# gleb-kov/wordpiece

Hardware: AMD Instinct MI355X
Metric: input MB/s tokenized (bert-base-cased vocab; offline stand-in: synthetic BERT-like vocab) (higher is better)
Workload: dtype int32

## Files before the change

wordpiece_amd/csrc/context.h:

```cpp
#pragma once
#include <array>
#include <cstring>
#include <memory>
#include <mutex>
#include <string>
#include <vector>

#include "../../include/wordpiece_amd.h"
#include "code.h"
#include "decode.h"
#include "detok.h"
#include "radix_sort.h"
#include "scanline.h"
#include "suffix_array.h"
#include "vocab.h"

namespace wp {

static thread_local std::string g_last_error;

struct EnvOptions {
  bool arena_guard;
  bool vocab_in_s;
  bool sparse_emit;
  bool no_pool;
  static bool flag(const char *name) {
    const char *e = getenv(name);
    return e && atoi(e) != 0;
  }
  static const EnvOptions &get() {
    static const EnvOptions o{flag("WP_ARENA_GUARD"), flag("WP_VOCAB_IN_S"), flag("WP_SPARSE_EMIT"), flag("WP_NO_CONTEXT_POOL")};
    return o;
  }
};

struct DeviceBuffer {
  void *p = nullptr;
  size_t cap = 0;
  void ensure(size_t bytes, bool slack = true) {
    if (bytes <= cap) return;
    if (p) WP_HIP(hipFree(p));
    p = nullptr;
    cap = 0;
    size_t want = slack ? bytes + bytes / 16 + (1 << 20) : bytes;
    WP_HIP(hipMalloc(&p, want));
    cap = want;
  }
  void release() {
    if (p) (void)hipFree(p);
    p = nullptr;
    cap = 0;
  }
};

static size_t text_room(size_t len) { return len + 64; }
static void zero_text_tail(void *d_text, size_t len, hipStream_t st) {
  WP_HIP(hipMemsetAsync(static_cast<char *>(d_text) + (len & ~static_cast<size_t>(15)), 0, 32, st));
}

constexpr size_t kGuardBytes = 256;
constexpr uint32_t kGuardWord = 0xA5C3F00Du;

__global__ __launch_bounds__(kBlock) void guard_fill_kernel(char *base, const unsigned long long *offs, int count) {
  const int z = blockIdx.x;
  if (z >= count) return;
  uint32_t *g = reinterpret_cast<uint32_t *>(base + offs[z]);
  if (threadIdx.x < kGuardBytes / 4) g[threadIdx.x] = kGuardWord;
}
__global__ __launch_bounds__(kBlock) void guard_check_kernel(const char *base, const unsigned long long *offs, int count,
                                                             uint32_t *bad) {
  const int z = blockIdx.x;
  if (z >= count) return;
  const uint32_t *g = reinterpret_cast<const uint32_t *>(base + offs[z]);
  const bool broken = threadIdx.x < kGuardBytes / 4 && g[threadIdx.x] != kGuardWord;
  if (__syncthreads_or(broken) && threadIdx.x == 0) {
    atomicAdd(&bad[0], 1u);
    atomicMin(&bad[1], static_cast<uint32_t>(z) + 1u);
  }
}

struct Arena {
  DeviceBuffer *buf;
  size_t off = 0, planned = 0;
  bool planning = true, guard = false;
  std::vector<unsigned long long> zones;
  explicit Arena(DeviceBuffer *b, bool g = false) : buf(b), guard(g) {}
  template <typename T>
  T *take(size_t count) {
    size_t bytes = (count * sizeof(T) + 255) & ~static_cast<size_t>(255);
    size_t o = off;
    off += bytes;
    if (guard) {
      if (!planning) zones.push_back(off);
      off += kGuardBytes;
    }
    if (planning) return nullptr;
    if (off > planned) throw std::logic_error("arena: the allocation sequence differs from the planned one");
    return reinterpret_cast<T *>(static_cast<char *>(buf->p) + o);
  }
  void commit() {
    buf->ensure(off + (guard ? 8 * 512 : 0));
    planned = off;
    off = 0;
    planning = false;
  }
  unsigned long long *zone_table() const {
    return reinterpret_cast<unsigned long long *>(static_cast<char *>(buf->p) + ((off + 255) & ~static_cast<size_t>(255)));
  }
  void arm(hipStream_t st) {
    if (!guard || zones.empty()) return;
    if (zones.size() > 500) throw std::logic_error("arena guard: too many allocations");
    WP_HIP(hipMemcpyAsync(zone_table(), zones.data(), zones.size() * sizeof(unsigned long long), hipMemcpyHostToDevice, st));
    WP_HIP(hipStreamSynchronize(st));
    hipLaunchKernelGGL(guard_fill_kernel, dim3(zones.size()), dim3(kBlock), 0, st, static_cast<char *>(buf->p), zone_table(),
                       static_cast<int>(zones.size()));
  }
  void check(hipStream_t st, uint32_t *bad) const {
    if (!guard || zones.empty()) return;
    hipLaunchKernelGGL(guard_check_kernel, dim3(zones.size()), dim3(kBlock), 0, st, static_cast<const char *>(buf->p),
                       zone_table(), static_cast<int>(zones.size()), bad);
  }
};

static int bit_length(uint64_t v) {
  int b = 0;
  while (v) {
    b++;
    v >>= 1;
  }
  return b;
}

constexpr int kScalars = 56;
constexpr int kScalarCps = 0;
constexpr int kScalarAlphabet = 1;
constexpr int kScalarInvalid = 2;
constexpr int kScalarList = 4;
constexpr int kScalarListEntries = kScalarList + 0;
constexpr int kScalarListGroups = kScalarList + 1;
constexpr int kScalarListLargeGroups = kScalarList + 2;
constexpr int kScalarListLargeEntries = kScalarList + 3;
constexpr int kScalarListWanted = 8;
constexpr int kScalarIds = 9;
constexpr int kScalarAnchors = 10;
constexpr int kScalarAnchorGap = 11;
constexpr int kScalarLongWords = 12;
constexpr int kScalarWideWords = 13;
constexpr int kScalarCps64 = 14;
constexpr int kScalarGuard = 16;
constexpr int kScalarGuardBad = kScalarGuard + 0;
constexpr int kScalarGuardFirst = kScalarGuard + 1;
constexpr int kScalarSplitTotals = 18;
constexpr int kScalarAlphaWord0 = 20;
constexpr int kScalarRows = 21, kScalarRowsBad = 22, kScalarRowsCut = 23;
constexpr int kScalarCand = 24;
constexpr int kScalarKept = 25;
constexpr int kScalarSrcRows = 26;
constexpr int kScalarInCut = 27, kScalarInRows = 28, kScalarInWindowed = 30;
constexpr int kScalarFree31 = 31;
constexpr int kScalarMask = 32;
constexpr int kScalarDetokLast = 44, kScalarDetokBad = 46;
constexpr int kScalarFree47 = 47;
constexpr int kScalarDetok = 48;
constexpr int kScalarNormBytes = kScalarCps;
constexpr int kScalarNormCps = kScalarAlphabet;
constexpr int kScalarNormSrcCps = kScalarListEntries;
constexpr int kScalarNormBytes64 = kScalarCps64;

struct ScalarRange {
  int first, words;
};
constexpr ScalarRange kScalarLayout[] = {
    {kScalarCps, 1},         {kScalarAlphabet, 1},   {kScalarInvalid, 2},         {kScalarListEntries, 1},
    {kScalarListGroups, 1},  {kScalarListLargeGroups, 1}, {kScalarListLargeEntries, 1}, {kScalarListWanted, 1},
    {kScalarIds, 1},         {kScalarAnchors, 1},    {kScalarAnchorGap, 1},       {kScalarLongWords, 1},
    {kScalarWideWords, 1},   {kScalarCps64, 2},      {kScalarGuardBad, 1},        {kScalarGuardFirst, 1},
    {kScalarSplitTotals, 2},      {kScalarAlphaWord0, 1}, {kScalarRows, 1},            {kScalarRowsBad, 1},
    {kScalarRowsCut, 1},     {kScalarCand, 1},       {kScalarKept, 1},            {kScalarSrcRows, 1},
    {kScalarInCut, 1},       {kScalarInRows, 2},     {kScalarInWindowed, 1},      {kScalarFree31, 1},
    {kScalarMask, 12},       {kScalarDetokLast, 2},  {kScalarDetokBad, 1},        {kScalarFree47, 1},
    {kScalarDetok, 8}};
constexpr int scalar_end(int slot) {
  for (const ScalarRange &r : kScalarLayout) {
    if (slot < r.first + r.words) return r.first + r.words;
  }
  return kScalars;
}
constexpr bool scalar_layout_ok() {
  int at = 0;
  for (const ScalarRange &r : kScalarLayout) {
    if (r.first != at || r.words < 1 || (r.words % 2 == 0 && r.first % 2 != 0)) return false;
    at += r.words;
  }
  return at == kScalars;
}
static_assert(scalar_layout_ok(), "the scalar table must cover d_scalars word by word, 64-bit slots on even words");
static_assert(kScalarList % 2 == 0 && kScalarListLargeGroups % 2 == 0, "both halves of the list block are also read as 64-bit words");

struct RowsCall {
  const long long *d_doc_off = nullptr;
  size_t n_docs = 0;
  int unit = -1;
  size_t capacity = SIZE_MAX;
  size_t n_rows = 0;
  const long long *d_starts = nullptr;
  const long long *d_row_splits = nullptr;
  uint32_t *d_line_cnt = nullptr;
};

enum SideEvent { kEvFork, kEvJoin, kEvScalars, kEvKeysFree, kEvPartition, kEvTrieNodes, kEvLargeSorted, kEvKeysBuilt, kEvCandCount,
                 kEvSpine, kEvKept, kEvSorted, kEvListBuilt, kEvRoundDone, kSideEvents };
enum TimingMark { kMarkStart, kMarkCounted, kMarkSymbols, kMarkSorted, kMarkLcp, kMarkScanned, kMarkWalked, kMarkNormStart,
                  kMarkRound0, kTimingMarks, kMarkNormEnd = kMarkStart };

struct Context {
  int device = 0;
  hipStream_t stream = nullptr;
  hipStream_t stream2 = nullptr;
  hipStream_t stream3 = nullptr;
  hipEvent_t evs[kSideEvents] = {};
  uint32_t *d_stream = nullptr, *d_elig_start = nullptr, *d_elig_info = nullptr, *d_soft = nullptr;
  uint32_t *d_vocab_word_idx = nullptr, *d_vocab_word_bits = nullptr;
  uint8_t *d_cls_bmp = nullptr;
  uint32_t *d_lt_chain_len = nullptr, *d_lt_chain_off = nullptr, *d_lt_child_begin = nullptr, *d_lt_child_cp = nullptr,
           *d_lt_child_node = nullptr, *d_elig_node = nullptr, *d_elig_subtree = nullptr;
  int32_t *d_elig_id = nullptr, *d_tok_len = nullptr;
  uint8_t *d_tok_class = nullptr;
  DetokRec *d_detok_rec = nullptr;
  uint8_t *d_detok_pool = nullptr;
  size_t detok_pool_bytes = 0;
  unsigned long long *d_trie_key = nullptr;
  uint32_t *d_trie_child = nullptr;
  int32_t *d_trie_id = nullptr;
  DeviceBuffer text_buf, a_buf, b_buf, fmt_buf;
  DeviceBuffer text_buf2, ids_stage[2];
  DeviceBuffer rows_in, rows_out, pad_buf;
  DeviceBuffer inputs_buf;
  DeviceBuffer detok_in, detok_aux, detok_out;
  uint16_t *d_norm_index = nullptr;
  uint32_t *d_norm_pages = nullptr, *d_norm_pool = nullptr;
  DeviceBuffer norm_buf, norm_aux, norm_map;
  hipStream_t up_stream = nullptr, down_stream = nullptr;
  hipEvent_t pipe_ev[4] = {};
  uint32_t *d_used = nullptr, *d_lut = nullptr, *d_scan_tmp = nullptr;
  uint32_t *d_scalars = nullptr;
  uint8_t *d_code = nullptr;
  size_t list_hint = 0;
  SymbolCode code_cache;
  bool code_cached = false;
  uint32_t code_alphabet = 0;
  int code_bits = 0, code_lo = 0, code_uses = 0;
  double code_blank_share = 0.0;
  uint8_t *h_code = nullptr;
  uint32_t *d_symhist = nullptr;
  uint32_t *h_scalars = nullptr;
  RadixStats rstats;
  hipEvent_t ev[kTimingMarks] = {};
  const int32_t *d_ids = nullptr;
  const uint32_t *d_offs = nullptr;
  struct {
    const void *sym = nullptr;
    int sym_bytes = 0;
    const uint32_t *sa = nullptr, *cps = nullptr;
    const RankEntry *rank = nullptr;
    const int32_t *lcp = nullptr;
    const uint8_t *cls = nullptr;
    StepTable steps{};
    int32_t *best_scratch = nullptr;
    const int32_t *step_views = nullptr;
    size_t n = 0, n_text = 0;
  } dbg;
  std::array<DeviceBuffer *, 17> buffers() {
    return {&text_buf, &a_buf,    &b_buf,   &fmt_buf,    &text_buf2, &ids_stage[0], &ids_stage[1], &rows_in,   &rows_out,
            &pad_buf,  &inputs_buf, &norm_buf, &norm_aux, &norm_map, &detok_in,     &detok_aux,    &detok_out};
  }
  Context() = default;
  Context(const Context &) = delete;
  Context &operator=(const Context &) = delete;
  ~Context();
};

struct DeviceGuard {
  int prev = -1;
  DeviceGuard() {
    if (hipGetDevice(&prev) != hipSuccess) prev = -1;
  }
  ~DeviceGuard() {
    if (prev >= 0) (void)hipSetDevice(prev);
  }
  DeviceGuard(const DeviceGuard &) = delete;
  DeviceGuard &operator=(const DeviceGuard &) = delete;
};

#ifdef WP_DEBUG_BOUNDS
static void take_oob(int first, int count, unsigned int *oob) {
  WP_HIP(hipMemcpyFromSymbol(oob, HIP_SYMBOL(g_wp_oob), count * sizeof(unsigned int), first * sizeof(unsigned int)));
  bool any = false;
  for (int i = 0; i < count; i++) any = any || oob[i] != 0;
  if (!any) return;
  const unsigned int zero[kBoundSites] = {};
  WP_HIP(hipMemcpyToSymbol(HIP_SYMBOL(g_wp_oob), zero, count * sizeof(unsigned int), first * sizeof(unsigned int)));
}
#endif

}

using namespace wp;

struct EncodeStats : wp_stats {
  int32_t normalize;
  int64_t norm_bytes;
  double ms_normalize;
  wp_walk_stats walk;
  wp_refine_stats refine;
  wp_refine_sched sched;
  wp_step_stats step;
  wp_inputs_stats inputs;
  int32_t inputs_call;
  wp_mask_stats mask;
  int32_t mask_call;
  wp_detok_stats detok;
  int32_t detok_call;
};

#ifndef WP_LATE_REFINE_DEFAULT
#define WP_LATE_REFINE_DEFAULT 0
#endif

struct wp_vocab {
  HostVocab hv;
  std::unique_ptr<Context> ctx;
  std::vector<std::unique_ptr<Context>> multi;
  int device = -1;
  bool full_depth = false, keep_debug = false, stage_timing = false, lcp_kasai = false, cover_anchors = false;
  bool keep_step_views = false;
  bool arena_guard = false;
  bool sparse_emit = false;
  bool vocab_in_s = false;
  bool indexed_round0 = false;
  bool sort_blanks = false;
  bool late_refine = WP_LATE_REFINE_DEFAULT != 0;
  int normalize = 0;
  int n_devices = 1;
  EncodeStats stats{};
  ~wp_vocab();
};

namespace wp {

template <typename... T>
static void free_dev(T *&...p) {
  (((p ? (void)hipFree(p) : (void)0), p = nullptr), ...);
}

static void free_vocab_tables(Context *c) {
  free_dev(c->d_stream, c->d_elig_start, c->d_elig_info, c->d_soft, c->d_elig_id, c->d_tok_len, c->d_tok_class, c->d_detok_rec, c->d_detok_pool, c->d_trie_key,
           c->d_trie_child, c->d_trie_id, c->d_vocab_word_idx, c->d_vocab_word_bits, c->d_cls_bmp, c->d_lt_chain_len,
           c->d_lt_chain_off, c->d_lt_child_begin, c->d_lt_child_cp, c->d_lt_child_node, c->d_elig_node, c->d_elig_subtree);
}

template <size_t N>
static void destroy_events(hipEvent_t (&events)[N]) {
  for (auto &e : events) {
    if (e) (void)hipEventDestroy(e);
    e = nullptr;
  }
}

static void destroy_context(Context *c) {
  if (!c) return;
  bool owns = c->stream || c->stream2 || c->stream3 || c->d_used || c->d_lut || c->d_scan_tmp || c->d_scalars || c->d_code ||
              c->d_symhist || c->h_scalars || c->h_code || c->d_stream;
  for (DeviceBuffer *b : c->buffers()) owns = owns || b->p;
  if (!owns) return;
  DeviceGuard keep;
  (void)hipSetDevice(c->device);
  free_vocab_tables(c);
  free_dev(c->d_used, c->d_lut, c->d_scan_tmp, c->d_scalars, c->d_code, c->d_symhist, c->d_norm_index, c->d_norm_pages, c->d_norm_pool);
  if (c->h_scalars) (void)hipHostFree(c->h_scalars);
  if (c->h_code) (void)hipHostFree(c->h_code);
  c->h_scalars = nullptr;
  c->h_code = nullptr;
  for (DeviceBuffer *b : c->buffers()) b->release();
  destroy_events(c->pipe_ev);
  destroy_events(c->ev);
  destroy_events(c->evs);
  for (hipStream_t *s : {&c->up_stream, &c->down_stream, &c->stream3, &c->stream2, &c->stream}) {
    if (*s) (void)hipStreamDestroy(*s);
    *s = nullptr;
  }
}
Context::~Context() { destroy_context(this); }

template <typename T>
static T *upload(const std::vector<T> &v, hipStream_t st) {
  T *d = nullptr;
  WP_HIP(hipMalloc(&d, std::max<size_t>(v.size(), 1) * sizeof(T)));
  if (!v.empty()) WP_HIP(hipMemcpyAsync(d, v.data(), v.size() * sizeof(T), hipMemcpyHostToDevice, st));
  return d;
}

static constexpr size_t kPoolArenaBytes = size_t(256) << 20;
static constexpr size_t kPoolContexts = 4;
static std::mutex g_pool_mu;
static std::vector<std::unique_ptr<Context>> &context_pool() {
  static auto *pool = new std::vector<std::unique_ptr<Context>>();
  return *pool;
}

static void release_arenas(Context *c) {
  for (DeviceBuffer *b : c->buffers()) b->release();
  c->d_ids = nullptr;
  c->d_offs = nullptr;
  c->dbg = {};
}

static void park_context(std::unique_ptr<Context> c) {
  if (!c) return;
  const bool no_pool = EnvOptions::get().no_pool;
  DeviceGuard keep;
  (void)hipSetDevice(c->device);
  if (!no_pool && hipStreamSynchronize(c->stream) == hipSuccess && hipStreamSynchronize(c->stream2) == hipSuccess &&
      hipStreamSynchronize(c->stream3) == hipSuccess) {
    free_vocab_tables(c.get());
    size_t held = 0;
    for (DeviceBuffer *b : c->buffers()) held += b->cap;
    if (held > kPoolArenaBytes) release_arenas(c.get());
    c->d_ids = nullptr;
    c->d_offs = nullptr;
    c->dbg = {};
    std::lock_guard<std::mutex> g(g_pool_mu);
    if (context_pool().size() < kPoolContexts) {
      context_pool().push_back(std::move(c));
      return;
    }
  }
  destroy_context(c.get());
}

static void upload_vocab_tables(Context *c, const HostVocab &hv) {
  c->d_stream = upload(hv.stream, c->stream);
  c->d_elig_start = upload(hv.elig_start, c->stream);
  c->d_elig_info = upload(hv.elig_info, c->stream);
  c->d_elig_id = upload(hv.elig_id, c->stream);
  c->d_tok_len = upload(hv.tok_len, c->stream);
  c->d_soft = upload(hv.soft, c->stream);
  c->d_vocab_word_idx = upload(hv.used_word_idx, c->stream);
  c->d_vocab_word_bits = upload(hv.used_word_bits, c->stream);
  c->d_cls_bmp = upload(hv.cls_bmp, c->stream);
  c->d_lt_chain_len = upload(hv.lt_chain_len, c->stream);
  c->d_lt_chain_off = upload(hv.lt_chain_off, c->stream);
  c->d_lt_child_begin = upload(hv.lt_child_begin, c->stream);
  c->d_lt_child_cp = upload(hv.lt_child_cp, c->stream);
  c->d_lt_child_node = upload(hv.lt_child_node, c->stream);
  c->d_elig_node = upload(hv.elig_node, c->stream);
  c->d_elig_subtree = upload(hv.elig_subtree, c->stream);
  {
    std::vector<unsigned long long> tk(hv.trie_key.begin(), hv.trie_key.end());
    c->d_trie_key = upload(tk, c->stream);
    WP_HIP(hipStreamSynchronize(c->stream));
  }
  c->d_trie_child = upload(hv.trie_child, c->stream);
  c->d_trie_id = upload(hv.trie_id, c->stream);
  WP_HIP(hipStreamSynchronize(c->stream));
}

static int device_count_or_throw() {
  int count = 0;
  if (hipGetDeviceCount(&count) != hipSuccess || count == 0) {
    throw HipError("no HIP device available: the Linear WordPiece path has no CPU fallback");
  }
  return count;
}

static std::unique_ptr<Context> make_context(const wp_vocab *v, int device) {
  const int count = device_count_or_throw();
  if (device >= 0) {
    if (device >= count) throw std::invalid_argument("no such HIP device: " + std::to_string(device));
  } else {
    WP_HIP(hipGetDevice(&device));
  }
  WP_HIP(hipSetDevice(device));
  std::unique_ptr<Context> c;
  {
    std::lock_guard<std::mutex> g(g_pool_mu);
    auto &pool = context_pool();
    for (size_t i = 0; i < pool.size(); i++) {
      if (pool[i]->device == device) {
        c = std::move(pool[i]);
        pool.erase(pool.begin() + static_cast<long>(i));
        break;
      }
    }
  }
  if (c) {
    upload_vocab_tables(c.get(), v->hv);
    return c;
  }
  c.reset(new Context());
  c->device = device;
  WP_HIP(hipStreamCreateWithFlags(&c->stream, hipStreamNonBlocking));
  WP_HIP(hipStreamCreateWithFlags(&c->stream2, hipStreamNonBlocking));
  WP_HIP(hipStreamCreateWithFlags(&c->stream3, hipStreamNonBlocking));
  for (auto &e : c->evs) WP_HIP(hipEventCreateWithFlags(&e, hipEventDisableTiming));
  WP_HIP(hipMalloc(&c->d_used, sizeof(uint32_t) * kCpWords));
  WP_HIP(hipMalloc(&c->d_lut, sizeof(uint32_t) * kCpTableSize));
  WP_HIP(hipMalloc(&c->d_scan_tmp, sizeof(uint32_t) * kCpWords));
  WP_HIP(hipMalloc(&c->d_scalars, sizeof(uint32_t) * kScalars));
  WP_HIP(hipMalloc(&c->d_code, 512 + 256 + kDecodeTableBytes));
  WP_HIP(hipHostMalloc(&c->h_code, 512 + 256 + kDecodeTableBytes));
  WP_HIP(hipMalloc(&c->d_symhist, sizeof(uint32_t) * 256));
  WP_HIP(hipHostMalloc(&c->h_scalars, sizeof(uint32_t) * kScalars));
  for (auto &e : c->ev) WP_HIP(hipEventCreate(&e));
  upload_vocab_tables(c.get(), v->hv);
  return c;
}

static Context *get_context(wp_vocab *v) {
  if (!v->ctx) v->ctx = make_context(v, v->device);
  WP_HIP(hipSetDevice(v->ctx->device));
  return v->ctx.get();
}

static void queue_scalars(Context *c, int last, hipStream_t st) {
  WP_HIP(hipMemcpyAsync(c->h_scalars, c->d_scalars, sizeof(uint32_t) * scalar_end(last), hipMemcpyDeviceToHost, st));
}
static void fetch_scalars(Context *c, int last) {
  queue_scalars(c, last, c->stream);
  WP_HIP(hipStreamSynchronize(c->stream));
}
static void clear_scalars(Context *c, int first, int last, hipStream_t st) {
  WP_HIP(hipMemsetAsync(c->d_scalars + first, 0, sizeof(uint32_t) * (scalar_end(last) - first), st));
}

}
```

wordpiece_amd/csrc/linear_path.h:

```cpp
#pragma once
#include <functional>

#include "context.h"
#include "local_sort.h"
#include "prune.h"
#include "trie.h"
#include "offsets.h"
#include "normalize.h"
#include "rows.h"
#include "walk.h"

namespace wp {

struct ListOverflow {
  size_t wanted;
};

__global__ void needed_list_clamp_kernel(uint32_t *__restrict__ totals, uint32_t cap, uint32_t *__restrict__ wanted) {
  if (totals[0] > cap) {
    *wanted = totals[0];
    totals[0] = 0;
    totals[1] = 0;
  }
}

constexpr double kBlankDropMinShare = 1.0 / 16;

#ifdef WP_DEBUG_BOUNDS
__device__ unsigned int g_wp_sorted_sig[6];
__global__ __launch_bounds__(kBlock) void sorted_check_kernel(const uint32_t *__restrict__ sorted, size_t n_sorted,
                                                              const uint32_t *__restrict__ unsorted, size_t n,
                                                              const uint8_t *__restrict__ cls, size_t n_text,
                                                              const uint32_t *__restrict__ blank_bits) {
  __shared__ uint32_t acc[7];
  if (threadIdx.x < 7) acc[threadIdx.x] = 0u;
  __syncthreads();
  uint32_t bad = 0, cnt[2] = {0, 0}, sum[2] = {0, 0}, x[2] = {0, 0};
  const size_t first = static_cast<size_t>(blockIdx.x) * kBlock + threadIdx.x, stride = static_cast<size_t>(gridDim.x) * kBlock;
  for (size_t i = first; i < n_sorted; i += stride) {
    const uint32_t k = sorted[i];
    if (i + 1 < n_sorted && k > sorted[i + 1]) bad++;
    if (blank_bits && key_is_blank(blank_bits, k)) bad++;
    cnt[0]++;
    sum[0] += k;
    x[0] ^= k;
  }
  for (size_t i = first; i < n; i += stride) {
    if (blank_bits && i < n_text && (cls[i] & kClsSpace)) continue;
    const uint32_t k = unsorted[i];
    cnt[1]++;
    sum[1] += k;
    x[1] ^= k;
  }
  if (bad) atomicAdd(&acc[6], bad);
  for (int s = 0; s < 2; s++) {
    if (cnt[s]) {
      atomicAdd(&acc[3 * s], cnt[s]);
      atomicAdd(&acc[3 * s + 1], sum[s]);
      atomicXor(&acc[3 * s + 2], x[s]);
    }
  }
  __syncthreads();
  if (threadIdx.x < 6 && acc[threadIdx.x]) {
    if (threadIdx.x % 3 == 2) {
      atomicXor(&g_wp_sorted_sig[threadIdx.x], acc[threadIdx.x]);
    } else {
      atomicAdd(&g_wp_sorted_sig[threadIdx.x], acc[threadIdx.x]);
    }
  }
  if (threadIdx.x == 6 && acc[6]) atomicAdd(&g_wp_oob[kSiteSortOrder], acc[6]);
}
__global__ void sorted_check_close_kernel() {
  bool same = true;
  for (int j = 0; j < 3; j++) same = same && g_wp_sorted_sig[j] == g_wp_sorted_sig[3 + j];
  wp_in_bounds(same, kSiteSortOrder);
  for (int j = 0; j < 6; j++) g_wp_sorted_sig[j] = 0u;
}
#endif

template <typename SymT>
struct LinearPath {
  const wp_vocab *v;
  Context *c;
  EncodeStats &S;
  Arena &ar, &aa;
  const uint8_t *d_text;
  size_t nbytes;
  const uint32_t *d_tile_prefix;
  size_t n_text, n;
  uint32_t *d_cps;
  uint8_t *d_cls;
  int bits;
  bool text_only;
  int offs_unit;
  RowsCall *rows;
  const NormMap *nmap;

  hipStream_t st, st2;
  const HostVocab &hv;
  bool full, prune, use_trie, key_lookup, keys_only, window_store, use_digit_bytes, staged_possible, sparse_emit;
  bool early_refine;
  bool wide_ran = false;
  uint32_t need_depth;
  int M, P, P_cap, bucket_shift, bucket_shift_all, key_shift, key_shift_all, hb_n, win_mid;
  unsigned sl_tiles, sl_groups, nbuckets, nbuckets_all, nkbuckets, nkbuckets_all;
  size_t radix_words, emit_tiles, walk_blocks, claim_size, list_cap;

  SymT *d_sym = nullptr, *d_vsym = nullptr;
  Key0 *KA = nullptr, *KB = nullptr;
  uint32_t *VA = nullptr, *VB = nullptr;
  uint32_t *X0 = nullptr, *X1 = nullptr;
  uint8_t *DG0 = nullptr, *DG1 = nullptr;
  RankEntry *d_rank = nullptr;
  uint32_t *d_node_of_slot = nullptr;
  int32_t *d_lcp = nullptr;
  uint32_t *d_sa = nullptr, *d_gdepth = nullptr;
  RankEntry *d_hd_n = nullptr;
  int32_t *d_emit = nullptr, *d_dbg_best = nullptr;
  int32_t *d_step_views = nullptr;
  uint32_t *d_anchors = nullptr, *d_anchor_cnt = nullptr, *d_anchor_tmp = nullptr, *d_emit_cnt = nullptr, *d_emit_tmp = nullptr,
           *d_blk_cnt = nullptr, *d_blk_off = nullptr, *d_tile_scratch = nullptr;
  uint32_t *AS0 = nullptr, *AS1 = nullptr, *AG = nullptr, *AD0 = nullptr, *AD1 = nullptr, *LA = nullptr, *LB = nullptr, *d_tdep = nullptr;
  uint64_t *LK0 = nullptr, *LK1 = nullptr, *LK2 = nullptr;
  uint32_t *LV0 = nullptr, *LV1 = nullptr, *LPOS = nullptr;
  uint32_t *d_ghead = nullptr, *d_gneed0 = nullptr, *d_gneed1 = nullptr, *d_lg_head = nullptr, *d_lg_off = nullptr;
  RerankAgg *d_agg = nullptr, *d_chunk_agg = nullptr;
  uint32_t *d_claim = nullptr, *d_claim_need = nullptr, *d_gclaim = nullptr, *d_gfirst = nullptr, *d_gdep = nullptr, *d_gnode = nullptr,
           *d_gdone = nullptr, *d_rng_lo = nullptr, *d_rng_hi = nullptr, *d_child_sym = nullptr, *d_radix_tmp = nullptr,
           *d_radix_tmp2 = nullptr;
  uint8_t *d_rng_long = nullptr;
  uint32_t *d_mslot0 = nullptr, *d_mslot1 = nullptr, *d_midx0 = nullptr, *d_midx1 = nullptr, *d_minfo = nullptr, *d_tile_mlo = nullptr;
  int32_t *d_mid = nullptr, *d_rf = nullptr, *d_rb = nullptr, *d_cover_f = nullptr, *d_cover_b = nullptr;
  int32_t *d_tmin_f = nullptr, *d_tmin_b = nullptr, *d_gmin_f = nullptr, *d_gmin_b = nullptr, *d_pval_p = nullptr, *d_pval_s = nullptr;
  uint32_t *d_ps0 = nullptr, *d_ps1 = nullptr, *d_pv0 = nullptr, *d_pv1 = nullptr, *d_bidx = nullptr;
  int2 *d_bfast = nullptr, *d_bfast_all = nullptr;
  uint32_t *d_bidx_all = nullptr;
  uint32_t *d_gend = nullptr, *d_kstart = nullptr, *d_kbidx = nullptr, *d_kbidx_all = nullptr;
  int32_t *d_kval_p = nullptr, *d_kval_s = nullptr;
  int2 *d_kbfast = nullptr, *d_kbfast_all = nullptr;
  unsigned long long *d_cand_table = nullptr;
  uint32_t *d_cand_filter = nullptr, *d_cand_lo = nullptr, *d_cand_hi = nullptr, *d_gcand = nullptr;
  uint32_t *d_tok_group = nullptr;
  uint32_t *d_cand_bcnt = nullptr, *d_cand_boff = nullptr, *d_cand_scan = nullptr;
  int cand_bits = 0;
  uint32_t *d_blank_bits = nullptr;
  uint2 *d_ospill = nullptr, *d_cspan = nullptr, *d_offs = nullptr;
  uint32_t *d_byte_of = nullptr;
  long long *d_line_starts = nullptr, *d_row_splits = nullptr;
  uint32_t *d_row_base = nullptr;

  SymbolCode code;
  DevCode dcode{};
  DigitBytes db;
  RadixPlan sort_plan;
  bool hist_in_keys = false;
  bool drop_blanks = false;
  size_t n_sorted = 0;
  int cur = 0, rounds = 1;
  Key0 *keys = nullptr, *other_keys = nullptr;
  uint32_t *vals = nullptr, *other_vals = nullptr, *slots = nullptr, *other_slots = nullptr, *adep = nullptr, *other_dep = nullptr;
  uint32_t *avals = nullptr, *spare_vals = nullptr;
  bool classified = false, anchors_queued = false;
  size_t n_act = 0, n_large = 0, n_large_groups = 0, n_groups = 0;
  StepTable steps{}, steps_all{};
  StepTable ksteps{}, ksteps_all{};
  CandSet cand{};
  CandRuns cand_runs{};
  size_t n_cand = 0;

  LinearPath(const wp_vocab *v_, Context *c_, EncodeStats &S_, Arena &ar_, Arena &aa_, const uint8_t *text, size_t nb,
             const uint32_t *tile_prefix, size_t n_text_, size_t n_, uint32_t *cps, uint8_t *cls, int bits_, bool text_only_,
             int offs_unit_, RowsCall *rows_ = nullptr, const NormMap *nmap_ = nullptr)
      : v(v_), c(c_), S(S_), ar(ar_), aa(aa_), d_text(text), nbytes(nb), d_tile_prefix(tile_prefix), n_text(n_text_), n(n_),
        d_cps(cps), d_cls(cls), bits(bits_), text_only(text_only_), offs_unit(offs_unit_), rows(rows_), nmap(nmap_), st(c_->stream), st2(c_->stream2),
        hv(v_->hv) {
    full = v->full_depth || hv.n_dup_eligible > 0 || v->lcp_kasai;
    need_depth = static_cast<uint32_t>(std::min<int64_t>(hv.longest + 1, 0x7fffffff));
    M = static_cast<int>(hv.elig_id.size());
    prune = !full && (M > 0 || text_only);
    use_trie = text_only && !full && M > 0;
    key_lookup = use_trie && !v->keep_debug && kKeyBits <= 32;
    keys_only = key_lookup && !v->indexed_round0 && sizeof(SymT) == 1;
    early_refine = keys_only && !v->late_refine;
    sl_tiles = cdiv(n, kSlTile);
    sl_groups = cdiv(sl_tiles, kSlGroup);
    P = kStepsPerMark * M + 1;
    P_cap = P + 2 * M + 2;
    const int bucket_bits = std::min(kStepBucketBitsMax, std::max(kStepBucketBits, bit_length(4 * static_cast<size_t>(P))));
    bucket_shift = std::max(0, bit_length(n) - bucket_bits);
    nbuckets = static_cast<unsigned>(((n - 1) >> bucket_shift) + 1);
    bucket_shift_all = std::max(0, bit_length(n) - kStepBucketBits);
    nbuckets_all = static_cast<unsigned>(((n - 1) >> bucket_shift_all) + 1);
    const int kb = std::min(kKeyBits, std::max(1, bit_length(n - 1) - bucket_shift));
    const int kb_all = std::min(kKeyBits, std::max(1, bit_length(n - 1) - bucket_shift_all));
    key_shift = kKeyBits - kb;
    key_shift_all = kKeyBits - kb_all;
    nkbuckets = 1u << kb;
    nkbuckets_all = 1u << kb_all;
    radix_words = std::max(radix_tmp_words<uint64_t>(n), radix_tmp_words<uint32_t>(std::max<size_t>(n, static_cast<size_t>(P_cap))));
    emit_tiles = cdiv(std::max<size_t>(n_text, 1), kScanTile);
    walk_blocks = cdiv(std::max<size_t>(n_text, 1), kBlock);
    sparse_emit = v->sparse_emit || EnvOptions::get().sparse_emit;
    staged_possible = !sparse_emit && !v->cover_anchors && hv.soft.empty();
    use_digit_bytes = n > kRadixSmallN;
    claim_size = 1024;
    while (claim_size < 2 * static_cast<size_t>(std::max(M, 1))) claim_size *= 2;
    cand_bits = bit_length(claim_size - 1);
    hb_n = bit_length(n - 1);
    window_store = n >= (1u << 22);
    win_mid = hb_n - kWinBits <= kRadixBits ? hb_n : kWinBits + (hb_n - kWinBits + 1) / 2;
    if (!prune) {
      list_cap = n;
    } else {
      const size_t guess = c->list_hint ? c->list_hint : n / 8;
      list_cap = std::min(n, guess + guess / 4 + 65536);
    }
    S.symbol_bits = bits;
    S.full_depth = full;
    S.trie_refine = use_trie ? 1 : 0;
    S.key_bits = kKeyBits;
    S.round0_keys_only = keys_only ? 1 : 0;
    S.round0_candidates = keys_only ? 0 : -1;
    n_sorted = n;
    S.round0_sorted = static_cast<int64_t>(n);
  }

  void fork() {
    WP_HIP(hipEventRecord(c->evs[kEvFork], st));
    WP_HIP(hipStreamWaitEvent(st2, c->evs[kEvFork], 0));
  }
  void join() {
    WP_HIP(hipEventRecord(c->evs[kEvJoin], st2));
    WP_HIP(hipStreamWaitEvent(st, c->evs[kEvJoin], 0));
  }

  void plan() {
    const bool ref = !text_only;
    const bool want_lcp = ref || v->keep_debug;
    const size_t lc = list_cap, lg = lc / 2 + static_cast<size_t>(M) + 8;
    const size_t rr_tiles_l = cdiv(lc, kRrTile);
    const size_t rtiles = cdiv(std::max<size_t>(n_text, 1), kReachTile);
    for (int pass = 0; pass < 2; pass++) {
      d_sym = ar.take<SymT>(n + 16);
      KA = ar.take<Key0>(n + 16);
      KB = ar.take<Key0>(n + 16);
      VA = ar.take<uint32_t>(n + 16);
      VB = ar.take<uint32_t>(n + 16);
      X0 = ar.take<uint32_t>(n + 16);
      X1 = ar.take<uint32_t>(n + 16);
      DG0 = use_digit_bytes ? ar.take<uint8_t>(n + 64) : nullptr;
      DG1 = use_digit_bytes ? ar.take<uint8_t>(n + 64) : nullptr;
      d_rank = ar.take<RankEntry>(n);
      d_node_of_slot = use_trie ? ar.take<uint32_t>(n) : nullptr;
      d_lcp = want_lcp ? ar.take<int32_t>(n) : nullptr;
      d_sa = (v->keep_debug || v->lcp_kasai) ? ar.take<uint32_t>(n) : nullptr;
      d_gdepth = (use_trie && !want_lcp) ? nullptr : ar.take<uint32_t>(n);
      d_hd_n = (want_lcp || !prune) ? ar.take<RankEntry>(n + 16) : nullptr;
      d_dbg_best = v->keep_debug ? ar.take<int32_t>(2 * n) : nullptr;
      d_emit = ar.take<int32_t>(n_text + 1);
      d_anchors = ar.take<uint32_t>(n_text + 1);
      d_anchor_cnt = ar.take<uint32_t>(emit_tiles + 1);
      d_anchor_tmp = ar.take<uint32_t>(cdiv(emit_tiles, kScanTile) + 8);
      d_emit_cnt = ar.take<uint32_t>(emit_tiles + 1);
      d_emit_tmp = ar.take<uint32_t>(cdiv(walk_blocks, kScanTile) + 8);
      d_blk_cnt = ar.take<uint32_t>(walk_blocks + 2);
      d_blk_off = ar.take<uint32_t>(walk_blocks + 2);
      d_tile_scratch = ar.take<uint32_t>(5 * (rtiles + 2) + 4 * (n_text / kMaxAnchorGap + 4));
      AS0 = ar.take<uint32_t>(lc);
      AS1 = ar.take<uint32_t>(lc);
      AG = ar.take<uint32_t>(lc);
      AD0 = ar.take<uint32_t>(lc);
      AD1 = ar.take<uint32_t>(lc);
      LA = ar.take<uint32_t>(lc);
      LB = ar.take<uint32_t>(lc);
      d_tdep = ar.take<uint32_t>(lc + 2);
      LK0 = ar.take<uint64_t>(lc + 2);
      LK1 = ar.take<uint64_t>(lc + 2);
      LK2 = ar.take<uint64_t>(lc + 2);
      LV0 = ar.take<uint32_t>(lc);
      LV1 = ar.take<uint32_t>(lc);
      LPOS = ar.take<uint32_t>(lc + 16);
      d_ghead = ar.take<uint32_t>(lg);
      d_gneed0 = use_trie ? nullptr : ar.take<uint32_t>(lg);
      d_gneed1 = use_trie ? nullptr : ar.take<uint32_t>(lg);
      d_lg_head = ar.take<uint32_t>(lc / kLsMaxGroup + 4);
      d_lg_off = ar.take<uint32_t>(lc / kLsMaxGroup + 4);
      d_agg = ar.take<RerankAgg>(rr_tiles_l + 1);
      d_chunk_agg = ar.take<RerankAgg>(cdiv(rr_tiles_l, kRrChunk) + 1);
      d_radix_tmp = ar.take<uint32_t>(radix_words);
      d_radix_tmp2 = use_trie ? ar.take<uint32_t>(std::max(radix_tmp_words<uint64_t>(lc), keys_only ? radix_tmp_words<uint32_t>(n) : 0))
                              : nullptr;
      d_claim = ar.take<uint32_t>(claim_size);
      if (keys_only) {
        uint32_t *zeroed = ar.take<uint32_t>(3 * claim_size);
        d_cand_lo = zeroed;
        d_cand_hi = zeroed ? zeroed + claim_size : nullptr;
        d_claim_need = zeroed ? zeroed + 2 * claim_size : nullptr;
      } else {
        d_claim_need = ar.take<uint32_t>(claim_size);
      }
      d_gclaim = ar.take<uint32_t>(M + 4);
      d_gfirst = ar.take<uint32_t>(M + 4);
      d_gdep = ar.take<uint32_t>(M + 4);
      d_gnode = ar.take<uint32_t>(M + 4);
      d_gdone = ar.take<uint32_t>(M + 4);
      d_rng_lo = ar.take<uint32_t>(M + 1);
      d_rng_hi = ar.take<uint32_t>(M + 1);
      d_rng_long = ar.take<uint8_t>(M + 1);
      d_vsym = use_trie ? ar.take<SymT>(hv.stream.size() + 16) : nullptr;
      d_child_sym = use_trie ? ar.take<uint32_t>(hv.lt_child_cp.size() + 1) : nullptr;
      d_mslot0 = ar.take<uint32_t>(M + 1);
      d_mslot1 = ar.take<uint32_t>(M + 1);
      d_midx0 = ar.take<uint32_t>(M + 1);
      d_midx1 = ar.take<uint32_t>(M + 1);
      d_mid = ar.take<int32_t>(M + 1);
      d_minfo = ar.take<uint32_t>(M + 1);
      d_rf = ar.take<int32_t>(M + 1);
      d_cover_f = ar.take<int32_t>(2 * static_cast<size_t>(M) + 2);
      d_cover_b = ar.take<int32_t>(2 * static_cast<size_t>(M) + 2);
      d_rb = ar.take<int32_t>(M + 1);
      d_tile_mlo = ref ? ar.take<uint32_t>(sl_tiles + 2) : nullptr;
      d_tmin_f = ref ? ar.take<int32_t>(sl_tiles + 1) : nullptr;
      d_tmin_b = ref ? ar.take<int32_t>(sl_tiles + 1) : nullptr;
      d_gmin_f = ref ? ar.take<int32_t>(sl_groups + 1) : nullptr;
      d_gmin_b = ref ? ar.take<int32_t>(sl_groups + 1) : nullptr;
      d_ps0 = ar.take<uint32_t>(P_cap + 1);
      d_ps1 = ar.take<uint32_t>(P_cap + 1);
      d_pv0 = ar.take<uint32_t>(P_cap + 1);
      d_pv1 = ar.take<uint32_t>(P_cap + 1);
      d_pval_p = ar.take<int32_t>(P_cap + 1);
      d_pval_s = ar.take<int32_t>(P_cap + 1);
      d_bidx = ar.take<uint32_t>(static_cast<size_t>(nbuckets) + 2);
      d_bfast = ar.take<int2>(static_cast<size_t>(nbuckets) + 1);
      d_bidx_all = bucket_shift_all != bucket_shift ? ar.take<uint32_t>(static_cast<size_t>(nbuckets_all) + 2) : nullptr;
      d_bfast_all = bucket_shift_all != bucket_shift ? ar.take<int2>(static_cast<size_t>(nbuckets_all) + 1) : nullptr;
      d_gend = key_lookup ? ar.take<uint32_t>(M + 4) : nullptr;
      d_kstart = key_lookup ? ar.take<uint32_t>(P_cap + 1) : nullptr;
      d_kval_p = key_lookup ? ar.take<int32_t>(P_cap + 1) : nullptr;
      d_kval_s = key_lookup ? ar.take<int32_t>(P_cap + 1) : nullptr;
      d_kbidx = key_lookup ? ar.take<uint32_t>(static_cast<size_t>(nkbuckets) + 2) : nullptr;
      d_kbfast = key_lookup ? ar.take<int2>(static_cast<size_t>(nkbuckets) + 1) : nullptr;
      d_kbidx_all = (key_lookup && key_shift_all != key_shift) ? ar.take<uint32_t>(static_cast<size_t>(nkbuckets_all) + 2) : nullptr;
      d_kbfast_all = (key_lookup && key_shift_all != key_shift) ? ar.take<int2>(static_cast<size_t>(nkbuckets_all) + 1) : nullptr;
      d_cand_table = keys_only ? ar.take<unsigned long long>(claim_size) : nullptr;
      d_cand_filter = keys_only ? ar.take<uint32_t>(kCandFilterWords) : nullptr;
      d_gcand = keys_only ? ar.take<uint32_t>(M + 4) : nullptr;
      d_tok_group = keys_only ? ar.take<uint32_t>(M + 1) : nullptr;
      d_cand_bcnt = keys_only ? ar.take<uint32_t>(cdiv(n, kKeyTile) + 2) : nullptr;
      d_cand_boff = keys_only ? ar.take<uint32_t>(cdiv(n, kKeyTile) + 2) : nullptr;
      d_cand_scan = keys_only ? ar.take<uint32_t>(cdiv(cdiv(n, kKeyTile), kScanTile) + 8) : nullptr;
      d_blank_bits = keys_only ? ar.take<uint32_t>(kBlankWords) : nullptr;
      const bool offs = offs_unit >= 0;
      d_ospill = offs ? ar.take<uint2>(n_text + 16) : nullptr;
      d_cspan = offs ? ar.take<uint2>(n_text + 16) : nullptr;
      d_offs = offs ? ar.take<uint2>(n_text + 1) : nullptr;
      d_byte_of = ((offs_unit == WP_OFFSETS_BYTES && !nmap) || rows) ? ar.take<uint32_t>(n_text + 1) : nullptr;
      d_line_starts = (rows && (!rows->d_doc_off || nmap)) ? ar.take<long long>(rows->n_rows + 1) : nullptr;
      d_row_splits = rows ? ar.take<long long>(rows->n_rows + 1) : nullptr;
      d_row_base = (rows && rows->unit >= 0) ? ar.take<uint32_t>(rows->n_rows + 1) : nullptr;
      d_step_views = v->keep_step_views ? ar.take<int32_t>(4 * n_text + 4) : nullptr;
      if (pass == 0) ar.commit();
    }
    ar.arm(st);
  }

  void launch_anchors(hipStream_t as) {
    anchors_queued = true;
    const unsigned atiles = cdiv(n_text, kAnchorTile);
    if (!staged_possible) WP_HIP(hipMemsetAsync(d_emit, 0x80, n_text * sizeof(int32_t), as));
    hipLaunchKernelGGL(anchor_count_kernel, dim3(atiles), dim3(kBlock), 0, as, d_cls, static_cast<const uint8_t *>(nullptr),
                       n_text, d_anchor_cnt);
    device_exclusive_scan(d_anchor_cnt, d_anchor_cnt, atiles, d_anchor_tmp, c->d_scalars + kScalarAnchors, as);
    hipLaunchKernelGGL(anchor_write_kernel, dim3(atiles), dim3(kBlock), 0, as, d_cls, static_cast<const uint8_t *>(nullptr),
                       n_text, d_anchor_cnt, d_anchors);
    hipLaunchKernelGGL(anchor_gap_kernel, dim3(std::min<size_t>(atiles, 1024)), dim3(kBlock), 0, as, d_anchors,
                       c->d_scalars + kScalarAnchors, n_text, d_cls, hv.soft.empty() ? 1 : 0, c->d_scalars + kScalarAnchorGap);
  }

  void symbols_and_keys() {
    const int lo_bits = sizeof(SymT) == 1 ? 0 : std::max(0, bits - 8);
    constexpr int kCodeReuse = 64;
    const bool reuse_code = c->code_cached && c->code_alphabet == static_cast<uint32_t>(S.alphabet) && c->code_bits == bits &&
                            c->code_lo == lo_bits && c->code_uses < kCodeReuse;
    if (!reuse_code) WP_HIP(hipMemsetAsync(c->d_symhist, 0, sizeof(uint32_t) * 256, st));
    constexpr uint32_t kBlankCpRuns[3][2] = {{0x09, 7}, {0x20, 2}, {kSpaceToken, 2}};
    uint32_t h_blank_lut[3][7] = {};
    hipLaunchKernelGGL(HIP_KERNEL_NAME(decode_write_kernel<SymT>), dim3(cdiv(nbytes, kDecTile)), dim3(kBlock), 0, st, d_text,
                       nbytes, d_tile_prefix, c->d_lut, d_sym, d_cls, d_cps, c->d_cls_bmp, c->d_soft,
                       static_cast<int>(hv.soft.size()), reuse_code ? nullptr : c->d_symhist, lo_bits);
    hipLaunchKernelGGL(HIP_KERNEL_NAME(map_vocab_symbols_kernel<SymT>), dim3(cdiv(n - n_text, kBlock)), dim3(kBlock), 0, st,
                       c->d_stream, n_text, n, c->d_lut, d_sym);
    if (reuse_code) {
      code = c->code_cache;
      c->code_uses++;
    } else {
      std::vector<uint32_t> h32(256);
      WP_HIP(hipMemcpyAsync(h32.data(), c->d_symhist, sizeof(uint32_t) * 256, hipMemcpyDeviceToHost, st));
      if (sizeof(SymT) == 1) {
        for (int r = 0; r < 3; r++) {
          WP_HIP(hipMemcpyAsync(h_blank_lut[r], c->d_lut + kBlankCpRuns[r][0], sizeof(uint32_t) * kBlankCpRuns[r][1],
                                hipMemcpyDeviceToHost, st));
        }
      }
      WP_HIP(hipStreamSynchronize(st));
      const size_t nitems = (static_cast<size_t>(S.alphabet) >> lo_bits) + 1;
      std::vector<uint64_t> freq(nitems);
      for (size_t i = 0; i < nitems; i++) freq[i] = h32[i];
      code = build_symbol_code(freq, bits, true);
      if (!code.uniform_bits) {
        code.lo_bits = lo_bits;
        code.avg_bits += lo_bits;
      }
      c->code_cache = code;
      c->code_cached = true;
      c->code_alphabet = static_cast<uint32_t>(S.alphabet);
      c->code_bits = bits;
      c->code_lo = lo_bits;
      c->code_uses = 0;
      uint64_t all = 0, blank = 0;
      for (size_t i = 0; i < nitems; i++) all += freq[i];
      if (sizeof(SymT) == 1) {
        for (int r = 0; r < 3; r++) {
          for (uint32_t k = 0; k + 1 < kBlankCpRuns[r][1]; k++) {
            const uint32_t cp = kBlankCpRuns[r][0] + k, s = h_blank_lut[r][k] + 1u;
            if (is_space(cp) && h_blank_lut[r][k + 1] != h_blank_lut[r][k] && s < nitems) blank += freq[s];
          }
        }
      }
      c->code_blank_share = all ? static_cast<double>(blank) / static_cast<double>(all) : 0.0;
      if (!code.uniform_bits) {
        const size_t blob_bytes = 512 + 256 + kDecodeTableBytes;
        std::memset(c->h_code, 0, blob_bytes);
        std::memcpy(c->h_code, code.cw.data(), code.cw.size() * sizeof(uint16_t));
        std::memcpy(c->h_code + 512, code.len.data(), code.len.size());
        std::memcpy(c->h_code + 768, code.bmask.data(), kDecodeTableBytes);
        WP_HIP(hipMemcpyAsync(c->d_code, c->h_code, blob_bytes, hipMemcpyHostToDevice, st));
      }
    }
    dcode = DevCode{reinterpret_cast<const uint16_t *>(c->d_code), c->d_code + 512, c->d_code + 768,
                    code.uniform_bits ? code.uniform_bits : -code.lo_bits};
    S.symbols_per_key = static_cast<int32_t>(kKeyBits / std::max(1.0, code.avg_bits));
    if (keys_only) {
      WP_HIP(hipMemsetAsync(d_cand_table, 0, claim_size * sizeof(unsigned long long), st));
      WP_HIP(hipMemsetAsync(d_cand_filter, 0, kCandFilterWords * sizeof(uint32_t), st));
      hipLaunchKernelGGL(long_key_set_kernel, dim3(cdiv(static_cast<size_t>(M) * kWave, kBlock)), dim3(kBlock), 0, st, c->d_stream,
                         c->d_elig_start, c->d_elig_info, M, c->d_lut, dcode, d_cand_table, cand_bits, d_cand_filter);
      cand.filter = d_cand_filter;
      cand.table = d_cand_table;
      cand.table_bits = cand_bits;
      cand.slot = VA;
      cand.pos = VB;
      cand.bcount = d_cand_bcnt;
    }
    size_t cand_blocks = 0;
    int min_len = code.uniform_bits ? code.uniform_bits : 99;
    for (uint8_t l : code.len) min_len = std::min<int>(min_len, l);
    if (sizeof(SymT) == 1 && min_len >= kKeys8MinLen) {
      cand.tile = kKeys8Tile;
      cand_blocks = cdiv(n, kKeys8Tile);
      if (n > kRadixSmallN) {
        sort_plan = radix_plan<Key0>(n, d_radix_tmp, radix_words, st);
        hist_in_keys = true;
      }
      drop_blanks = keys_only && hist_in_keys && !v->sort_blanks && c->code_blank_share >= kBlankDropMinShare;
      if (drop_blanks) {
        hipLaunchKernelGGL(blank_bits_kernel, dim3(1), dim3(kBlankWords), 0, st, c->d_lut, dcode, d_blank_bits);
      }
      hipLaunchKernelGGL(build_keys0_u8_kernel, dim3(cdiv(n, kKeys8Tile)), dim3(kKeys8Threads), 0, st,
                         reinterpret_cast<const uint8_t *>(d_sym), n, dcode, KA, hist_in_keys ? nullptr : DG0,
                         hist_in_keys ? sort_plan.table : nullptr, hist_in_keys ? sort_plan.chunk_sums0 : nullptr, cand,
                         drop_blanks ? d_blank_bits : nullptr);
    } else {
      cand.tile = kKeyTile;
      cand_blocks = cdiv(n, kKeyTile);
      if (keys_only) {
        hipLaunchKernelGGL(HIP_KERNEL_NAME(build_keys0_kernel<SymT, true>), dim3(cdiv(n, kKeyTile)), dim3(kBlock), 0, st, d_sym, n,
                           dcode, KA, DG0, cand);
      } else {
        hipLaunchKernelGGL(HIP_KERNEL_NAME(build_keys0_kernel<SymT, false>), dim3(cdiv(n, kKeyTile)), dim3(kBlock), 0, st, d_sym, n,
                           dcode, KA, DG0, cand);
      }
    }
    if (keys_only) {
      WP_HIP(hipEventRecord(c->evs[kEvKeysBuilt], st));
      WP_HIP(hipStreamWaitEvent(st2, c->evs[kEvKeysBuilt], 0));
      device_exclusive_scan(d_cand_bcnt, d_cand_boff, cand_blocks, d_cand_scan, c->d_scalars + kScalarCand, st2);
      hipLaunchKernelGGL(cand_compact_kernel, dim3(cand_blocks), dim3(kBlock), 0, st2, VA, VB, d_cand_bcnt, d_cand_boff, cand.tile, n,
                         X1, d_node_of_slot);
      WP_HIP(hipMemcpyAsync(c->h_scalars + kScalarCand, c->d_scalars + kScalarCand, sizeof(uint32_t), hipMemcpyDeviceToHost, st2));
      WP_HIP(hipEventRecord(c->evs[kEvCandCount], st2));
    }
    WP_LAUNCH_CHECK();
  }

  void sort_round0() {
    db.dg0 = DG0;
    db.dg1 = DG1;
    db.dg0_ready = DG0 != nullptr && !hist_in_keys;
    if (key_lookup) {
      Key0 *sk = reinterpret_cast<Key0 *>(X0);
      RadixDrop drop;
      drop.blank_bits = d_blank_bits;
      drop.d_kept = c->d_scalars + kScalarKept;
      drop.h_kept = c->h_scalars + kScalarKept;
      drop.side = st2;
      drop.spine_done = c->evs[kEvSpine];
      drop.copied = c->evs[kEvKept];
      cur = radix_sort_pairs<Key0>(sk, keys_only ? nullptr : VA, KB, keys_only ? nullptr : VB, n, 0, kKeyBits, d_radix_tmp, radix_words,
                                   st, &c->rstats, true, code.uniform_bits ? 0 : 8, db, true, hist_in_keys ? &sort_plan : nullptr, KA,
                                   drop_blanks ? &drop : nullptr);
      if (drop_blanks) n_sorted = drop.kept;
      S.round0_sorted = static_cast<int64_t>(n_sorted);
      S.hist_in_keys = hist_in_keys ? 1 : 0;
      keys = cur ? KB : sk;
      other_keys = cur ? sk : KB;
#ifdef WP_DEBUG_BOUNDS
      if constexpr (sizeof(Key0) == 4) {
        hipLaunchKernelGGL(sorted_check_kernel, dim3(std::min<size_t>(cdiv(n, kBlock), 1024)), dim3(kBlock), 0, st,
                           reinterpret_cast<const uint32_t *>(keys), n_sorted, reinterpret_cast<const uint32_t *>(KA), n, d_cls, n_text,
                           drop_blanks ? d_blank_bits : static_cast<const uint32_t *>(nullptr));
        hipLaunchKernelGGL(sorted_check_close_kernel, dim3(1), dim3(1), 0, st);
        WP_LAUNCH_CHECK();
      }
#endif
      vals = keys_only ? nullptr : (cur ? VB : VA);
      other_vals = keys_only ? nullptr : (cur ? VA : VB);
      if (keys_only) sort_candidates();
      slots = AS0;
      other_slots = AS1;
      adep = AD0;
      other_dep = AD1;
      avals = LA;
      spare_vals = LB;
      return;
    }
    if (window_store) {
      db.tail_bit = kWinBits;
      db.tail_mask = (1u << (win_mid - kWinBits)) - 1u;
      db.tail_from_val = true;
    }
    cur = radix_sort_pairs<Key0>(KA, VA, KB, VB, n, 0, kKeyBits, d_radix_tmp, radix_words, st, &c->rstats, true,
                                 code.uniform_bits ? 0 : 8, db, true, hist_in_keys ? &sort_plan : nullptr);
    S.hist_in_keys = hist_in_keys ? 1 : 0;
    keys = cur ? KB : KA;
    other_keys = cur ? KA : KB;
    vals = cur ? VB : VA;
    other_vals = cur ? VA : VB;
    slots = AS0;
    other_slots = AS1;
    adep = AD0;
    other_dep = AD1;
    avals = LA;
    spare_vals = LB;
  }

  void sort_candidates() {
    WP_HIP(hipEventSynchronize(c->evs[kEvCandCount]));
    n_cand = c->h_scalars[kScalarCand];
    S.round0_candidates = static_cast<int64_t>(n_cand);
    WP_HIP(hipMemsetAsync(d_cand_lo, 0, 3 * claim_size * sizeof(uint32_t), st2));
    const uint32_t *sorted_slot = X1, *sorted_pos = d_node_of_slot;
    if (n_cand > 1) {
      const int cc = radix_sort_pairs<uint32_t>(X1, d_node_of_slot, VA, VB, n_cand, 0, cand_bits, d_radix_tmp2,
                                                std::max(radix_tmp_words<uint64_t>(list_cap), radix_tmp_words<uint32_t>(n)), st2, nullptr,
                                                false, cand_bits, DigitBytes(), true);
      sorted_slot = cc ? VA : X1;
      sorted_pos = cc ? VB : d_node_of_slot;
    }
    if (n_cand > 0) {
      hipLaunchKernelGGL(cand_runs_kernel, dim3(cdiv(n_cand, kBlock)), dim3(kBlock), 0, st2, sorted_slot, n_cand, d_cand_lo, d_cand_hi);
    }
    WP_LAUNCH_CHECK();
    cand_runs.table = d_cand_table;
    cand_runs.bits = cand_bits;
    cand_runs.lo = d_cand_lo;
    cand_runs.hi = d_cand_hi;
    cand_runs.pos = sorted_pos;
  }

  bool classify_groups(size_t list_len) {
    if (list_len <= static_cast<size_t>(kLsMaxGroup)) return false;
    const size_t cap = list_len / 2 + 1;
    clear_scalars(c, kScalarListLargeGroups, kScalarListLargeEntries, st2);
    hipLaunchKernelGGL(large_groups_kernel, dim3(std::min<size_t>(cdiv(cap, kBlock), 2048)), dim3(kBlock), 0, st2, d_ghead,
                       c->d_scalars + kScalarListGroups, reinterpret_cast<unsigned long long *>(c->d_scalars + kScalarListLargeGroups),
                       d_lg_head, d_lg_off);
    hipLaunchKernelGGL(large_groups_close_kernel, dim3(1), dim3(1), 0, st2, c->d_scalars + kScalarListLargeGroups, d_lg_off);
    return true;
  }

  void store_ranks(uint32_t *dst, uint32_t *val, uint32_t *t_dst, uint32_t *t_val, size_t m) {
    if (val && m >= (1u << 22)) {
      const int hb = bit_length(n - 1);
      const int bc = radix_sort_pairs<uint32_t>(dst, val, t_dst, t_val, m, std::max(0, hb - 8), hb, d_radix_tmp, radix_words, st,
                                                nullptr, false, hb + 1, DigitBytes(), true);
      hipLaunchKernelGGL(scatter_pairs_kernel, dim3(cdiv(m, kSpTile)), dim3(kBlock), 0, st, bc ? t_dst : dst, bc ? t_val : val, m,
                         d_rank, n, 1);
    } else {
      hipLaunchKernelGGL(scatter_pairs_kernel, dim3(cdiv(m, kSpTile)), dim3(kBlock), 0, st, dst, val, m, d_rank, n, 0);
    }
  }

  void store_ranks_round0(uint32_t *dst, uint32_t *val, uint8_t *dig, uint8_t *other, const std::function<void()> &before_second,
                          const std::function<void()> &before_window) {
    WP_HIP(hipFuncSetAttribute(reinterpret_cast<const void *>(window_store_kernel), hipFuncAttributeMaxDynamicSharedMemorySize,
                               static_cast<int>(kWinLdsBytes)));
    uint32_t *a_dst = X0, *a_val = X1, *b_dst = other_vals, *b_val = reinterpret_cast<uint32_t *>(keys);
    DigitBytes d1;
    d1.dg0 = dig;
    d1.dg1 = other;
    d1.dg0_ready = dig != nullptr;
    if (win_mid < hb_n) {
      d1.tail_bit = win_mid;
      d1.tail_mask = (1u << (hb_n - win_mid)) - 1u;
    }
    radix_sort_pairs<uint32_t>(dst, val, a_dst, a_val, n, kWinBits, win_mid, d_radix_tmp, radix_words, st, &c->rstats,
                               val == nullptr, 0, d1, true);
    if (before_second) before_second();
    const uint32_t *f_dst = a_dst, *f_val = a_val;
    if (win_mid < hb_n) {
      DigitBytes d2;
      d2.dg0 = dig ? d1.tail_out(1) : nullptr;
      d2.dg1 = dig ? dig : nullptr;
      d2.dg0_ready = dig != nullptr;
      radix_sort_pairs<uint32_t>(a_dst, a_val, b_dst, b_val, n, win_mid, hb_n, d_radix_tmp, radix_words, st, &c->rstats, false, 0,
                                 d2);
      f_dst = b_dst;
      f_val = b_val;
    }
    if (before_window) before_window();
    hipLaunchKernelGGL(window_store_kernel, dim3(cdiv(n, size_t(1) << kWinBits)), dim3(kWinThreads), kWinLdsBytes, st, f_dst, f_val,
                       n, d_rank);
  }

  void ranks_round0() {
    const DepthRule rule{need_depth, full ? 1 : 0, nullptr, nullptr, 0, nullptr};
    const unsigned tiles = cdiv(n, kRrTile);
    const bool slot_ranks = text_only && !d_lcp;
    uint8_t *dig = DG0 ? db.tail_out(cur) : nullptr, *dig_other = DG0 ? db.tail_out(cur ^ 1) : nullptr;
    auto enqueue_needed_groups = [&](hipEvent_t start_after) {
      if (start_after) WP_HIP(hipStreamWaitEvent(st2, start_after, 0));
      WP_HIP(hipMemsetAsync(d_claim, 0xff, claim_size * sizeof(uint32_t), st2));
      if (!keys_only) WP_HIP(hipMemsetAsync(d_claim_need, 0, claim_size * sizeof(uint32_t), st2));
      NeededList nl{slots, avals, AG, adep, d_ghead, d_gfirst, d_gdep, reinterpret_cast<unsigned long long *>(c->d_scalars + kScalarList),
                    static_cast<uint32_t *>(nullptr), need_depth, d_claim_need, d_gclaim, d_gneed0,
                    keys_only ? d_gcand : nullptr, keys_only ? cand_runs.pos : nullptr, keys_only ? n_cand : 0};
      const TokenTrie trie{c->d_lt_chain_len, c->d_lt_chain_off, c->d_lt_child_begin, c->d_lt_child_node, d_child_sym};
      if (use_trie) {
        const size_t ns = hv.stream.size(), nc = hv.lt_child_cp.size();
        hipLaunchKernelGGL(HIP_KERNEL_NAME(trie_map_symbols_kernel<SymT>), dim3(cdiv(std::max<size_t>(std::max(ns, nc), 1), kBlock)),
                           dim3(kBlock), 0, st2, c->d_stream, ns, c->d_lt_child_cp, nc, c->d_lut, d_vsym, d_child_sym);
      }
      if (M > 0) {
        hipLaunchKernelGGL(HIP_KERNEL_NAME(need_groups_kernel<SymT>), dim3(cdiv(static_cast<size_t>(M) * kWave, kBlock)),
                           dim3(kBlock), 0, st2, keys, vals, n_sorted, n, d_sym, c->d_stream, c->d_elig_start, c->d_elig_info, M, c->d_lut, dcode,
                           d_claim, static_cast<uint32_t>(claim_size - 1), nl, text_only ? d_rng_lo : nullptr, d_rng_hi, d_rng_long,
                           cand_runs);
      }
      hipLaunchKernelGGL(needed_list_clamp_kernel, dim3(1), dim3(1), 0, st2, c->d_scalars + kScalarList, static_cast<uint32_t>(list_cap),
                         c->d_scalars + kScalarListWanted);
      hipLaunchKernelGGL(needed_list_close_kernel, dim3(1), dim3(1), 0, st2, c->d_scalars + kScalarList, d_ghead);
      if (key_lookup) {
        hipLaunchKernelGGL(group_starts_kernel, dim3(cdiv(M, kBlock)), dim3(kBlock), 0, st2, d_gfirst, d_ghead, c->d_scalars + kScalarList,
                           n_sorted, d_ps0 + P, d_gend);
      }
      if (M > 0) {
        if (!use_trie) hipLaunchKernelGGL(needed_need_kernel, dim3(cdiv(M, kBlock)), dim3(kBlock), 0, st2, nl);
        hipLaunchKernelGGL(needed_fill_kernel, dim3(1024), dim3(kBlock), 0, st2, nl, vals, n_sorted);
        if (use_trie) {
          hipLaunchKernelGGL(HIP_KERNEL_NAME(trie_group_start_kernel<SymT>), dim3(cdiv(M, kBlock)), dim3(kBlock), 0, st2, vals,
                             keys_only ? cand_runs.pos : nullptr, d_gcand, d_gfirst,
                             d_gdep, c->d_scalars + kScalarList, d_sym, n, d_vsym, trie, d_gnode, d_gdone);
        }
      }
      WP_HIP(hipEventRecord(c->evs[kEvKeysFree], st2));
      if (use_trie) trie_round_sizes();
    };
    if (early_refine) {
      refine_early();
      return;
    }
    if (key_lookup) {
      fork();
      enqueue_needed_groups(nullptr);
      trie_round_sort();
      if (n_text > 0) launch_anchors(st);
      WP_LAUNCH_CHECK();
      trie_round_finish();
      return;
    }
    if (prune) {
      fork();
      enqueue_needed_groups(nullptr);
      if (!slot_ranks) {
        hipLaunchKernelGGL(round0_rank_kernel<true>, dim3(cdiv(n, kR0Tile)), dim3(kBlock), 0, st, keys, vals, n, dcode.first_len,
                           dcode.uniform_bits, d_sa, d_hd_n, d_lcp, d_gdepth);
      }
    } else {
      hipLaunchKernelGGL(widen_keys_kernel, dim3(std::min<size_t>(cdiv(n, kBlock), 8192)), dim3(kBlock), 0, st, keys, LK2, n);
      hipLaunchKernelGGL(HIP_KERNEL_NAME(rerank_agg_kernel<true>), dim3(tiles), dim3(kBlock), 0, st, LK2, vals, n,
                         static_cast<const uint32_t *>(nullptr), static_cast<const RankEntry *>(nullptr),
                         static_cast<const uint32_t *>(nullptr), n, dcode.first_len, dcode.uniform_bits, rule, d_tdep, d_agg);
      hipLaunchKernelGGL(rerank_chunk_kernel, dim3(cdiv(tiles, kRrChunk)), dim3(kBlock), 0, st, d_agg, tiles, d_chunk_agg);
      hipLaunchKernelGGL(rerank_prefix_kernel, dim3(cdiv(tiles, kRrChunk)), dim3(kBlock), 0, st, d_agg, d_chunk_agg, tiles);
      hipLaunchKernelGGL(HIP_KERNEL_NAME(rerank_apply_kernel<SymT, true>), dim3(tiles), dim3(kBlock), 0, st, LK2, vals,
                         static_cast<const uint32_t *>(nullptr), static_cast<const uint32_t *>(nullptr), d_tdep, n, d_agg, d_sym, n,
                         dcode.first_len, dcode.uniform_bits, rule, d_sa, d_hd_n, d_lcp, slots, avals, AG, adep, d_ghead, d_gdepth,
                         c->d_scalars + kScalarList);
    }
    uint32_t *rank_vals = slot_ranks ? nullptr : reinterpret_cast<uint32_t *>(d_hd_n);
    auto keys_free = [&] {
      if (prune) WP_HIP(hipStreamWaitEvent(st, c->evs[kEvKeysFree], 0));
    };
    auto start_trie_round = [&] {
      if (!use_trie) return;
      WP_HIP(hipEventRecord(c->evs[kEvPartition], st));
      WP_HIP(hipStreamWaitEvent(st2, c->evs[kEvPartition], 0));
      trie_round_sort();
    };
    if (window_store) {
      store_ranks_round0(vals, rank_vals, dig, dig_other, keys_free, start_trie_round);
    } else {
      keys_free();
      start_trie_round();
      store_ranks(vals, rank_vals, X0, X1, n);
    }
    WP_LAUNCH_CHECK();
    if (use_trie) {
      trie_round_finish();
    } else {
      if (prune) join();
      fork();
      classified = classify_groups(std::min(n, list_cap));
      join();
    }
  }

  void refine_early() {
    WP_HIP(hipMemsetAsync(d_claim, 0xff, claim_size * sizeof(uint32_t), st2));
    NeededList nl{slots, avals, AG, adep, d_ghead, static_cast<uint32_t *>(nullptr), d_gdep,
                  reinterpret_cast<unsigned long long *>(c->d_scalars + kScalarList), static_cast<uint32_t *>(nullptr), need_depth,
                  d_claim_need, d_gclaim, d_gneed0, d_gcand, cand_runs.pos, n_cand};
    const TokenTrie trie{c->d_lt_chain_len, c->d_lt_chain_off, c->d_lt_child_begin, c->d_lt_child_node, d_child_sym};
    const size_t ns = hv.stream.size(), nc = hv.lt_child_cp.size();
    const unsigned tok_blocks = cdiv(static_cast<size_t>(M) * kWave, kBlock);
    hipLaunchKernelGGL(HIP_KERNEL_NAME(trie_map_symbols_kernel<SymT>), dim3(cdiv(std::max<size_t>(std::max(ns, nc), 1), kBlock)),
                       dim3(kBlock), 0, st2, c->d_stream, ns, c->d_lt_child_cp, nc, c->d_lut, d_vsym, d_child_sym);
    hipLaunchKernelGGL(HIP_KERNEL_NAME(need_groups_early_kernel<SymT>), dim3(tok_blocks), dim3(kBlock), 0, st2, n, d_sym, c->d_stream,
                       c->d_elig_start, c->d_elig_info, M, c->d_lut, dcode, d_claim, nl, d_rng_lo, d_rng_hi, d_rng_long, cand_runs);
    hipLaunchKernelGGL(needed_list_clamp_kernel, dim3(1), dim3(1), 0, st2, c->d_scalars + kScalarList, static_cast<uint32_t>(list_cap),
                       c->d_scalars + kScalarListWanted);
    hipLaunchKernelGGL(needed_list_close_kernel, dim3(1), dim3(1), 0, st2, c->d_scalars + kScalarList, d_ghead);
    hipLaunchKernelGGL(needed_fill_kernel, dim3(1024), dim3(kBlock), 0, st2, nl, static_cast<const uint32_t *>(nullptr), n_sorted);
    hipLaunchKernelGGL(HIP_KERNEL_NAME(trie_group_start_kernel<SymT>), dim3(cdiv(M, kBlock)), dim3(kBlock), 0, st2,
                       static_cast<const uint32_t *>(nullptr), cand_runs.pos, d_gcand, static_cast<const uint32_t *>(nullptr), d_gdep,
                       c->d_scalars + kScalarList, d_sym, n, d_vsym, trie, d_gnode, d_gdone);
    WP_HIP(hipEventRecord(c->evs[kEvListBuilt], st2));
    trie_round_sizes();
    trie_round_sort();
    S.sched.early = 1;
    WP_HIP(hipEventRecord(c->evs[kEvSorted], st));
    WP_HIP(hipStreamWaitEvent(st, c->evs[kEvListBuilt], 0));
    hipLaunchKernelGGL(need_ranges_kernel, dim3(tok_blocks), dim3(kBlock), 0, st, keys, n_sorted, c->d_stream, c->d_elig_start,
                       c->d_elig_info, M, c->d_lut, dcode, d_claim, d_gfirst, d_rng_lo, d_rng_hi, d_rng_long, d_tok_group);
    hipLaunchKernelGGL(group_starts_kernel, dim3(cdiv(M, kBlock)), dim3(kBlock), 0, st, d_gfirst, d_ghead, c->d_scalars + kScalarList,
                       n_sorted, d_ps0 + P, d_gend);
    WP_LAUNCH_CHECK();
    trie_round_finish();
  }

  int trie_rb() const { return bit_length(hv.lt_chain_len.size() + 1); }
  void trie_round_sizes() {
    classified = classify_groups(list_cap);
    queue_scalars(c, kScalarAnchorGap, st2);
    WP_HIP(hipEventRecord(c->evs[kEvScalars], st2));
  }
  void trie_round_sort() {
    const TokenTrie trie{c->d_lt_chain_len, c->d_lt_chain_off, c->d_lt_child_begin, c->d_lt_child_node, d_child_sym};
    hipLaunchKernelGGL(HIP_KERNEL_NAME(trie_walk_kernel<SymT>), dim3(std::min<size_t>(cdiv(list_cap, kBlock), 16384)), dim3(kBlock), 0,
                       st2, avals, AG, d_gnode, d_gdone, c->d_scalars + kScalarList, d_sym, n, d_vsym, trie, adep);
    WP_HIP(hipEventRecord(c->evs[kEvTrieNodes], st2));
    hipLaunchKernelGGL(local_sort_kernel, dim3(cdiv(list_cap, kLsT)), dim3(kBlock), 0, st2, avals, AG, adep, c->d_scalars + kScalarList,
                       d_ghead, d_rank, n, trie_rb(), LK0, spare_vals, adep);
  }
  void refine_stats(size_t groups, int rbits) {
    S.refine.n_groups = static_cast<int64_t>(groups);
    S.refine.n_entries = static_cast<int64_t>(n_act);
    S.refine.n_large_groups = static_cast<int64_t>(n_large_groups);
    S.refine.n_large_entries = static_cast<int64_t>(n_large);
    S.refine.trie_nodes = static_cast<int64_t>(hv.lt_chain_len.size());
    S.refine.sort_bits = rbits;
    S.refine.key_lookup = key_lookup ? 1 : 0;
    S.refine.symbol_bytes = static_cast<int32_t>(sizeof(SymT));
  }
  void trie_round_finish() {
    WP_HIP(hipEventSynchronize(c->evs[kEvScalars]));
    n_act = c->h_scalars[kScalarListEntries];
    n_groups = c->h_scalars[kScalarListGroups];
    n_large_groups = classified ? c->h_scalars[kScalarListLargeGroups] : 0;
    n_large = classified ? c->h_scalars[kScalarListLargeEntries] : 0;
    if (c->h_scalars[kScalarListWanted] > list_cap) throw ListOverflow{c->h_scalars[kScalarListWanted]};
    S.active_per_round[0] = static_cast<int64_t>(n);
    refine_stats(n_groups, trie_rb());
    uint64_t *skeys = LK0;
    RankEntry *hd = reinterpret_cast<RankEntry *>(LK1);
    if (n_act > 0) {
      S.active_per_round[1] = static_cast<int64_t>(n_act);
      const int rb = trie_rb();
      if (n_large > 0) {
        hipStream_t st3 = c->stream3;
        WP_HIP(hipStreamWaitEvent(st3, c->evs[kEvTrieNodes], 0));
        const int lgb = bit_length(n_large_groups > 0 ? n_large_groups - 1 : 0);
        hipLaunchKernelGGL(large_extract_kernel, dim3(cdiv(cdiv(n_large, kLxSpan), kBlock / kWave)), dim3(kBlock), 0, st3, avals, adep,
                           d_lg_head, d_lg_off, static_cast<uint32_t>(n_large_groups), n_large, d_rank, n, rb, LK1, LV0, LPOS, adep);
        const int lc = radix_sort_pairs<uint64_t>(LK1, LV0, LK2, LV1, n_large, 0, rb + lgb, d_radix_tmp2,
                                                  radix_tmp_words<uint64_t>(list_cap), st3, nullptr);
        hipLaunchKernelGGL(large_writeback_kernel, dim3(std::min<size_t>(cdiv(n_large, kBlock), 8192)), dim3(kBlock), 0, st3,
                           lc ? LK2 : LK1, lc ? LV1 : LV0, LPOS, n_large, AG, rb, skeys, spare_vals);
        WP_HIP(hipEventRecord(c->evs[kEvLargeSorted], st3));
        WP_HIP(hipStreamWaitEvent(st2, c->evs[kEvLargeSorted], 0));
      }
      DepthRule rrule{need_depth, 0, nullptr, nullptr, 1, d_node_of_slot};
      const unsigned tiles = cdiv(n_act, kRrTile);
      hipLaunchKernelGGL(HIP_KERNEL_NAME(rerank_agg_kernel<false>), dim3(tiles), dim3(kBlock), 0, st2, skeys, spare_vals, n_act, adep,
                         d_rank, d_gdepth, n, dcode.first_len, dcode.uniform_bits, rrule, d_tdep, d_agg);
      hipLaunchKernelGGL(rerank_chunk_kernel, dim3(cdiv(tiles, kRrChunk)), dim3(kBlock), 0, st2, d_agg, tiles, d_chunk_agg);
      hipLaunchKernelGGL(rerank_prefix_kernel, dim3(cdiv(tiles, kRrChunk)), dim3(kBlock), 0, st2, d_agg, d_chunk_agg, tiles);
      hipLaunchKernelGGL(HIP_KERNEL_NAME(rerank_apply_kernel<SymT, false>), dim3(tiles), dim3(kBlock), 0, st2, skeys, spare_vals, slots,
                         adep, d_tdep, n_act, d_agg, d_sym, n, dcode.first_len, dcode.uniform_bits, rrule, d_sa, hd, d_lcp,
                         other_slots, avals, AG, other_dep, d_ghead, d_gdepth,
                         c->d_scalars + (early_refine ? kScalarSplitTotals : kScalarList));
    }
    if (early_refine) {
      WP_HIP(hipEventRecord(c->evs[kEvRoundDone], st2));
      if (n_text > 0) {
        WP_HIP(hipStreamWaitEvent(st2, c->evs[kEvSorted], 0));
        launch_anchors(st2);
      }
      WP_HIP(hipStreamWaitEvent(st, c->evs[kEvRoundDone], 0));
      if (n_act > 0) {
        if (n_act >= (1u << 22)) {
          hipLaunchKernelGGL(list_rank_base_kernel, dim3(cdiv(n_act, kBlock)), dim3(kBlock), 0, st, hd, AG, d_gfirst, d_ghead, n_act);
          store_ranks(spare_vals, hd, reinterpret_cast<uint32_t *>(hd) + list_cap + 2, reinterpret_cast<uint32_t *>(skeys), n_act);
        } else {
          hipLaunchKernelGGL(scatter_list_ranks_kernel, dim3(cdiv(n_act, kBlock)), dim3(kBlock), 0, st, spare_vals, hd, AG, d_gfirst,
                             d_ghead, n_act, d_rank, n);
        }
        rounds = 2;
      }
      WP_LAUNCH_CHECK();
      return;
    }
    join();
    if (n_act > 0) {
      store_ranks(spare_vals, hd, reinterpret_cast<uint32_t *>(hd) + list_cap + 2, reinterpret_cast<uint32_t *>(skeys), n_act);
      rounds = 2;
    }
    WP_LAUNCH_CHECK();
  }

  void next_round_begin(size_t upper, int rb) {
    queue_scalars(c, kScalarAnchorGap, st);
    WP_HIP(hipEventRecord(c->evs[kEvScalars], st));
    fork();
    if (upper > 0) {
      hipLaunchKernelGGL(local_sort_kernel, dim3(cdiv(upper, kLsT)), dim3(kBlock), 0, st, avals, AG, adep, c->d_scalars + kScalarList, d_ghead,
                         d_rank, n, rb, LK0, spare_vals, static_cast<const uint32_t *>(nullptr));
    }
    WP_HIP(hipEventSynchronize(c->evs[kEvScalars]));
    n_act = c->h_scalars[kScalarListEntries];
    n_large_groups = classified ? c->h_scalars[kScalarListLargeGroups] : 0;
    n_large = classified ? c->h_scalars[kScalarListLargeEntries] : 0;
    if (c->h_scalars[kScalarListWanted] > list_cap) throw ListOverflow{c->h_scalars[kScalarListWanted]};
  }

  void refine() {
    if (!use_trie) doubling_rounds();
    S.rounds = rounds;
    const int max_len = code.uniform_bits ? code.uniform_bits : kMaxCodeLen + code.lo_bits;
    const int32_t key_syms = std::max(1, kKeyBits / max_len);
    S.sorted_depth = full ? 0x7fffffff
                          : (prune ? std::min<int32_t>(static_cast<int32_t>(need_depth), key_syms) : static_cast<int32_t>(need_depth));
    S.needed_after_round0 = prune ? (rounds > 1 ? S.active_per_round[1] : 0) : -1;
    if (prune && rounds > 1) c->list_hint = static_cast<size_t>(S.active_per_round[1]);
  }

  void doubling_rounds() {
    const int rb = bit_length(n);
    const DepthRule rule{need_depth, full ? 1 : 0, nullptr, nullptr, 0, nullptr};
    next_round_begin(std::min(n, list_cap), rb);
    S.active_per_round[0] = static_cast<int64_t>(n);
    refine_stats(c->h_scalars[kScalarListGroups], rb);
    uint32_t *gneed_cur = d_gneed0, *gneed_nxt = d_gneed1;
    const bool group_need = prune && M > 0;
    while (n_act > 0) {
      DepthRule rrule = rule;
      if (group_need) {
        rrule.gneed_in = gneed_cur;
        rrule.gneed_out = gneed_nxt;
        std::swap(gneed_cur, gneed_nxt);
      }
      if (static_cast<uint64_t>(rounds) > 80 + (full ? 0ull : static_cast<uint64_t>(need_depth))) {
        throw HipError("prefix doubling did not converge (internal error)");
      }
      if (rounds < 40) S.active_per_round[rounds] = static_cast<int64_t>(n_act);
      uint64_t *skeys = LK0, *kfree = LK1;
      uint32_t *svals = spare_vals, *nvals = avals;
      if (n_large > 0) {
        const int lgb = bit_length(n_large_groups > 0 ? n_large_groups - 1 : 0);
        hipLaunchKernelGGL(large_extract_kernel, dim3(cdiv(cdiv(n_large, kLxSpan), kBlock / kWave)), dim3(kBlock), 0, st2, avals, adep,
                           d_lg_head, d_lg_off, static_cast<uint32_t>(n_large_groups), n_large, d_rank, n, rb, LK1, LV0, LPOS,
                           static_cast<const uint32_t *>(nullptr));
        const int lc = radix_sort_pairs<uint64_t>(LK1, LV0, LK2, LV1, n_large, 0, rb + lgb, d_radix_tmp, radix_words, st2, nullptr);
        hipLaunchKernelGGL(large_writeback_kernel, dim3(std::min<size_t>(cdiv(n_large, kBlock), 8192)), dim3(kBlock), 0, st2,
                           lc ? LK2 : LK1, lc ? LV1 : LV0, LPOS, n_large, AG, rb, skeys, svals);
        join();
      }
      const unsigned tiles = cdiv(n_act, kRrTile);
      RankEntry *hd = reinterpret_cast<RankEntry *>(kfree);
      hipLaunchKernelGGL(HIP_KERNEL_NAME(rerank_agg_kernel<false>), dim3(tiles), dim3(kBlock), 0, st, skeys, svals, n_act, adep,
                         d_rank, d_gdepth, n, dcode.first_len, dcode.uniform_bits, rrule, d_tdep, d_agg);
      hipLaunchKernelGGL(rerank_chunk_kernel, dim3(cdiv(tiles, kRrChunk)), dim3(kBlock), 0, st, d_agg, tiles, d_chunk_agg);
      hipLaunchKernelGGL(rerank_prefix_kernel, dim3(cdiv(tiles, kRrChunk)), dim3(kBlock), 0, st, d_agg, d_chunk_agg, tiles);
      hipLaunchKernelGGL(HIP_KERNEL_NAME(rerank_apply_kernel<SymT, false>), dim3(tiles), dim3(kBlock), 0, st, skeys, svals, slots,
                         adep, d_tdep, n_act, d_agg, d_sym, n, dcode.first_len, dcode.uniform_bits, rrule, d_sa, hd, d_lcp,
                         other_slots, nvals, AG, other_dep, d_ghead, d_gdepth, c->d_scalars + kScalarList);
      fork();
      store_ranks(svals, hd, reinterpret_cast<uint32_t *>(hd) + list_cap + 2, reinterpret_cast<uint32_t *>(skeys), n_act);
      WP_LAUNCH_CHECK();
      rounds++;
      classified = classify_groups(n_act);
      join();
      std::swap(slots, other_slots);
      std::swap(adep, other_dep);
      avals = nvals;
      spare_vals = svals;
      next_round_begin(n_act, rb);
    }
  }

  void scanlines() {
    if (n_text > 0) fork();
    MarkView mv{};
    const int pack_steps = (hv.longest < kStepMaxLen && hv.tokens.size() < (size_t(1) << kStepIdBits)) ? 1 : 0;
    const size_t vocab_base = n_text + 1;
    uint32_t *mslot = d_mslot0, *midx = d_midx0;
    if (text_only) {
      if (M > 0) {
        if (early_refine) {
          hipLaunchKernelGGL(trie_token_range_list_kernel, dim3(cdiv(M, kBlock)), dim3(kBlock), 0, st, d_node_of_slot, c->d_elig_node,
                             c->d_elig_subtree, M, d_rng_lo, d_rng_hi, d_rng_long, d_tok_group, d_ghead);
        } else {
          hipLaunchKernelGGL(trie_token_range_kernel, dim3(cdiv(M, kBlock)), dim3(kBlock), 0, st, d_node_of_slot, c->d_elig_node,
                             c->d_elig_subtree, M, d_rng_lo, d_rng_hi, d_rng_long);
        }
        hipLaunchKernelGGL(virtual_marks_kernel, dim3(cdiv(M, kBlock)), dim3(kBlock), 0, st, d_rng_lo, d_rng_hi, M, c->d_elig_id,
                           c->d_elig_info, d_mslot0, d_mid, d_minfo, d_rf, d_rb);
      }
      mv = MarkView{mslot, d_mid, d_minfo, d_rf, d_rb, M, d_cover_f, d_cover_b};
    } else {
      if (M > 0) {
        hipLaunchKernelGGL(mark_slots_kernel, dim3(cdiv(M, kBlock)), dim3(kBlock), 0, st, c->d_elig_start, M, vocab_base, d_rank,
                           d_mslot0, d_midx0);
        int mc = radix_sort_pairs<uint32_t>(d_mslot0, d_midx0, d_mslot1, d_midx1, M, 0, bit_length(n), d_radix_tmp, radix_words, st,
                                            nullptr);
        mslot = mc ? d_mslot1 : d_mslot0;
        midx = mc ? d_midx1 : d_midx0;
        hipLaunchKernelGGL(mark_gather_kernel, dim3(cdiv(M, kBlock)), dim3(kBlock), 0, st, midx, M, c->d_elig_id, c->d_elig_info,
                           d_mid, d_minfo);
      }
      hipLaunchKernelGGL(tile_mlo_kernel, dim3(cdiv(sl_tiles + 1, kBlock)), dim3(kBlock), 0, st, mslot, M, n, sl_tiles, d_tile_mlo);
      hipLaunchKernelGGL(sl_summary_kernel, dim3(sl_tiles), dim3(kBlock), 0, st, d_lcp, n, mslot, d_minfo, d_tile_mlo, d_tmin_f,
                         d_tmin_b, d_rf, d_rb);
      hipLaunchKernelGGL(sl_group_min_kernel, dim3(cdiv(static_cast<size_t>(sl_groups) * kWave, kBlock)), dim3(kBlock), 0, st,
                         d_tmin_f, d_tmin_b, sl_tiles, sl_groups, d_gmin_f, d_gmin_b);
      mv = MarkView{mslot, d_mid, d_minfo, d_rf, d_rb, M, d_cover_f, d_cover_b};
      if (M > 0) {
        hipLaunchKernelGGL(sl_reach_global_kernel, dim3(cdiv(static_cast<size_t>(M) * kWave, kBlock)), dim3(kBlock), 0, st, d_lcp, n,
                           sl_tiles, sl_groups, mslot, d_minfo, M, d_tmin_f, d_tmin_b, d_gmin_f, d_gmin_b, d_rf, d_rb);
      }
    }
    if (M > 0) {
      hipLaunchKernelGGL(mark_cover_kernel, dim3(4), dim3(kCoverThreads), 0, st, d_minfo, d_rf, d_rb, M, d_cover_f, d_cover_b);
    }
    if (n_text > 0 && !anchors_queued) launch_anchors(st2);
    hipLaunchKernelGGL(piece_starts_kernel, dim3(cdiv(std::max(M, 1), kBlock)), dim3(kBlock), 0, st, mv, n_sorted, d_ps0);
    const int P = this->P + (key_lookup ? 2 * static_cast<int>(n_groups) : 0);
    const int pc = radix_sort_pairs<uint32_t>(d_ps0, d_pv0, d_ps1, d_pv1, P, 0, bit_length(n), d_radix_tmp, radix_words, st, nullptr);
    nbuckets = static_cast<unsigned>(((n_sorted - 1) >> bucket_shift) + 1);
    nbuckets_all = static_cast<unsigned>(((n_sorted - 1) >> bucket_shift_all) + 1);
    uint32_t *pstart = pc ? d_ps1 : d_ps0;
    hipLaunchKernelGGL(piece_values_kernel, dim3(cdiv(static_cast<size_t>(P) * kWave, kBlock)), dim3(kBlock), 0, st, mv, pstart, P,
                       d_pval_p, d_pval_s, pack_steps);
    hipLaunchKernelGGL(piece_bucket_kernel, dim3(cdiv(nbuckets + 1, kBlock)), dim3(kBlock), 0, st, pstart, P, bucket_shift, nbuckets,
                       d_bidx);
    hipLaunchKernelGGL(piece_bucket_fast_kernel, dim3(cdiv(nbuckets, kBlock)), dim3(kBlock), 0, st, d_bidx, d_pval_p, d_pval_s, nbuckets,
                       d_bfast);
    WP_LAUNCH_CHECK();
    steps = StepTable{pstart, d_pval_p, d_pval_s, d_bidx, bucket_shift, pack_steps, d_bfast};
    steps_all = steps;
    if (bucket_shift_all != bucket_shift) {
      hipLaunchKernelGGL(piece_bucket_kernel, dim3(cdiv(nbuckets_all + 1, kBlock)), dim3(kBlock), 0, st, pstart, P, bucket_shift_all,
                         nbuckets_all, d_bidx_all);
      hipLaunchKernelGGL(piece_bucket_fast_kernel, dim3(cdiv(nbuckets_all, kBlock)), dim3(kBlock), 0, st, d_bidx_all, d_pval_p, d_pval_s,
                         nbuckets_all, d_bfast_all);
      WP_LAUNCH_CHECK();
      steps_all = StepTable{pstart, d_pval_p, d_pval_s, d_bidx_all, bucket_shift_all, pack_steps, d_bfast_all};
    }
    if (key_lookup) key_steps(pstart, P, pack_steps);
    S.step.n_marks = M;
    S.step.n_steps = P;
    S.step.n_tiles = sl_tiles;
    S.step.n_groups_of_tiles = sl_groups;
    S.step.bucket_shift = bucket_shift;
    S.step.bucket_shift_all = bucket_shift_all;
    S.step.key_shift = key_shift;
    S.step.key_shift_all = key_shift_all;
    S.step.packed = pack_steps;
    S.step.key_lookup = key_lookup ? 1 : 0;
  }

  void key_steps(const uint32_t *pstart, int P, int pack_steps) {
    const uint32_t *skeys = reinterpret_cast<const uint32_t *>(keys);
    hipLaunchKernelGGL(key_steps_kernel, dim3(cdiv(P, kBlock)), dim3(kBlock), 0, st, pstart, d_pval_p, d_pval_s, P, skeys, d_kstart,
                       d_kval_p, d_kval_s);
    if (n_groups > 0) {
      hipLaunchKernelGGL(key_steps_needed_kernel, dim3(cdiv(n_groups, kBlock)), dim3(kBlock), 0, st, d_gfirst, d_gend,
                         static_cast<uint32_t>(n_groups), pstart, P, d_kval_p, d_kval_s);
    }
#ifdef WP_DEBUG_BOUNDS
    hipLaunchKernelGGL(key_steps_check_kernel, dim3(cdiv(P, kBlock)), dim3(kBlock), 0, st, pstart, P, skeys, d_kval_p, d_kval_s);
#endif
    hipLaunchKernelGGL(piece_bucket_kernel, dim3(cdiv(nkbuckets + 1, kBlock)), dim3(kBlock), 0, st, d_kstart, P, key_shift, nkbuckets,
                       d_kbidx);
    hipLaunchKernelGGL(piece_bucket_fast_kernel, dim3(cdiv(nkbuckets, kBlock)), dim3(kBlock), 0, st, d_kbidx, d_kval_p, d_kval_s,
                       nkbuckets, d_kbfast);
    ksteps = StepTable{d_kstart, d_kval_p, d_kval_s, d_kbidx, key_shift, pack_steps, d_kbfast};
    ksteps_all = ksteps;
    if (key_shift_all != key_shift) {
      hipLaunchKernelGGL(piece_bucket_kernel, dim3(cdiv(nkbuckets_all + 1, kBlock)), dim3(kBlock), 0, st, d_kstart, P, key_shift_all,
                         nkbuckets_all, d_kbidx_all);
      hipLaunchKernelGGL(piece_bucket_fast_kernel, dim3(cdiv(nkbuckets_all, kBlock)), dim3(kBlock), 0, st, d_kbidx_all, d_kval_p,
                         d_kval_s, nkbuckets_all, d_kbfast_all);
      ksteps_all = StepTable{d_kstart, d_kval_p, d_kval_s, d_kbidx_all, key_shift_all, pack_steps, d_kbfast_all};
    }
    WP_LAUNCH_CHECK();
  }

  void walk_long_words(const WalkArgs &wa, size_t n_anchors) {
    const uint32_t lw_cap = static_cast<uint32_t>(n_text / kMaxAnchorGap + 2);
    LongWord *d_lw = reinterpret_cast<LongWord *>(d_tile_scratch);
    uint32_t *d_lw_off = d_tile_scratch + 2 * static_cast<size_t>(lw_cap);
    uint32_t *d_lw_fail = d_lw_off + lw_cap + 1;
    hipLaunchKernelGGL(long_word_collect_kernel, dim3(std::min<size_t>(cdiv(std::max<size_t>(n_anchors, 1), kBlock), 2048)),
                       dim3(kBlock), 0, st, d_anchors, c->d_scalars + kScalarAnchors, n_text, d_cls, d_lw, lw_cap, c->d_scalars + kScalarLongWords);
    WP_LAUNCH_CHECK();
    fetch_scalars(c, kScalarLongWords);
    const uint32_t nw = std::min(c->h_scalars[kScalarLongWords], lw_cap);
    if (nw == 0) return;
    S.walk.n_long_words = static_cast<int64_t>(nw);
    std::vector<LongWord> h_lw(nw);
    WP_HIP(hipMemcpyAsync(h_lw.data(), d_lw, sizeof(LongWord) * nw, hipMemcpyDeviceToHost, st));
    WP_HIP(hipStreamSynchronize(st));
    std::vector<uint32_t> h_off(nw + 1);
    uint64_t total64 = 0;
    uint32_t longest = 0;
    for (uint32_t i = 0; i < nw; i++) {
      h_off[i] = static_cast<uint32_t>(total64);
      total64 += h_lw[i].end - h_lw[i].begin;
      longest = std::max(longest, h_lw[i].end - h_lw[i].begin);
    }
    h_off[nw] = static_cast<uint32_t>(total64);
    const uint32_t total = static_cast<uint32_t>(total64);
    WP_HIP(hipMemcpyAsync(d_lw_off, h_off.data(), sizeof(uint32_t) * (nw + 1), hipMemcpyHostToDevice, st));
    WP_HIP(hipMemsetAsync(d_lw_fail, 0, sizeof(uint32_t) * nw, st));
    int32_t *d_lid = reinterpret_cast<int32_t *>(VA);
    uint32_t *jump_a = X1, *jump_b = X0;
    uint8_t *d_mark = reinterpret_cast<uint8_t *>(KB);
    const dim3 grid(cdiv(total, kBlock));
    WalkArgs wa_all = wa;
    wa_all.steps = steps_all;
    wa_all.ksteps = ksteps_all;
    hipLaunchKernelGGL(long_word_next_kernel, grid, dim3(kBlock), 0, st, wa_all, d_lw, d_lw_off, nw, total, d_lid, jump_a, d_mark);
    WP_HIP(hipStreamSynchronize(st));
    for (uint32_t reach = 1; reach < longest; reach *= 2) {
      hipLaunchKernelGGL(long_word_mark_kernel, grid, dim3(kBlock), 0, st, jump_a, total, d_mark);
      hipLaunchKernelGGL(long_word_double_kernel, grid, dim3(kBlock), 0, st, jump_a, total, jump_b);
      std::swap(jump_a, jump_b);
    }
    hipLaunchKernelGGL(long_word_mark_kernel, grid, dim3(kBlock), 0, st, jump_a, total, d_mark);
    hipLaunchKernelGGL(long_word_fail_kernel, grid, dim3(kBlock), 0, st, d_lid, d_mark, d_lw_off, nw, total, d_lw_fail);
    if (offs_unit >= 0) {
      uint32_t *d_lw_end = d_lw_fail + lw_cap;
      WP_HIP(hipMemsetAsync(d_lw_end, 0xff, sizeof(uint32_t) * nw, st));
      hipLaunchKernelGGL(long_word_end_kernel, grid, dim3(kBlock), 0, st, d_lw, d_lw_off, nw, total, d_lid, d_lw_end);
      hipLaunchKernelGGL(HIP_KERNEL_NAME(long_word_emit_kernel<true>), grid, dim3(kBlock), 0, st, wa, d_lw, d_lw_off, nw, total, d_lid,
                         d_mark, d_lw_fail, d_ospill, static_cast<const uint32_t *>(d_lw_end));
    } else {
      hipLaunchKernelGGL(HIP_KERNEL_NAME(long_word_emit_kernel<false>), grid, dim3(kBlock), 0, st, wa, d_lw, d_lw_off, nw, total, d_lid,
                         d_mark, d_lw_fail, static_cast<uint2 *>(nullptr), static_cast<const uint32_t *>(nullptr));
    }
    WP_LAUNCH_CHECK();
    S.anchor_mode = 2;
  }

  size_t cover_anchors(WalkArgs &wa) {
    uint32_t *d_reach = VA, *d_reach_tiles = d_tile_scratch;
    uint8_t *d_aflags = reinterpret_cast<uint8_t *>(X1);
    const unsigned rtiles = cdiv(n_text, kReachTile), atiles = cdiv(n_text, kAnchorTile);
    uint32_t *d_wp_tiles = d_reach_tiles + rtiles + 1;
    uint32_t *d_ns_tiles = d_wp_tiles + rtiles + 1;
    uint32_t *d_gap_a = d_ns_tiles + rtiles + 1, *d_gap_b = d_gap_a + rtiles + 1;
    hipLaunchKernelGGL(gap_tiles_kernel, dim3(cdiv(rtiles, kBlock)), dim3(kBlock), 0, st, d_anchors, c->d_scalars + kScalarAnchors, n_text, rtiles,
                       v->cover_anchors ? 1 : 0, d_gap_a, d_gap_b);
    hipLaunchKernelGGL(reach_kernel, dim3(rtiles), dim3(kBlock), 0, st, wa, d_reach, d_reach_tiles, d_gap_a, d_gap_b);
    hipLaunchKernelGGL(reach_spine_kernel, dim3(1), dim3(1024), 0, st, d_reach_tiles, static_cast<size_t>(rtiles));
    WP_HIP(hipMemsetAsync(d_anchor_cnt, 0, sizeof(uint32_t) * atiles, st));
    hipLaunchKernelGGL(cover_flags_kernel, dim3(rtiles), dim3(kBlock), 0, st, d_cls, d_reach, d_reach_tiles, n_text, d_aflags,
                       d_wp_tiles, d_ns_tiles, d_gap_a, d_gap_b, d_anchor_cnt);
    hipLaunchKernelGGL(suffix_min_kernel, dim3(2), dim3(1024), 0, st, d_wp_tiles, d_ns_tiles, static_cast<size_t>(rtiles));
    device_exclusive_scan(d_anchor_cnt, d_anchor_cnt, atiles, d_anchor_tmp, c->d_scalars + kScalarAnchors, st);
    hipLaunchKernelGGL(anchor_write_kernel, dim3(atiles), dim3(kBlock), 0, st, d_cls, d_aflags, n_text, d_anchor_cnt, d_anchors);
    WP_LAUNCH_CHECK();
    fetch_scalars(c, kScalarAnchors);
    wa.aflags = d_aflags;
    wa.wp_from_tile = d_wp_tiles;
    wa.ns_from_tile = d_ns_tiles;
    S.anchor_mode = 1;
    return c->h_scalars[kScalarAnchors];
  }

  WalkArgs walk_args() const {
    return WalkArgs{d_cls, n_text, d_rank, steps, c->d_tok_len, hv.unk_id, d_emit, nullptr, nullptr, nullptr,
                    hv.soft.empty() ? 1 : 0, static_cast<int32_t>(hv.tokens.size()),
                    key_lookup ? reinterpret_cast<const uint32_t *>(KA) : nullptr, ksteps, drop_blanks ? 1 : 0};
  }

  void step_views() {
    if (!d_step_views || n_text == 0) return;
    hipLaunchKernelGGL(step_views_kernel, dim3(cdiv(n_text, kBlock)), dim3(kBlock), 0, st, walk_args(), d_step_views);
    WP_LAUNCH_CHECK();
  }

  int32_t *walk(size_t *n_ids_out) {
    int32_t *d_ids = reinterpret_cast<int32_t *>(VB);
    *n_ids_out = 0;
    if (n_text == 0) return d_ids;
    WalkArgs wa = walk_args();
    S.anchor_mode = 0;
    join();
    fetch_scalars(c, kScalarAnchorGap);
    size_t n_anchors = c->h_scalars[kScalarAnchors];
    const size_t max_anchor_gap = c->h_scalars[kScalarAnchorGap];
    S.walk.max_anchor_gap = static_cast<int32_t>(max_anchor_gap);
    const bool all_hard = hv.soft.empty();
    bool staged = staged_possible && max_anchor_gap <= kMaxAnchorGap;
    if (staged_possible && !staged) WP_HIP(hipMemsetAsync(d_emit, 0x80, n_text * sizeof(int32_t), st));
    if (!v->cover_anchors && all_hard && max_anchor_gap > kMaxAnchorGap) {
      walk_long_words(wa, n_anchors);
    } else if (v->cover_anchors || max_anchor_gap > kMaxAnchorGap) {
      n_anchors = cover_anchors(wa);
      staged = !sparse_emit;
    }
    S.n_anchors = static_cast<int64_t>(n_anchors);
    const size_t acap = std::max<size_t>(n_anchors, 1);
    const bool offs = offs_unit >= 0;
    if (staged) {
      int32_t *d_ctmp = reinterpret_cast<int32_t *>(X0);
      const unsigned sblocks = cdiv(acap, static_cast<size_t>(kWbWords));
      if (S.anchor_mode == 0 && all_hard && max_anchor_gap > kWideMin) {
        uint32_t *d_wide_list = reinterpret_cast<uint32_t *>(KB), *d_wide_cnt = VA;
        wide_ran = true;
        clear_scalars(c, kScalarWideWords, kScalarWideWords, st);
        hipLaunchKernelGGL(wide_collect_kernel, dim3(std::min<size_t>(cdiv(acap, kBlock), 2048)), dim3(kBlock), 0, st, d_anchors,
                           c->d_scalars + kScalarAnchors, n_text, d_wide_list, c->d_scalars + kScalarWideWords);
        WalkArgs wa_all = wa;
        wa_all.steps = steps_all;
        wa_all.ksteps = ksteps_all;
        const dim3 wgrid(std::min<size_t>(cdiv(acap, kBlock / kWave), 8192));
        if (offs) {
          hipLaunchKernelGGL(HIP_KERNEL_NAME(walk_wide_kernel<true>), wgrid, dim3(kBlock), 0, st, wa_all, d_anchors, c->d_scalars + kScalarAnchors,
                             d_wide_list, c->d_scalars + kScalarWideWords, d_wide_cnt, d_ospill);
          hipLaunchKernelGGL(HIP_KERNEL_NAME(walk_lean_kernel<true, true>), dim3(sblocks), dim3(kBlock), 0, st, wa, d_anchors,
                             c->d_scalars + kScalarAnchors, acap, d_ctmp, d_blk_cnt, d_wide_cnt, d_ospill, d_cspan);
        } else {
          hipLaunchKernelGGL(HIP_KERNEL_NAME(walk_wide_kernel<false>), wgrid, dim3(kBlock), 0, st, wa_all, d_anchors, c->d_scalars + kScalarAnchors,
                             d_wide_list, c->d_scalars + kScalarWideWords, d_wide_cnt, static_cast<uint2 *>(nullptr));
          hipLaunchKernelGGL(HIP_KERNEL_NAME(walk_lean_kernel<true, false>), dim3(sblocks), dim3(kBlock), 0, st, wa, d_anchors,
                             c->d_scalars + kScalarAnchors, acap, d_ctmp, d_blk_cnt, d_wide_cnt, static_cast<uint2 *>(nullptr),
                             static_cast<uint2 *>(nullptr));
        }
      } else if (offs) {
        hipLaunchKernelGGL(HIP_KERNEL_NAME(walk_lean_kernel<false, true>), dim3(sblocks), dim3(kBlock), 0, st, wa, d_anchors,
                           c->d_scalars + kScalarAnchors, acap, d_ctmp, d_blk_cnt, static_cast<const uint32_t *>(nullptr), d_ospill, d_cspan);
      } else {
        hipLaunchKernelGGL(HIP_KERNEL_NAME(walk_lean_kernel<false, false>), dim3(sblocks), dim3(kBlock), 0, st, wa, d_anchors,
                           c->d_scalars + kScalarAnchors, acap, d_ctmp, d_blk_cnt, static_cast<const uint32_t *>(nullptr),
                           static_cast<uint2 *>(nullptr), static_cast<uint2 *>(nullptr));
      }
      device_exclusive_scan(d_blk_cnt, d_blk_off, sblocks, d_emit_tmp, c->d_scalars + kScalarIds, st);
      if (offs) {
        hipLaunchKernelGGL(HIP_KERNEL_NAME(emit_gather_kernel<true>), dim3(sblocks), dim3(kBlock), 0, st, d_anchors, c->d_scalars + kScalarAnchors,
                           acap, d_ctmp, d_blk_cnt, d_blk_off, d_ids, kWbWords, static_cast<const uint2 *>(d_cspan), d_offs);
      } else {
        hipLaunchKernelGGL(HIP_KERNEL_NAME(emit_gather_kernel<false>), dim3(sblocks), dim3(kBlock), 0, st, d_anchors, c->d_scalars + kScalarAnchors,
                           acap, d_ctmp, d_blk_cnt, d_blk_off, d_ids, kWbWords, static_cast<const uint2 *>(nullptr),
                           static_cast<uint2 *>(nullptr));
      }
    } else {
      if (offs) {
        hipLaunchKernelGGL(HIP_KERNEL_NAME(walk_kernel<true>), dim3(cdiv(acap, kBlock)), dim3(kBlock), 0, st, wa, d_anchors,
                           c->d_scalars + kScalarAnchors, acap, d_ospill);
      } else {
        hipLaunchKernelGGL(HIP_KERNEL_NAME(walk_kernel<false>), dim3(cdiv(acap, kBlock)), dim3(kBlock), 0, st, wa, d_anchors,
                           c->d_scalars + kScalarAnchors, acap, static_cast<uint2 *>(nullptr));
      }
      const unsigned tiles = cdiv(n_text, kScanTile);
      hipLaunchKernelGGL(emit_count_kernel, dim3(tiles), dim3(kBlock), 0, st, d_emit, n_text, d_emit_cnt);
      device_exclusive_scan(d_emit_cnt, d_emit_cnt, tiles, d_emit_tmp, c->d_scalars + kScalarIds, st);
      if (offs) {
        hipLaunchKernelGGL(HIP_KERNEL_NAME(emit_write_kernel<true>), dim3(tiles), dim3(kBlock), 0, st, d_emit, n_text, d_emit_cnt, d_ids,
                           static_cast<const uint2 *>(d_ospill), d_offs);
      } else {
        hipLaunchKernelGGL(HIP_KERNEL_NAME(emit_write_kernel<false>), dim3(tiles), dim3(kBlock), 0, st, d_emit, n_text, d_emit_cnt, d_ids,
                           static_cast<const uint2 *>(nullptr), static_cast<uint2 *>(nullptr));
      }
    }
    S.staged_emit = staged ? 1 : 0;
    S.walk.lean = staged ? 1 : 0;
    WP_LAUNCH_CHECK();
    return d_ids;
  }

  void row_structure(size_t n_ids) {
    const size_t n_rows = rows->n_rows;
    const long long *d_starts = rows->d_doc_off;
    if (!d_starts) {
      if (nmap) hipLaunchKernelGGL(norm_fill_starts_kernel, dim3(cdiv(n_rows + 1, kBlock)), dim3(kBlock), 0, st, d_line_starts, n_rows + 1, static_cast<long long>(nbytes));
      hipLaunchKernelGGL(line_write_kernel, dim3(cdiv(nbytes, kLineTile)), dim3(kBlock), 0, st, d_text, nbytes,
                         static_cast<const uint32_t *>(rows->d_line_cnt), n_rows, d_line_starts);
      d_starts = d_line_starts;
    }
    if (n_ids > 0) {
      hipLaunchKernelGGL(cp_byte_kernel, dim3(cdiv(nbytes, kDecTile)), dim3(kBlock), 0, st, d_text, nbytes, d_tile_prefix, n_text,
                         d_byte_of);
      if (nmap && rows->d_doc_off) {
        hipLaunchKernelGGL(norm_doc_starts_kernel, dim3(cdiv(n_rows + 1, kBlock)), dim3(kBlock), 0, st, rows->d_doc_off, n_rows, *nmap,
                           static_cast<const uint32_t *>(d_byte_of), nbytes, d_line_starts);
        d_starts = d_line_starts;
      }
      hipLaunchKernelGGL(row_splits_kernel, dim3(cdiv(n_rows + 1, kBlock)), dim3(kBlock), 0, st, d_starts, n_rows,
                         static_cast<const uint32_t *>(d_byte_of), n_text, static_cast<const uint2 *>(d_offs), n_ids, rows->unit,
                         d_row_splits, d_row_base);
      if (nmap && d_row_base) {
        hipLaunchKernelGGL(norm_row_base_kernel, dim3(cdiv(n_rows + 1, kBlock)), dim3(kBlock), 0, st, d_starts, n_rows,
                           static_cast<const uint32_t *>(d_byte_of), n_text, *nmap, rows->unit, d_row_base);
      }
    } else {
      WP_HIP(hipMemsetAsync(d_row_splits, 0, (n_rows + 1) * sizeof(long long), st));
    }
    WP_LAUNCH_CHECK();
    rows->d_starts = d_starts;
    rows->d_row_splits = d_row_splits;
  }

  void finish(int32_t *d_ids, size_t *n_ids_out) {
    c->d_offs = nullptr;
    if (offs_unit >= 0 && n_text > 0) {
      fetch_scalars(c, kScalarIds);
      const size_t n_ids = c->h_scalars[kScalarIds];
      if (rows) row_structure(n_ids);
      if (nmap) {
        if (n_ids > 0 && (!rows || rows->unit >= 0)) {
          hipLaunchKernelGGL(span_source_kernel, dim3(cdiv(n_ids, kBlock)), dim3(kBlock), 0, st, d_offs, n_ids, *nmap, offs_unit);
          WP_LAUNCH_CHECK();
        }
      } else if (offs_unit == WP_OFFSETS_BYTES && n_ids > 0) {
        if (!rows) {
          hipLaunchKernelGGL(cp_byte_kernel, dim3(cdiv(nbytes, kDecTile)), dim3(kBlock), 0, st, d_text, nbytes, d_tile_prefix, n_text,
                             d_byte_of);
        }
        hipLaunchKernelGGL(span_bytes_kernel, dim3(cdiv(n_ids, kBlock)), dim3(kBlock), 0, st, d_offs, n_ids,
                           static_cast<const uint32_t *>(d_byte_of), d_text, n_text);
        WP_LAUNCH_CHECK();
      }
      if (rows && rows->unit >= 0 && n_ids > 0) {
        hipLaunchKernelGGL(rebase_kernel, dim3(cdiv(n_ids, kRebaseTile)), dim3(kBlock), 0, st, d_offs, n_ids,
                           static_cast<const long long *>(d_row_splits), rows->n_rows, static_cast<const uint32_t *>(d_row_base));
        WP_LAUNCH_CHECK();
      }
      c->d_offs = reinterpret_cast<const uint32_t *>(d_offs);
    } else if (rows) {
      row_structure(0);
    }
    if (ar.guard) {
      static const uint32_t init[2] = {0u, 0xffffffffu};
      WP_HIP(hipMemcpyAsync(c->d_scalars + kScalarGuard, init, sizeof(init), hipMemcpyHostToDevice, st));
      ar.check(st, c->d_scalars + kScalarGuard);
      aa.check(st, c->d_scalars + kScalarGuard);
      fetch_scalars(c, kScalarGuardFirst);
      if (c->h_scalars[kScalarGuardBad] != 0) {
        throw HipError("arena guard: " + std::to_string(c->h_scalars[kScalarGuardBad]) + " guard zone(s) overwritten, first behind allocation #" +
                       std::to_string(c->h_scalars[kScalarGuardFirst] - 1));
      }
      S.guard_zones = static_cast<int32_t>(ar.zones.size() + aa.zones.size());
    }
#ifdef WP_DEBUG_BOUNDS
    {
      unsigned int oob[kBoundSites] = {};
      WP_HIP(hipStreamSynchronize(st));
      take_oob(0, kBoundSites, oob);
      if (oob[0] | oob[1] | oob[2] | oob[3] | oob[4] | oob[5] | oob[6] | oob[7] | oob[8]) {
        throw HipError("debug bounds: out-of-range addresses skipped: radix scatter " + std::to_string(oob[0]) + ", rank store " +
                       std::to_string(oob[1]) + ", token id " + std::to_string(oob[2]) + ", list slot " + std::to_string(oob[3]) +
                       "; key-space step starts inside a run of equal keys " + std::to_string(oob[4]) +
                       "; candidate runs unlike their group " + std::to_string(oob[5]) + "; offsets " + std::to_string(oob[6]) +
                       "; step values used at blanks " + std::to_string(oob[7]) +
                       "; round-0 sorted array: descents, blank keys left, multiset unlike the kept keys " + std::to_string(oob[8]));
      }
      S.reserved0 = 1;
    }
#endif
    fetch_scalars(c, kScalarSplitTotals);
    const size_t n_ids = n_text > 0 ? c->h_scalars[kScalarIds] : 0;
    S.n_ids = static_cast<int64_t>(n_ids);
    S.walk.n_wide_words = wide_ran ? static_cast<int64_t>(c->h_scalars[kScalarWideWords]) : 0;
    S.radix_passes = c->rstats.passes;
    S.radix_pass_elems = c->rstats.elems;
    S.radix_digit_bytes = c->rstats.digit_bytes;
    S.radix_pass_bytes = c->rstats.bytes;
    S.arena_bytes = static_cast<int64_t>(c->a_buf.cap + c->b_buf.cap);
    if (v->stage_timing) {
      auto span = [&](int a, int b) {
        float ms = 0;
        WP_HIP(hipEventElapsedTime(&ms, c->ev[a], c->ev[b]));
        return static_cast<double>(ms);
      };
      S.ms_decode = span(kMarkStart, kMarkSymbols);
      S.ms_sa = span(kMarkSymbols, kMarkSorted);
      S.ms_lcp = span(kMarkSorted, kMarkLcp);
      S.ms_scan = span(kMarkLcp, kMarkScanned);
      S.ms_walk = span(kMarkScanned, kMarkWalked);
      S.ms_total = span(kMarkStart, kMarkWalked) + S.ms_normalize;
      S.ms_radix_scatter = c->rstats.spans.resolve();
      S.sched.ms_sort_to_scan = span(kMarkRound0, kMarkLcp);
    }
    c->d_ids = d_ids;
    c->dbg.sym = d_sym;
    c->dbg.sym_bytes = sizeof(SymT);
    c->dbg.sa = d_sa;
    c->dbg.rank = d_rank;
    c->dbg.lcp = d_lcp;
    c->dbg.steps = steps;
    c->dbg.best_scratch = d_dbg_best;
    c->dbg.step_views = n_text > 0 ? d_step_views : nullptr;
    c->dbg.cps = d_cps;
    c->dbg.cls = v->keep_debug ? d_cls : nullptr;
    c->dbg.n = n;
    c->dbg.n_text = n_text;
    *n_ids_out = n_ids;
  }

  void run(size_t *n_ids_out) {
    plan();
    symbols_and_keys();
    if (v->stage_timing) WP_HIP(hipEventRecord(c->ev[kMarkSymbols], st));
    sort_round0();
    if (v->stage_timing) WP_HIP(hipEventRecord(c->ev[kMarkRound0], st));
    ranks_round0();
    refine();
    if (v->stage_timing) WP_HIP(hipEventRecord(c->ev[kMarkSorted], st));
    if (v->lcp_kasai) {
      const size_t chunk = 64;
      hipLaunchKernelGGL(HIP_KERNEL_NAME(kasai_kernel<SymT>), dim3(cdiv(cdiv(n, chunk), kBlock)), dim3(kBlock), 0, st, d_sym, d_sa,
                         d_rank, n, chunk, d_lcp);
      WP_LAUNCH_CHECK();
    }
    if (v->stage_timing) WP_HIP(hipEventRecord(c->ev[kMarkLcp], st));
    scanlines();
    if (v->stage_timing) WP_HIP(hipEventRecord(c->ev[kMarkScanned], st));
    if (v->keep_step_views) step_views();
    size_t n_ids = 0;
    int32_t *d_ids = walk(&n_ids);
    if (v->stage_timing) WP_HIP(hipEventRecord(c->ev[kMarkWalked], st));
    finish(d_ids, n_ids_out);
  }
};

static void encode_on_device(const wp_vocab *v, Context *c, const uint8_t *d_text, size_t nbytes, size_t *n_ids_out,
                             EncodeStats &S, int offs_unit = -1, RowsCall *rows = nullptr) {
  hipStream_t st = c->stream;
  const HostVocab &hv = v->hv;
  std::memset(&S, 0, sizeof(S));
  S.offsets_unit = -1;
  S.n_rows = -1;
  S.rows_route = -1;
  S.n_bytes = static_cast<int64_t>(nbytes);
  S.longest_token = hv.longest;
  c->d_ids = nullptr;
  c->d_offs = nullptr;
  c->dbg = {};
  *n_ids_out = 0;
  if (nbytes == 0) return;
  const bool guard = v->arena_guard || EnvOptions::get().arena_guard;
  S.offsets_unit = offs_unit;
  c->d_offs = nullptr;

  const uint8_t *src_text = d_text;
  const size_t src_bytes = nbytes;
  NormResult norm;
  const NormMap *nmap = nullptr;
  if (v->normalize != 0) {
    normalize_on_device(c, d_text, nbytes, v->normalize, offs_unit >= 0, v->stage_timing, norm);
    S.normalize = v->normalize;
    S.norm_bytes = static_cast<int64_t>(norm.nbytes);
    S.ms_normalize = norm.ms;
    if (norm.nbytes == 0) {
      if (!rows) return;
      WP_HIP(hipMemsetAsync(c->norm_buf.p, 0x20, 1, st));
      norm.nbytes = 1;
    }
    d_text = norm.text;
    nbytes = norm.nbytes;
    if (offs_unit >= 0) nmap = &norm.map;
  }

  c->rstats.passes = 0;
  c->rstats.elems = 0;
  c->rstats.digit_bytes = 0;
  c->rstats.bytes = 0;
  c->rstats.spans.on = v->stage_timing;
  c->rstats.spans.used = 0;
  if (v->stage_timing) WP_HIP(hipEventRecord(c->ev[kMarkStart], st));

  const unsigned dec_tiles = cdiv(nbytes, kDecTile);
  Arena aa(&c->a_buf, guard);
  uint32_t *d_tile_cnt = nullptr, *d_cnt_tmp = nullptr, *d_cps = nullptr;
  uint8_t *d_cls = nullptr;
  const unsigned line_tiles = cdiv(nbytes, kLineTile), src_line_tiles = cdiv(src_bytes, kLineTile);
  uint32_t *d_line_tmp = nullptr, *d_src_line_cnt = nullptr;
  for (int pass = 0; pass < 2; pass++) {
    d_tile_cnt = aa.take<uint32_t>(dec_tiles + 1);
    d_cnt_tmp = aa.take<uint32_t>(cdiv(dec_tiles, kScanTile) + 8);
    d_cps = v->keep_debug ? aa.take<uint32_t>(nbytes + 1) : nullptr;
    d_cls = aa.take<uint8_t>(nbytes + 32);
    if (rows && !rows->d_doc_off) {
      rows->d_line_cnt = aa.take<uint32_t>(line_tiles + 1);
      d_line_tmp = aa.take<uint32_t>(cdiv(line_tiles, kScanTile) + 8);
      if (v->normalize != 0) d_src_line_cnt = aa.take<uint32_t>(src_line_tiles + 1 + cdiv(src_line_tiles, kScanTile) + 8);
    }
    if (pass == 0) aa.commit();
  }
  aa.arm(st);
  WP_HIP(hipMemsetAsync(c->d_scalars, 0, sizeof(uint32_t) * kScalars, st));
  WP_HIP(hipMemsetAsync(c->d_used, 0, sizeof(uint32_t) * kCpWords, st));
  hipLaunchKernelGGL(decode_count_kernel<true>, dim3(dec_tiles), dim3(kBlock), 0, st, d_text, nbytes, d_tile_cnt,
                     reinterpret_cast<unsigned long long *>(c->d_scalars + kScalarInvalid), c->d_used);
  device_exclusive_scan(d_tile_cnt, d_tile_cnt, dec_tiles, d_cnt_tmp, c->d_scalars + kScalarCps, st, nullptr,
                        reinterpret_cast<unsigned long long *>(c->d_scalars + kScalarCps64));
  WP_HIP(hipMemcpyAsync(c->d_scalars + kScalarAlphaWord0, c->d_used, sizeof(uint32_t), hipMemcpyDeviceToDevice, st));
  hipLaunchKernelGGL(vocab_alphabet_kernel, dim3(cdiv(hv.used_word_idx.size(), kBlock)), dim3(kBlock), 0, st,
                     c->d_vocab_word_idx, c->d_vocab_word_bits, static_cast<uint32_t>(hv.used_word_idx.size()), c->d_used);
  hipLaunchKernelGGL(alphabet_prefix_kernel, dim3(1), dim3(kAlphaThreads), 0, st, c->d_used, c->d_scan_tmp, c->d_scalars + kScalarAlphabet);
  hipLaunchKernelGGL(alphabet_lut_kernel, dim3(kCpTableSize / kBlock), dim3(kBlock), 0, st, c->d_used, c->d_scan_tmp, c->d_lut);
  if (rows) {
    if (rows->d_doc_off) {
      hipLaunchKernelGGL(rows_check_kernel, dim3(cdiv(rows->n_docs + 1, kBlock)), dim3(kBlock), 0, st, src_text, src_bytes, rows->d_doc_off,
                         rows->n_docs, c->d_scalars + kScalarRowsBad);
    } else {
      if (v->normalize != 0) {
        hipLaunchKernelGGL(line_count_kernel, dim3(src_line_tiles), dim3(kBlock), 0, st, src_text, src_bytes, d_src_line_cnt);
        device_exclusive_scan(d_src_line_cnt, d_src_line_cnt, src_line_tiles, d_src_line_cnt + src_line_tiles + 1,
                              c->d_scalars + kScalarSrcRows, st);
      }
      hipLaunchKernelGGL(line_count_kernel, dim3(line_tiles), dim3(kBlock), 0, st, d_text, nbytes, rows->d_line_cnt);
      device_exclusive_scan(rows->d_line_cnt, rows->d_line_cnt, line_tiles, d_line_tmp, c->d_scalars + kScalarRows, st);
    }
  }
  WP_LAUNCH_CHECK();
  fetch_scalars(c, rows ? (v->normalize != 0 ? kScalarSrcRows : kScalarRowsCut) : kScalarRows);
  if (rows) {
    if (rows->d_doc_off && c->h_scalars[kScalarRowsBad] != 0) {
      throw std::invalid_argument("document offsets: " + std::to_string(c->h_scalars[kScalarRowsBad]) +
                                  " boundaries are not increasing from 0 to nbytes with a '\\n' in front of each");
    }
    rows->n_rows = rows->d_doc_off ? rows->n_docs : c->h_scalars[v->normalize != 0 ? kScalarSrcRows : kScalarRows];
    if (rows->n_rows > rows->capacity) throw std::invalid_argument("capacity_rows is smaller than the number of rows");
    S.n_rows = static_cast<int64_t>(rows->n_rows);
    S.rows_route = 1;
  }
  unsigned long long n_text64;
  std::memcpy(&n_text64, c->h_scalars + kScalarCps64, sizeof(n_text64));
  if (n_text64 + 1 + hv.stream.size() > 2000000000ull) throw std::length_error("64bit not implemented");
  const size_t n_text = c->h_scalars[kScalarCps];
  const bool full_sa = v->full_depth || hv.n_dup_eligible > 0 || v->lcp_kasai;
  const bool text_only = !full_sa && !v->vocab_in_s && !EnvOptions::get().vocab_in_s && !hv.low_cp && (c->h_scalars[kScalarAlphaWord0] & 3u) == 0;
  S.vocab_in_s = text_only ? 0 : 1;
  const uint32_t sigma = c->h_scalars[kScalarAlphabet];
  unsigned long long dropped;
  std::memcpy(&dropped, c->h_scalars + kScalarInvalid, sizeof(dropped));
  if (dropped != 0) std::cerr << "WARNING Input contains invalid unicode characters." << std::endl;

  const size_t n = n_text + 1 + (text_only ? 0 : hv.stream.size());
  S.n_text = static_cast<int64_t>(n_text);
  S.n_total = static_cast<int64_t>(n);
  S.alphabet = sigma;
  if (n > 2000000000ull) throw std::length_error("64bit not implemented");
  if (v->stage_timing) WP_HIP(hipEventRecord(c->ev[kMarkCounted], st));

  const int bits = std::max(1, bit_length(sigma));
  for (int attempt = 0;; attempt++) {
    Arena ab(&c->b_buf, guard);
    try {
      if (sigma <= 255) {
        LinearPath<uint8_t>(v, c, S, ab, aa, d_text, nbytes, d_tile_cnt, n_text, n, d_cps, d_cls, bits, text_only,
                                 offs_unit, rows, nmap).run(n_ids_out);
      } else {
        LinearPath<uint32_t>(v, c, S, ab, aa, d_text, nbytes, d_tile_cnt, n_text, n, d_cps, d_cls, bits, text_only,
                                 offs_unit, rows, nmap).run(n_ids_out);
      }
      S.list_retries = attempt;
      return;
    } catch (const ListOverflow &o) {
      if (attempt >= 2) throw HipError("needed list overflow after a retry (internal error)");
      WP_HIP(hipStreamSynchronize(c->stream));
      WP_HIP(hipStreamSynchronize(c->stream2));
      c->list_hint = o.wanted;
      c->rstats.passes = 0;
      c->rstats.elems = 0;
      c->rstats.digit_bytes = 0;
      c->rstats.bytes = 0;
      c->rstats.spans.used = 0;
      clear_scalars(c, kScalarListEntries, kScalarWideWords, st);
    }
  }
}

}
```

wordpiece_amd/csrc/scanline.h:

```cpp
#pragma once
#include "primitives.h"
#include "suffix_array.h"

namespace wp {

constexpr int kSlItems = 16;
constexpr int kSlTile = kBlock * kSlItems;
constexpr int32_t kLcpInf = 0x7fffffff;
constexpr uint32_t kMarkLenMask = 0x0fffffffu;
#ifndef WP_STEP_BUCKET_BITS
#define WP_STEP_BUCKET_BITS 18
#endif
constexpr int kStepBucketBits = WP_STEP_BUCKET_BITS;
#ifndef WP_STEP_BUCKET_BITS_MAX
#define WP_STEP_BUCKET_BITS_MAX 21
#endif
constexpr int kStepBucketBitsMax = WP_STEP_BUCKET_BITS_MAX;
constexpr int kStepIdBits = 20;
constexpr int kStepMaxLen = 1 << 11;
constexpr uint32_t kMarkSurvBwd = 1u << 28;
constexpr uint32_t kMarkSurvFwd = 1u << 29;
constexpr int kMarkClsShift = 30;

__device__ __forceinline__ int32_t boundary_lcp(const int32_t *__restrict__ lcp, size_t n, long long x) {
  if (x < 0 || static_cast<size_t>(x) + 1 >= n) return kLcpInf;
  const int32_t v = lcp[x];
  return v < 0 ? kLcpInf : v;
}

__global__ __launch_bounds__(kBlock) void mark_slots_kernel(const uint32_t *__restrict__ tok_start, int M,
                                                            size_t vocab_base, const RankEntry *__restrict__ rank,
                                                            uint32_t *__restrict__ slot, uint32_t *__restrict__ idx) {
  int m = blockIdx.x * kBlock + threadIdx.x;
  if (m >= M) return;
  slot[m] = rank_of(rank[vocab_base + tok_start[m]]);
  idx[m] = static_cast<uint32_t>(m);
}

__global__ __launch_bounds__(kBlock) void mark_gather_kernel(const uint32_t *__restrict__ order, int M,
                                                             const int32_t *__restrict__ tok_id,
                                                             const uint32_t *__restrict__ tok_info,
                                                             int32_t *__restrict__ mid, uint32_t *__restrict__ minfo) {
  int m = blockIdx.x * kBlock + threadIdx.x;
  if (m >= M) return;
  mid[m] = tok_id[order[m]];
  minfo[m] = tok_info[order[m]];
}

__global__ __launch_bounds__(kBlock) void tile_mlo_kernel(const uint32_t *__restrict__ mslot, int M, size_t n,
                                                          unsigned ntiles, uint32_t *__restrict__ tile_mlo) {
  unsigned t = blockIdx.x * kBlock + threadIdx.x;
  if (t > ntiles) return;
  const size_t s = static_cast<size_t>(t) * kSlTile;
  int lo = 0, hi = M;
  while (lo < hi) {
    int mid = (lo + hi) >> 1;
    if (mslot[mid] < s) lo = mid + 1; else hi = mid;
  }
  tile_mlo[t] = (t == ntiles || s >= n) ? M : lo;
}

__global__ __launch_bounds__(kBlock) void sl_summary_kernel(const int32_t *__restrict__ lcp, size_t n,
                                                            const uint32_t *__restrict__ mslot,
                                                            uint32_t *__restrict__ minfo,
                                                            const uint32_t *__restrict__ tile_mlo,
                                                            int32_t *__restrict__ tmin_f, int32_t *__restrict__ tmin_b,
                                                            int32_t *__restrict__ reach_fwd,
                                                            int32_t *__restrict__ reach_bwd) {
  __shared__ int32_t bl[kSlTile + 1];
  __shared__ int32_t smin[8];
  const size_t s = static_cast<size_t>(blockIdx.x) * kSlTile;
  const int cnt = static_cast<int>(min(static_cast<size_t>(kSlTile), n - s));
  int32_t mf = kLcpInf, mb = kLcpInf;
  for (int q = threadIdx.x; q <= cnt; q += kBlock) {
    const int32_t v = boundary_lcp(lcp, n, static_cast<long long>(s) - 1 + q);
    bl[q] = v;
    if (q <= cnt - 1) mf = min(mf, v);
    if (q >= 1) mb = min(mb, v);
  }
  mf = block_reduce_min(mf, smin);
  mb = block_reduce_min(mb, smin);
  if (threadIdx.x == 0) {
    tmin_f[blockIdx.x] = mf;
    tmin_b[blockIdx.x] = mb;
  }

  const int lane = lane_id(), w = wave_id();
  const uint32_t lo = tile_mlo[blockIdx.x], hi = tile_mlo[blockIdx.x + 1];
  for (uint32_t m = lo + w; m < hi; m += kBlock / kWave) {
    const int i = static_cast<int>(mslot[m] - s);
    const uint32_t info = minfo[m];
    const int32_t len = static_cast<int32_t>(info & kMarkLenMask);
    int jf = cnt;
    for (int start = i + 1; start < cnt; start += kWave) {
      const int j = start + lane;
      const uint64_t b = __ballot(j < cnt && bl[j] < len);
      if (b) {
        jf = start + __ffsll(static_cast<long long>(b)) - 1;
        break;
      }
    }
    int jb = -1;
    for (int top = i - 1; top >= 0; top -= kWave) {
      const int j = top - lane;
      const uint64_t b = __ballot(j >= 0 && bl[j + 1] < len);
      if (b) {
        jb = top - (__ffsll(static_cast<long long>(b)) - 1);
        break;
      }
    }
    if (lane == 0) {
      reach_fwd[m] = static_cast<int32_t>(s + jf);
      reach_bwd[m] = static_cast<int32_t>(static_cast<long long>(s) + jb);
      minfo[m] = (info & ~(kMarkSurvFwd | kMarkSurvBwd)) | (jf == cnt ? kMarkSurvFwd : 0u)
                 | (jb == -1 ? kMarkSurvBwd : 0u);
    }
  }
}

constexpr int kSlGroup = 64;
__global__ __launch_bounds__(kBlock) void sl_group_min_kernel(const int32_t *__restrict__ tmin_f,
                                                              const int32_t *__restrict__ tmin_b, unsigned ntiles,
                                                              unsigned ngroups, int32_t *__restrict__ gmin_f,
                                                              int32_t *__restrict__ gmin_b) {
  const unsigned g = (blockIdx.x * kBlock + threadIdx.x) >> 6;
  const int lane = lane_id();
  if (g >= ngroups) return;
  const unsigned t = g * kSlGroup + lane;
  int32_t f = t < ntiles ? tmin_f[t] : kLcpInf, b = t < ntiles ? tmin_b[t] : kLcpInf;
  f = wave_reduce_min(f);
  b = wave_reduce_min(b);
  if (lane == 0) {
    gmin_f[g] = f;
    gmin_b[g] = b;
  }
}

__global__ __launch_bounds__(kBlock) void sl_reach_global_kernel(
    const int32_t *__restrict__ lcp, size_t n, unsigned ntiles, unsigned ngroups, const uint32_t *__restrict__ mslot,
    const uint32_t *__restrict__ minfo, int M, const int32_t *__restrict__ tmin_f, const int32_t *__restrict__ tmin_b,
    const int32_t *__restrict__ gmin_f, const int32_t *__restrict__ gmin_b, int32_t *__restrict__ reach_fwd,
    int32_t *__restrict__ reach_bwd) {
  const int m = static_cast<int>((static_cast<size_t>(blockIdx.x) * kBlock + threadIdx.x) >> 6);
  const int lane = lane_id();
  if (m >= M) return;
  const uint32_t info = minfo[m];
  const int32_t len = static_cast<int32_t>(info & kMarkLenMask);
  const unsigned t0 = mslot[m] / kSlTile;
  if (info & kMarkSurvFwd) {
    long long stop = -1;
    const unsigned g0 = t0 / kSlGroup;
    {
      const unsigned t = g0 * kSlGroup + lane;
      const uint64_t b = __ballot(t > t0 && t < ntiles && tmin_f[t] < len);
      if (b) stop = g0 * kSlGroup + __ffsll(static_cast<long long>(b)) - 1;
    }
    if (stop < 0) {
      for (unsigned gb = g0 + 1; gb < ngroups && stop < 0; gb += kWave) {
        const unsigned g = gb + lane;
        const uint64_t b = __ballot(g < ngroups && gmin_f[g] < len);
        if (b) {
          const unsigned gs = gb + __ffsll(static_cast<long long>(b)) - 1;
          const unsigned t = gs * kSlGroup + lane;
          const uint64_t b2 = __ballot(t < ntiles && tmin_f[t] < len);
          stop = gs * kSlGroup + __ffsll(static_cast<long long>(b2)) - 1;
        }
      }
    }
    long long r = static_cast<long long>(n);
    if (stop >= 0) {
      const size_t s = static_cast<size_t>(stop) * kSlTile;
      const size_t e = min(n, s + kSlTile);
      for (size_t j0 = s; j0 < e; j0 += kWave) {
        const size_t j = j0 + lane;
        const uint64_t b = __ballot(j < e && boundary_lcp(lcp, n, static_cast<long long>(j) - 1) < len);
        if (b) {
          r = static_cast<long long>(j0) + __ffsll(static_cast<long long>(b)) - 1;
          break;
        }
      }
    }
    if (lane == 0) reach_fwd[m] = static_cast<int32_t>(r);
  }
  if (info & kMarkSurvBwd) {
    long long stop = -1;
    const unsigned g0 = t0 / kSlGroup;
    {
      const unsigned t = g0 * kSlGroup + lane;
      const uint64_t b = __ballot(t < t0 && tmin_b[t] < len);
      if (b) stop = g0 * kSlGroup + (63 - __clzll(static_cast<long long>(b)));
    }
    if (stop < 0) {
      for (long long gb = static_cast<long long>(g0) - 1; gb >= 0 && stop < 0; gb -= kWave) {
        const long long g = gb - lane;
        const uint64_t b = __ballot(g >= 0 && gmin_b[g] < len);
        if (b) {
          const long long gs = gb - (__ffsll(static_cast<long long>(b)) - 1);
          const unsigned t = static_cast<unsigned>(gs) * kSlGroup + lane;
          const uint64_t b2 = __ballot(t < ntiles && tmin_b[t] < len);
          stop = gs * kSlGroup + (63 - __clzll(static_cast<long long>(b2)));
        }
      }
    }
    long long r = -1;
    if (stop >= 0) {
      const long long s = stop * kSlTile;
      const long long e = static_cast<long long>(min(n, static_cast<size_t>(s) + kSlTile));
      for (long long top = e - 1; top >= s; top -= kWave) {
        const long long j = top - lane;
        const uint64_t b = __ballot(j >= s && boundary_lcp(lcp, n, j) < len);
        if (b) {
          r = top - (__ffsll(static_cast<long long>(b)) - 1);
          break;
        }
      }
    }
    if (lane == 0) reach_bwd[m] = static_cast<int32_t>(r);
  }
}

struct MarkView {
  const uint32_t *mslot;
  const int32_t *mid;
  const uint32_t *minfo;
  const int32_t *reach_fwd, *reach_bwd;
  int M;
  const int32_t *cover_f, *cover_b;
};

constexpr int kCoverThreads = 1024;
constexpr int kCoverItems = 8;
__global__ __launch_bounds__(kCoverThreads) void mark_cover_kernel(const uint32_t *__restrict__ minfo,
                                                                   const int32_t *__restrict__ reach_fwd,
                                                                   const int32_t *__restrict__ reach_bwd, int M,
                                                                   int32_t *__restrict__ cover_f,
                                                                   int32_t *__restrict__ cover_b) {
  constexpr int WAVES = kCoverThreads / kWave;
  __shared__ int32_t wm[WAVES];
  const int tid = threadIdx.x, lane = tid & 63, w = tid >> 6;
  const int c = blockIdx.x >> 1, back = blockIdx.x & 1;
  constexpr int32_t kNone = -2147483647 - 1;
  int32_t carry = kNone;
  for (int base = 0; base < M; base += kCoverThreads * kCoverItems) {
    int32_t v[kCoverItems], mx = kNone;
    uint32_t info[kCoverItems];
    int32_t rv[kCoverItems];
    const int32_t *__restrict__ reach = back ? reach_bwd : reach_fwd;
#pragma unroll
    for (int j = 0; j < kCoverItems; j++) {
      const int i = base + tid * kCoverItems + j;
      const int q = i < M ? (back ? M - 1 - i : i) : 0;
      info[j] = minfo[q];
      rv[j] = reach[q];
    }
#pragma unroll
    for (int j = 0; j < kCoverItems; j++) {
      const int i = base + tid * kCoverItems + j;
      v[j] = kNone;
      if (i < M && static_cast<int>(info[j] >> kMarkClsShift) == c) v[j] = back ? -rv[j] - 1 : rv[j];
      mx = max(mx, v[j]);
      v[j] = mx;
    }
    const int32_t inc = wave_incl_max(mx);
    if (lane == kWave - 1) wm[w] = inc;
    __syncthreads();
    int32_t before = carry, all = carry;
#pragma unroll
    for (int q = 0; q < WAVES; q++) {
      if (q < w) before = max(before, wm[q]);
      all = max(all, wm[q]);
    }
    const int32_t up = __shfl_up(inc, 1, kWave);
    if (lane > 0) before = max(before, up);
#pragma unroll
    for (int j = 0; j < kCoverItems; j++) {
      const int i = base + tid * kCoverItems + j;
      if (i < M) {
        const int q = back ? M - 1 - i : i;
        const int32_t r = max(before, v[j]);
        if (back) cover_b[static_cast<size_t>(c) * M + q] = r == kNone ? 2147483647 : -(r + 1);
        else cover_f[static_cast<size_t>(c) * M + q] = r;
      }
    }
    carry = all;
    __syncthreads();
  }
}

constexpr int kStepsPerMark = 4;
__global__ __launch_bounds__(kBlock) void piece_starts_kernel(MarkView mv, size_t n, uint32_t *__restrict__ pstart) {
  const int m = blockIdx.x * kBlock + threadIdx.x;
  if (m == 0) pstart[kStepsPerMark * static_cast<size_t>(mv.M)] = 0;
  if (m >= mv.M) return;
  const uint32_t last = static_cast<uint32_t>(n - 1);
  uint32_t *o = pstart + kStepsPerMark * static_cast<size_t>(m);
  o[0] = min(static_cast<uint32_t>(mv.reach_bwd[m] + 1), last);
  o[1] = min(mv.mslot[m], last);
  o[2] = min(mv.mslot[m] + 1u, last);
  o[3] = min(static_cast<uint32_t>(mv.reach_fwd[m]), last);
}

__global__ __launch_bounds__(kBlock) void piece_values_kernel(MarkView mv, const uint32_t *__restrict__ pstart,
                                                              int P, int32_t *__restrict__ pval_prefix,
                                                              int32_t *__restrict__ pval_suffix, int packed) {
  const int k = static_cast<int>((static_cast<size_t>(blockIdx.x) * kBlock + threadIdx.x) >> 6);
  const int lane = lane_id();
  if (k >= P) return;
  const uint32_t slot = pstart[k];
  int lo = 0, hi = mv.M;
  while (hi - lo > 64) {
    const int st = (hi - lo) / kWave + 1;
    const int idx = lo + lane * st;
    const bool gt = idx < hi ? mv.mslot[idx] > slot : true;
    const uint64_t m = __ballot(gt);
    if (!m) {
      lo += (kWave - 1) * st + 1;
      continue;
    }
    const int t = __ffsll(static_cast<long long>(m)) - 1;
    const int first_gt = lo + t * st;
    if (t) lo += (t - 1) * st + 1;
    hi = first_gt < hi ? first_gt : hi;
    if (!t) hi = lo;
  }
  while (lo < hi) {
    const int md = (lo + hi) >> 1;
    if (mv.mslot[md] <= slot) lo = md + 1; else hi = md;
  }
  const int ub = lo;
  int xq[2] = {-1, -1}, yq[2] = {-1, -1};
  bool fdone[2] = {false, false}, bdone[2] = {false, false};
  for (int top = ub - 1; top >= 0; top -= kWave) {
#pragma unroll
    for (int c = 0; c < 2; c++) {
      if (xq[c] >= 0 || mv.cover_f[static_cast<size_t>(c) * mv.M + top] <= static_cast<int32_t>(slot)) fdone[c] = true;
    }
    if (fdone[0] && fdone[1]) break;
    const int q = top - lane;
    bool cover = false;
    int cls = 0;
    if (q >= 0) {
      const uint32_t info = mv.minfo[q];
      cls = static_cast<int>(info >> kMarkClsShift);
      cover = mv.reach_fwd[q] > static_cast<int32_t>(slot);
    }
#pragma unroll
    for (int c = 0; c < 2; c++) {
      const uint64_t b = __ballot(cover && cls == c);
      if (xq[c] < 0 && b) xq[c] = top - (__ffsll(static_cast<long long>(b)) - 1);
    }
  }
  int lb = ub;
  if (ub > 0 && mv.mslot[ub - 1] == slot) lb = ub - 1;
  for (int base = lb; base < mv.M; base += kWave) {
#pragma unroll
    for (int c = 0; c < 2; c++) {
      if (yq[c] >= 0 || mv.cover_b[static_cast<size_t>(c) * mv.M + base] >= static_cast<int32_t>(slot)) bdone[c] = true;
    }
    if (bdone[0] && bdone[1]) break;
    const int q = base + lane;
    bool cover = false;
    int cls = 0;
    if (q < mv.M) {
      const uint32_t info = mv.minfo[q];
      cls = static_cast<int>(info >> kMarkClsShift);
      cover = mv.reach_bwd[q] < static_cast<int32_t>(slot);
    }
#pragma unroll
    for (int c = 0; c < 2; c++) {
      const uint64_t b = __ballot(cover && cls == c);
      if (yq[c] < 0 && b) yq[c] = base + __ffsll(static_cast<long long>(b)) - 1;
    }
  }
  if (lane < 2) {
    const int c = lane;
    const int x = c ? xq[1] : xq[0], y = c ? yq[1] : yq[0];
    int wq = -1;
    if (x >= 0 && y >= 0) {
      const int32_t xl = static_cast<int32_t>(mv.minfo[x] & kMarkLenMask), yl = static_cast<int32_t>(mv.minfo[y] & kMarkLenMask);
      wq = xl > yl ? x : y;
    } else if (x >= 0) {
      wq = x;
    } else if (y >= 0) {
      wq = y;
    }
    int32_t r = wq >= 0 ? mv.mid[wq] : -1;
    if (packed && r >= 0) r |= static_cast<int32_t>(mv.minfo[wq] & kMarkLenMask) << kStepIdBits;
    (c ? pval_suffix : pval_prefix)[k] = r;
  }
}

__global__ __launch_bounds__(kBlock) void piece_bucket_kernel(const uint32_t *__restrict__ pstart, int P, int shift,
                                                              unsigned nbuckets, uint32_t *__restrict__ bidx) {
  const unsigned b = blockIdx.x * kBlock + threadIdx.x;
  if (b > nbuckets) return;
  const uint64_t key = static_cast<uint64_t>(b) << shift;
  int lo = 0, hi = P;
  while (lo < hi) {
    const int md = (lo + hi) >> 1;
    if (pstart[md] < key) lo = md + 1; else hi = md;
  }
  bidx[b] = static_cast<uint32_t>(lo);
}

constexpr int32_t kStepSlow = static_cast<int32_t>(0x80000000u);
constexpr int32_t kStepNeeded = -2;
__global__ __launch_bounds__(kBlock) void piece_bucket_fast_kernel(const uint32_t *__restrict__ bidx,
                                                                   const int32_t *__restrict__ pval_prefix,
                                                                   const int32_t *__restrict__ pval_suffix, unsigned nbuckets,
                                                                   int2 *__restrict__ bfast) {
  const unsigned b = blockIdx.x * kBlock + threadIdx.x;
  if (b >= nbuckets) return;
  const uint32_t lo = bidx[b], hi = bidx[b + 1];
  bfast[b] = lo == hi ? int2{pval_prefix[lo - 1], pval_suffix[lo - 1]}
                      : int2{kStepSlow | static_cast<int32_t>(hi - lo), static_cast<int32_t>(lo)};
}

struct StepTable {
  const uint32_t *pstart;
  const int32_t *pval_prefix, *pval_suffix;
  const uint32_t *bidx;
  int shift;
  int packed;
  const int2 *bfast;
};
__device__ __forceinline__ int32_t step_id(const StepTable &st, int32_t raw) {
  return (st.packed && raw >= 0) ? (raw & ((1 << kStepIdBits) - 1)) : raw;
}
__device__ __forceinline__ int32_t step_len(const StepTable &st, int32_t raw, const int32_t *__restrict__ tok_len) {
  return st.packed ? (raw >> kStepIdBits) : tok_len[raw];
}

__device__ __forceinline__ int step_lookup(const StepTable &st, uint32_t r) {
  const uint32_t b = r >> st.shift;
  int lo = static_cast<int>(st.bidx[b]), hi = static_cast<int>(st.bidx[b + 1]);
  while (lo < hi) {
    const int md = (lo + hi) >> 1;
    if (st.pstart[md] <= r) lo = md + 1; else hi = md;
  }
  return lo - 1;
}

__device__ __forceinline__ int32_t step_raw(const StepTable &st, uint32_t r, bool prefix) {
  const int2 e = st.bfast[r >> st.shift];
  if (e.x >= kStepNeeded) return prefix ? e.x : e.y;
  const int n = e.x & 0x7fffffff;
  int lo = e.y, hi = e.y + n;
  while (lo < hi) {
    const int md = (lo + hi) >> 1;
    if (st.pstart[md] <= r) lo = md + 1; else hi = md;
  }
  return prefix ? st.pval_prefix[lo - 1] : st.pval_suffix[lo - 1];
}


__global__ __launch_bounds__(kBlock) void group_starts_kernel(const uint32_t *__restrict__ gfirst,
                                                              const uint32_t *__restrict__ ghead,
                                                              const uint32_t *__restrict__ totals, size_t n,
                                                              uint32_t *__restrict__ pstart_tail, uint32_t *__restrict__ gend) {
  const uint32_t g = blockIdx.x * kBlock + threadIdx.x;
  if (g >= totals[1]) return;
  const uint32_t f = gfirst[g], e = f + (ghead[g + 1] - ghead[g]);
  const uint32_t last = static_cast<uint32_t>(n - 1);
  pstart_tail[2 * static_cast<size_t>(g)] = f;
  pstart_tail[2 * static_cast<size_t>(g) + 1] = min(e, last);
  gend[g] = e;
}

__global__ __launch_bounds__(kBlock) void key_steps_kernel(const uint32_t *__restrict__ pstart, const int32_t *__restrict__ pval_prefix,
                                                           const int32_t *__restrict__ pval_suffix, int P,
                                                           const uint32_t *__restrict__ sorted_keys, uint32_t *__restrict__ kstart,
                                                           int32_t *__restrict__ kval_prefix, int32_t *__restrict__ kval_suffix) {
  const int k = blockIdx.x * kBlock + threadIdx.x;
  if (k >= P) return;
  kstart[k] = k == 0 ? 0u : sorted_keys[pstart[k]];
  kval_prefix[k] = pval_prefix[k];
  kval_suffix[k] = pval_suffix[k];
}

__device__ __forceinline__ int starts_lower_bound(const uint32_t *__restrict__ pstart, int P, uint32_t x) {
  int lo = 0, hi = P;
  while (lo < hi) {
    const int md = (lo + hi) >> 1;
    if (pstart[md] < x) lo = md + 1; else hi = md;
  }
  return lo;
}

__global__ __launch_bounds__(kBlock) void key_steps_needed_kernel(const uint32_t *__restrict__ gfirst,
                                                                  const uint32_t *__restrict__ gend, uint32_t n_groups,
                                                                  const uint32_t *__restrict__ pstart, int P,
                                                                  int32_t *__restrict__ kval_prefix, int32_t *__restrict__ kval_suffix) {
  const uint32_t g = blockIdx.x * kBlock + threadIdx.x;
  if (g >= n_groups) return;
  const int k0 = starts_lower_bound(pstart, P, gfirst[g]), k1 = starts_lower_bound(pstart, P, gend[g]);
  for (int k = k0; k < k1; k++) {
    kval_prefix[k] = kStepNeeded;
    kval_suffix[k] = kStepNeeded;
  }
}

__global__ __launch_bounds__(kBlock) void key_steps_check_kernel(const uint32_t *__restrict__ pstart, int P,
                                                                 const uint32_t *__restrict__ sorted_keys,
                                                                 const int32_t *__restrict__ kval_prefix,
                                                                 const int32_t *__restrict__ kval_suffix) {
  const int k = blockIdx.x * kBlock + threadIdx.x;
  if (k == 0 || k >= P) return;
  const uint32_t s = pstart[k];
  if (s == 0 || kval_prefix[k] == kStepNeeded || sorted_keys[s - 1] != sorted_keys[s]) return;
  wp_in_bounds(kval_prefix[k] == kval_prefix[k - 1] && kval_suffix[k] == kval_suffix[k - 1], kSiteKeyStep);
}

__global__ __launch_bounds__(kBlock) void step_expand_kernel(StepTable st, size_t n, int32_t *__restrict__ best_prefix,
                                                             int32_t *__restrict__ best_suffix) {
  const size_t x = static_cast<size_t>(blockIdx.x) * kBlock + threadIdx.x;
  if (x >= n) return;
  const int k = step_lookup(st, static_cast<uint32_t>(x));
  best_prefix[x] = step_id(st, st.pval_prefix[k]);
  best_suffix[x] = step_id(st, st.pval_suffix[k]);
}

}
```

wordpiece_amd/csrc/trie.h:

```cpp
#pragma once
#include "decode.h"
#include "primitives.h"
#include "prune.h"

namespace wp {

struct TokenTrie {
  const uint32_t *chain_len;
  const uint32_t *chain_off;
  const uint32_t *child_begin;
  const uint32_t *child_node;
  const uint32_t *child_sym;
};

template <typename SymT>
__global__ __launch_bounds__(kBlock) void trie_map_symbols_kernel(const uint32_t *__restrict__ stream_cps, size_t n_stream,
                                                                  const uint32_t *__restrict__ child_cps, size_t n_child,
                                                                  const uint32_t *__restrict__ lut_excl,
                                                                  SymT *__restrict__ vsym, uint32_t *__restrict__ child_sym) {
  const size_t i = static_cast<size_t>(blockIdx.x) * kBlock + threadIdx.x;
  if (i < n_stream) vsym[i] = static_cast<SymT>(lut_excl[stream_cps[i]] + 1u);
  if (i < n_child) child_sym[i] = lut_excl[child_cps[i]] + 1u;
}

template <typename SymT>
__device__ __forceinline__ uint32_t trie_chain_match(const SymT *__restrict__ sym, size_t n, size_t pos,
                                                     const SymT *__restrict__ label, uint32_t len) {
  if (pos >= n) return 0u;
  const uint32_t lim = static_cast<uint32_t>(min(static_cast<size_t>(len), n - pos));
  uint32_t t = 0;
  if (sizeof(SymT) == 1) {
    const uint8_t *pa = reinterpret_cast<const uint8_t *>(sym) + pos, *pb = reinterpret_cast<const uint8_t *>(label);
    while (t < lim) {
      uint64_t wa, wb;
      __builtin_memcpy(&wa, pa + t, 8);
      __builtin_memcpy(&wb, pb + t, 8);
      const uint64_t x = wa ^ wb;
      if (x) {
        t += static_cast<uint32_t>(__ffsll(static_cast<long long>(x)) - 1) >> 3;
        break;
      }
      t += 8;
    }
    return min(t, lim);
  }
  while (t < lim && sym[pos + t] == label[t]) t++;
  return t;
}

template <typename SymT>
__device__ __forceinline__ uint32_t trie_descend(const TokenTrie &t, const SymT *__restrict__ sym, size_t n,
                                                 const SymT *__restrict__ vsym, uint32_t node, size_t pos, uint32_t limit,
                                                 uint32_t &left_out) {
  uint32_t left = limit ? limit : 0xffffffffu;
  for (;;) {
    const uint32_t len = t.chain_len[node];
    if (len) {
      const uint32_t want = min(len, left);
      const uint32_t l = trie_chain_match(sym, n, pos, vsym + t.chain_off[node], want);
      node += l;
      pos += l;
      left -= l;
      if (l < len) break;
    }
    if (left == 0) break;
    uint32_t lo = t.child_begin[node], hi = t.child_begin[node + 1];
    if (lo == hi || pos >= n) break;
    const uint32_t s = static_cast<uint32_t>(sym[pos]), end = hi;
    while (lo < hi) {
      const uint32_t md = (lo + hi) >> 1;
      if (t.child_sym[md] < s) lo = md + 1; else hi = md;
    }
    if (lo == end || t.child_sym[lo] != s) break;
    node = t.child_node[lo];
    pos++;
    left--;
  }
  left_out = limit ? left : 0u;
  return node;
}

template <typename SymT>
__global__ __launch_bounds__(kBlock) void trie_group_start_kernel(const uint32_t *__restrict__ sorted_vals,
                                                                  const uint32_t *__restrict__ cand_pos,
                                                                  const uint32_t *__restrict__ gcand,
                                                                  const uint32_t *__restrict__ gfirst,
                                                                  const uint32_t *__restrict__ gdepth,
                                                                  const uint32_t *__restrict__ sizes_dev,
                                                                  const SymT *__restrict__ sym, size_t n,
                                                                  const SymT *__restrict__ vsym, TokenTrie t,
                                                                  uint32_t *__restrict__ gnode, uint32_t *__restrict__ gdone) {
  const uint32_t g = blockIdx.x * kBlock + threadIdx.x;
  if (g >= sizes_dev[1]) return;
  const uint32_t d = gdepth[g];
  uint32_t left = 0, node = 0;
  if (d) {
    const uint32_t member = cand_pos ? cand_pos[gcand[g]] : sorted_vals[gfirst[g]];
    node = trie_descend(t, sym, n, vsym, 0u, static_cast<size_t>(member), d, left);
  }
  gnode[g] = node;
  gdone[g] = d - left;
}

template <typename SymT>
__global__ __launch_bounds__(kBlock) void trie_walk_kernel(const uint32_t *__restrict__ vals,
                                                           const uint32_t *__restrict__ gid,
                                                           const uint32_t *__restrict__ gnode,
                                                           const uint32_t *__restrict__ gdone,
                                                           const uint32_t *__restrict__ sizes_dev,
                                                           const SymT *__restrict__ sym, size_t n,
                                                           const SymT *__restrict__ vsym, TokenTrie t,
                                                           uint32_t *__restrict__ node_out) {
  const size_t m = sizes_dev[0];
  for (size_t p = static_cast<size_t>(blockIdx.x) * kBlock + threadIdx.x; p < m; p += static_cast<size_t>(gridDim.x) * kBlock) {
    const uint32_t g = gid[p];
    uint32_t unused;
    node_out[p] = trie_descend(t, sym, n, vsym, gnode[g], static_cast<size_t>(vals[p]) + gdone[g], 0u, unused);
  }
}


__global__ __launch_bounds__(kBlock) void trie_token_range_kernel(const uint32_t *__restrict__ node_of_slot,
                                                                  const uint32_t *__restrict__ tok_node,
                                                                  const uint32_t *__restrict__ tok_subtree, int M,
                                                                  uint32_t *__restrict__ rng_lo, uint32_t *__restrict__ rng_hi,
                                                                  const uint8_t *__restrict__ rng_long) {
  const int m = blockIdx.x * kBlock + threadIdx.x;
  if (m >= M || !rng_long[m]) return;
  const uint32_t glo = rng_lo[m], ghi = rng_hi[m];
  const uint32_t a = tok_node[m], b = a + tok_subtree[m];
  uint32_t lo = glo, hi = ghi;
  while (lo < hi) {
    const uint32_t md = lo + ((hi - lo) >> 1);
    if (node_of_slot[md] < a) lo = md + 1; else hi = md;
  }
  const uint32_t first = lo;
  hi = ghi;
  while (lo < hi) {
    const uint32_t md = lo + ((hi - lo) >> 1);
    if (node_of_slot[md] < b) lo = md + 1; else hi = md;
  }
  rng_lo[m] = first;
  rng_hi[m] = lo;
}

__global__ __launch_bounds__(kBlock) void trie_token_range_list_kernel(const uint32_t *__restrict__ node_of_entry,
                                                                       const uint32_t *__restrict__ tok_node,
                                                                       const uint32_t *__restrict__ tok_subtree, int M,
                                                                       uint32_t *__restrict__ rng_lo, uint32_t *__restrict__ rng_hi,
                                                                       const uint8_t *__restrict__ rng_long,
                                                                       const uint32_t *__restrict__ tok_group,
                                                                       const uint32_t *__restrict__ ghead) {
  const int m = blockIdx.x * kBlock + threadIdx.x;
  if (m >= M || !rng_long[m]) return;
  const uint32_t g = tok_group[m];
  if (g == kClaimNoGroup) return;
  const uint32_t base = rng_lo[m], glo = ghead[g], ghi = glo + (rng_hi[m] - base);
  const uint32_t a = tok_node[m], b = a + tok_subtree[m];
  uint32_t lo = glo, hi = ghi;
  while (lo < hi) {
    const uint32_t md = lo + ((hi - lo) >> 1);
    if (node_of_entry[md] < a) lo = md + 1; else hi = md;
  }
  const uint32_t first = lo;
  hi = ghi;
  while (lo < hi) {
    const uint32_t md = lo + ((hi - lo) >> 1);
    if (node_of_entry[md] < b) lo = md + 1; else hi = md;
  }
  rng_lo[m] = base + (first - glo);
  rng_hi[m] = base + (lo - glo);
}

}
```

Measured before the change: 31300.

## Fuse mark kernels and overlap step-table tail on a side stream

Merges the trie range refinement, virtual marks, group starts and piece starts into one token_marks kernel when early refine is on. The step-table tail (cover computation, bucket indexes, key steps) moves to a third stream with events, and the cover scan is split into chunked totals plus a per-chunk scan. Piece values now skip duplicate starts and use a wave ballot in place of a binary search, and the radix sort no longer carries a value array. The aim is fewer launches and more overlap in the serial tail, at the cost of extra cross-stream events and more complex synchronisation.

New measurement: 31990, median of 6. +2.2%, better.

```diff
diff --git a/wordpiece_amd/csrc/context.h b/wordpiece_amd/csrc/context.h
--- a/wordpiece_amd/csrc/context.h
+++ b/wordpiece_amd/csrc/context.h
@@ -209,7 +209,8 @@
 };
 
 enum SideEvent { kEvFork, kEvJoin, kEvScalars, kEvKeysFree, kEvPartition, kEvTrieNodes, kEvLargeSorted, kEvKeysBuilt, kEvCandCount,
-                 kEvSpine, kEvKept, kEvSorted, kEvListBuilt, kEvRoundDone, kSideEvents };
+                 kEvSpine, kEvKept, kEvSorted, kEvListBuilt, kEvRoundDone, kEvAnchorScalars,
+                 kEvMarks, kEvCovered, kEvStartsSorted, kEvTablesIndexed, kSideEvents };
 enum TimingMark { kMarkStart, kMarkCounted, kMarkSymbols, kMarkSorted, kMarkLcp, kMarkScanned, kMarkWalked, kMarkNormStart,
                   kMarkRound0, kTimingMarks, kMarkNormEnd = kMarkStart };
 
@@ -326,6 +327,9 @@
 #ifndef WP_LATE_REFINE_DEFAULT
 #define WP_LATE_REFINE_DEFAULT 0
 #endif
+#ifndef WP_SERIAL_TAIL
+#define WP_SERIAL_TAIL 0
+#endif
 
 struct wp_vocab {
   HostVocab hv;
@@ -529,6 +533,9 @@
   queue_scalars(c, last, c->stream);
   WP_HIP(hipStreamSynchronize(c->stream));
 }
+static void queue_scalar_slots(Context *c, int first, int last, hipStream_t st) {
+  WP_HIP(hipMemcpyAsync(c->h_scalars + first, c->d_scalars + first, sizeof(uint32_t) * (scalar_end(last) - first), hipMemcpyDeviceToHost, st));
+}
 static void clear_scalars(Context *c, int first, int last, hipStream_t st) {
   WP_HIP(hipMemsetAsync(c->d_scalars + first, 0, sizeof(uint32_t) * (scalar_end(last) - first), st));
 }
diff --git a/wordpiece_amd/csrc/linear_path.h b/wordpiece_amd/csrc/linear_path.h
--- a/wordpiece_amd/csrc/linear_path.h
+++ b/wordpiece_amd/csrc/linear_path.h
@@ -22,6 +22,46 @@
     totals[0] = 0;
     totals[1] = 0;
   }
+}
+
+__global__ __launch_bounds__(kBlock) void token_marks_kernel(const uint32_t *__restrict__ node_of_entry, const uint32_t *__restrict__ tok_node,
+                                                             const uint32_t *__restrict__ tok_subtree, int M, uint32_t *__restrict__ rng_lo,
+                                                             uint32_t *__restrict__ rng_hi, const uint8_t *__restrict__ rng_long,
+                                                             const uint32_t *__restrict__ tok_group, const uint32_t *__restrict__ ghead,
+                                                             const uint32_t *__restrict__ gfirst, const uint32_t *__restrict__ totals, size_t n,
+                                                             const int32_t *__restrict__ tok_id, const uint32_t *__restrict__ tok_info,
+                                                             uint32_t *__restrict__ mslot, int32_t *__restrict__ mid, uint32_t *__restrict__ minfo,
+                                                             int32_t *__restrict__ reach_fwd, int32_t *__restrict__ reach_bwd,
+                                                             uint32_t *__restrict__ pstart, uint32_t *__restrict__ gend) {
+  const int m = blockIdx.x * kBlock + threadIdx.x;
+  const uint32_t last = static_cast<uint32_t>(n - 1);
+  if (static_cast<uint32_t>(m) < totals[1]) {
+    const uint32_t f = gfirst[m], e = f + (ghead[m + 1] - ghead[m]);
+    uint32_t *tail = pstart + kStepsPerMark * static_cast<size_t>(M) + 1;
+    tail[2 * static_cast<size_t>(m)] = f;
+    tail[2 * static_cast<size_t>(m) + 1] = min(e, last);
+    gend[m] = e;
+  }
+  if (m == 0) pstart[kStepsPerMark * static_cast<size_t>(M)] = 0;
+  if (m >= M) return;
+  uint32_t lo = rng_lo[m], hi = rng_hi[m];
+  const uint32_t g = rng_long[m] ? tok_group[m] : kClaimNoGroup;
+  if (g != kClaimNoGroup) {
+    trie_token_range_in_list(node_of_entry, tok_node[m], tok_subtree[m], ghead[g], lo, hi);
+    rng_lo[m] = lo;
+    rng_hi[m] = hi;
+  }
+  const uint32_t reach = max(hi, lo);
+  mslot[m] = lo;
+  mid[m] = tok_id[m];
+  minfo[m] = tok_info[m];
+  reach_fwd[m] = static_cast<int32_t>(reach);
+  reach_bwd[m] = static_cast<int32_t>(lo);
+  uint32_t *o = pstart + kStepsPerMark * static_cast<size_t>(m);
+  o[0] = min(lo + 1u, last);
+  o[1] = min(lo, last);
+  o[2] = min(lo + 1u, last);
+  o[3] = min(reach, last);
 }
 
 constexpr double kBlankDropMinShare = 1.0 / 16;
@@ -97,6 +137,7 @@
   const NormMap *nmap;
 
   hipStream_t st, st2;
+  static constexpr bool kSerialTail = WP_SERIAL_TAIL != 0;
   const HostVocab &hv;
   bool full, prune, use_trie, key_lookup, keys_only, window_store, use_digit_bytes, staged_possible, sparse_emit;
   bool early_refine;
@@ -132,11 +173,12 @@
   uint32_t *d_mslot0 = nullptr, *d_mslot1 = nullptr, *d_midx0 = nullptr, *d_midx1 = nullptr, *d_minfo = nullptr, *d_tile_mlo = nullptr;
   int32_t *d_mid = nullptr, *d_rf = nullptr, *d_rb = nullptr, *d_cover_f = nullptr, *d_cover_b = nullptr;
   int32_t *d_tmin_f = nullptr, *d_tmin_b = nullptr, *d_gmin_f = nullptr, *d_gmin_b = nullptr, *d_pval_p = nullptr, *d_pval_s = nullptr;
-  uint32_t *d_ps0 = nullptr, *d_ps1 = nullptr, *d_pv0 = nullptr, *d_pv1 = nullptr, *d_bidx = nullptr;
+  uint32_t *d_ps0 = nullptr, *d_ps1 = nullptr, *d_bidx = nullptr;
   int2 *d_bfast = nullptr, *d_bfast_all = nullptr;
   uint32_t *d_bidx_all = nullptr;
   uint32_t *d_gend = nullptr, *d_kstart = nullptr, *d_kbidx = nullptr, *d_kbidx_all = nullptr;
-  int32_t *d_kval_p = nullptr, *d_kval_s = nullptr;
+  int32_t *d_kval_p = nullptr, *d_kval_s = nullptr, *d_cover_tot = nullptr;
+  uint8_t *d_kneed = nullptr;
   int2 *d_kbfast = nullptr, *d_kbfast_all = nullptr;
   unsigned long long *d_cand_table = nullptr;
   uint32_t *d_cand_filter = nullptr, *d_cand_lo = nullptr, *d_cand_hi = nullptr, *d_gcand = nullptr;
@@ -161,6 +203,7 @@
   uint32_t *vals = nullptr, *other_vals = nullptr, *slots = nullptr, *other_slots = nullptr, *adep = nullptr, *other_dep = nullptr;
   uint32_t *avals = nullptr, *spare_vals = nullptr;
   bool classified = false, anchors_queued = false;
+  bool anchor_scalars_queued = false;
   size_t n_act = 0, n_large = 0, n_large_groups = 0, n_groups = 0;
   StepTable steps{}, steps_all{};
   StepTable ksteps{}, ksteps_all{};
@@ -224,6 +267,8 @@
     n_sorted = n;
     S.round0_sorted = static_cast<int64_t>(n);
   }
+
+  bool fused_marks() const { return early_refine && !kSerialTail; }
 
   void fork() {
     WP_HIP(hipEventRecord(c->evs[kEvFork], st));
@@ -319,6 +364,7 @@
       d_cover_f = ar.take<int32_t>(2 * static_cast<size_t>(M) + 2);
       d_cover_b = ar.take<int32_t>(2 * static_cast<size_t>(M) + 2);
       d_rb = ar.take<int32_t>(M + 1);
+      d_cover_tot = ar.take<int32_t>(4 * cdiv(static_cast<size_t>(std::max(M, 1)), kCoverChunk));
       d_tile_mlo = ref ? ar.take<uint32_t>(sl_tiles + 2) : nullptr;
       d_tmin_f = ref ? ar.take<int32_t>(sl_tiles + 1) : nullptr;
       d_tmin_b = ref ? ar.take<int32_t>(sl_tiles + 1) : nullptr;
@@ -326,8 +372,6 @@
       d_gmin_b = ref ? ar.take<int32_t>(sl_groups + 1) : nullptr;
       d_ps0 = ar.take<uint32_t>(P_cap + 1);
       d_ps1 = ar.take<uint32_t>(P_cap + 1);
-      d_pv0 = ar.take<uint32_t>(P_cap + 1);
-      d_pv1 = ar.take<uint32_t>(P_cap + 1);
       d_pval_p = ar.take<int32_t>(P_cap + 1);
       d_pval_s = ar.take<int32_t>(P_cap + 1);
       d_bidx = ar.take<uint32_t>(static_cast<size_t>(nbuckets) + 2);
@@ -338,6 +382,7 @@
       d_kstart = key_lookup ? ar.take<uint32_t>(P_cap + 1) : nullptr;
       d_kval_p = key_lookup ? ar.take<int32_t>(P_cap + 1) : nullptr;
       d_kval_s = key_lookup ? ar.take<int32_t>(P_cap + 1) : nullptr;
+      d_kneed = key_lookup ? ar.take<uint8_t>(P_cap + 1) : nullptr;
       d_kbidx = key_lookup ? ar.take<uint32_t>(static_cast<size_t>(nkbuckets) + 2) : nullptr;
       d_kbfast = key_lookup ? ar.take<int2>(static_cast<size_t>(nkbuckets) + 1) : nullptr;
       d_kbidx_all = (key_lookup && key_shift_all != key_shift) ? ar.take<uint32_t>(static_cast<size_t>(nkbuckets_all) + 2) : nullptr;
@@ -375,6 +420,12 @@
                        n_text, d_anchor_cnt, d_anchors);
     hipLaunchKernelGGL(anchor_gap_kernel, dim3(std::min<size_t>(atiles, 1024)), dim3(kBlock), 0, as, d_anchors,
                        c->d_scalars + kScalarAnchors, n_text, d_cls, hv.soft.empty() ? 1 : 0, c->d_scalars + kScalarAnchorGap);
+    if (as == st2 && !kSerialTail) {
+      static_assert(kScalarAnchorGap == kScalarAnchors + 1, "one copy takes both anchor scalars");
+      queue_scalar_slots(c, kScalarAnchors, kScalarAnchorGap, as);
+      WP_HIP(hipEventRecord(c->evs[kEvAnchorScalars], as));
+      anchor_scalars_queued = true;
+    }
   }
 
   void symbols_and_keys() {
@@ -763,8 +814,10 @@
     WP_HIP(hipStreamWaitEvent(st, c->evs[kEvListBuilt], 0));
     hipLaunchKernelGGL(need_ranges_kernel, dim3(tok_blocks), dim3(kBlock), 0, st, keys, n_sorted, c->d_stream, c->d_elig_start,
                        c->d_elig_info, M, c->d_lut, dcode, d_claim, d_gfirst, d_rng_lo, d_rng_hi, d_rng_long, d_tok_group);
-    hipLaunchKernelGGL(group_starts_kernel, dim3(cdiv(M, kBlock)), dim3(kBlock), 0, st, d_gfirst, d_ghead, c->d_scalars + kScalarList,
-                       n_sorted, d_ps0 + P, d_gend);
+    if (!fused_marks()) {
+      hipLaunchKernelGGL(group_starts_kernel, dim3(cdiv(M, kBlock)), dim3(kBlock), 0, st, d_gfirst, d_ghead, c->d_scalars + kScalarList,
+                         n_sorted, d_ps0 + P, d_gend);
+    }
     WP_LAUNCH_CHECK();
     trie_round_finish();
   }
@@ -947,15 +1000,22 @@
     uint32_t *mslot = d_mslot0, *midx = d_midx0;
     if (text_only) {
       if (M > 0) {
-        if (early_refine) {
+        if (fused_marks()) {
+          hipLaunchKernelGGL(token_marks_kernel, dim3(cdiv(M, kBlock)), dim3(kBlock), 0, st, d_node_of_slot, c->d_elig_node,
+                             c->d_elig_subtree, M, d_rng_lo, d_rng_hi, d_rng_long, d_tok_group, d_ghead, d_gfirst,
+                             c->d_scalars + kScalarList, n_sorted, c->d_elig_id, c->d_elig_info, d_mslot0, d_mid, d_minfo, d_rf, d_rb,
+                             d_ps0, d_gend);
+        } else if (early_refine) {
           hipLaunchKernelGGL(trie_token_range_list_kernel, dim3(cdiv(M, kBlock)), dim3(kBlock), 0, st, d_node_of_slot, c->d_elig_node,
                              c->d_elig_subtree, M, d_rng_lo, d_rng_hi, d_rng_long, d_tok_group, d_ghead);
         } else {
           hipLaunchKernelGGL(trie_token_range_kernel, dim3(cdiv(M, kBlock)), dim3(kBlock), 0, st, d_node_of_slot, c->d_elig_node,
                              c->d_elig_subtree, M, d_rng_lo, d_rng_hi, d_rng_long);
         }
-        hipLaunchKernelGGL(virtual_marks_kernel, dim3(cdiv(M, kBlock)), dim3(kBlock), 0, st, d_rng_lo, d_rng_hi, M, c->d_elig_id,
-                           c->d_elig_info, d_mslot0, d_mid, d_minfo, d_rf, d_rb);
+        if (!fused_marks()) {
+          hipLaunchKernelGGL(virtual_marks_kernel, dim3(cdiv(M, kBlock)), dim3(kBlock), 0, st, d_rng_lo, d_rng_hi, M, c->d_elig_id,
+                             c->d_elig_info, d_mslot0, d_mid, d_minfo, d_rf, d_rb);
+        }
       }
       mv = MarkView{mslot, d_mid, d_minfo, d_rf, d_rb, M, d_cover_f, d_cover_b};
     } else {
@@ -980,34 +1040,68 @@
                            sl_tiles, sl_groups, mslot, d_minfo, M, d_tmin_f, d_tmin_b, d_gmin_f, d_gmin_b, d_rf, d_rb);
       }
     }
+    const bool side_tail = key_lookup && !kSerialTail;
+    hipStream_t st3 = side_tail ? c->stream3 : st;
     if (M > 0) {
-      hipLaunchKernelGGL(mark_cover_kernel, dim3(4), dim3(kCoverThreads), 0, st, d_minfo, d_rf, d_rb, M, d_cover_f, d_cover_b);
+      if (side_tail) {
+        WP_HIP(hipEventRecord(c->evs[kEvMarks], st));
+        WP_HIP(hipStreamWaitEvent(st3, c->evs[kEvMarks], 0));
+      }
+      const unsigned chunks = cdiv(M, kCoverChunk);
+      if (chunks > 1) {
+        hipLaunchKernelGGL(mark_cover_totals_kernel, dim3(chunks, 4), dim3(kCoverThreads), 0, st3, d_minfo, d_rf, d_rb, M, d_cover_tot);
+      }
+      hipLaunchKernelGGL(mark_cover_kernel, dim3(chunks, 4), dim3(kCoverThreads), 0, st3, d_minfo, d_rf, d_rb, M,
+                         chunks > 1 ? d_cover_tot : static_cast<const int32_t *>(nullptr), d_cover_f, d_cover_b);
+      if (side_tail) WP_HIP(hipEventRecord(c->evs[kEvCovered], st3));
     }
     if (n_text > 0 && !anchors_queued) launch_anchors(st2);
-    hipLaunchKernelGGL(piece_starts_kernel, dim3(cdiv(std::max(M, 1), kBlock)), dim3(kBlock), 0, st, mv, n_sorted, d_ps0);
+    if (!fused_marks()) {
+      hipLaunchKernelGGL(piece_starts_kernel, dim3(cdiv(std::max(M, 1), kBlock)), dim3(kBlock), 0, st, mv, n_sorted, d_ps0);
+    }
     const int P = this->P + (key_lookup ? 2 * static_cast<int>(n_groups) : 0);
-    const int pc = radix_sort_pairs<uint32_t>(d_ps0, d_pv0, d_ps1, d_pv1, P, 0, bit_length(n), d_radix_tmp, radix_words, st, nullptr);
+    const int pc = radix_sort_pairs<uint32_t>(d_ps0, nullptr, d_ps1, nullptr, P, 0, bit_length(n), d_radix_tmp, radix_words, st, nullptr);
     nbuckets = static_cast<unsigned>(((n_sorted - 1) >> bucket_shift) + 1);
     nbuckets_all = static_cast<unsigned>(((n_sorted - 1) >> bucket_shift_all) + 1);
     uint32_t *pstart = pc ? d_ps1 : d_ps0;
+    if (side_tail) {
+      WP_HIP(hipEventRecord(c->evs[kEvStartsSorted], st));
+      if (M > 0) WP_HIP(hipStreamWaitEvent(st, c->evs[kEvCovered], 0));
+    }
     hipLaunchKernelGGL(piece_values_kernel, dim3(cdiv(static_cast<size_t>(P) * kWave, kBlock)), dim3(kBlock), 0, st, mv, pstart, P,
                        d_pval_p, d_pval_s, pack_steps);
-    hipLaunchKernelGGL(piece_bucket_kernel, dim3(cdiv(nbuckets + 1, kBlock)), dim3(kBlock), 0, st, pstart, P, bucket_shift, nbuckets,
-                       d_bidx);
-    hipLaunchKernelGGL(piece_bucket_fast_kernel, dim3(cdiv(nbuckets, kBlock)), dim3(kBlock), 0, st, d_bidx, d_pval_p, d_pval_s, nbuckets,
-                       d_bfast);
+    if (side_tail) {
+      WP_HIP(hipStreamWaitEvent(st3, c->evs[kEvStartsSorted], 0));
+      side_tables(pstart, P, st3);
+      WP_HIP(hipEventRecord(c->evs[kEvTablesIndexed], st3));
+      WP_HIP(hipStreamWaitEvent(st, c->evs[kEvTablesIndexed], 0));
+      fill_tables(pstart, P);
+    } else {
+      hipLaunchKernelGGL(piece_bucket_kernel, dim3(cdiv(nbuckets + 1, kBlock)), dim3(kBlock), 0, st, pstart, P, bucket_shift, nbuckets,
+                         d_bidx);
+      hipLaunchKernelGGL(piece_bucket_fast_kernel, dim3(cdiv(nbuckets, kBlock)), dim3(kBlock), 0, st, d_bidx, d_pval_p, d_pval_s, nbuckets,
+                         d_bfast);
+      if (bucket_shift_all != bucket_shift) {
+        hipLaunchKernelGGL(piece_bucket_kernel, dim3(cdiv(nbuckets_all + 1, kBlock)), dim3(kBlock), 0, st, pstart, P, bucket_shift_all,
+                           nbuckets_all, d_bidx_all);
+        hipLaunchKernelGGL(piece_bucket_fast_kernel, dim3(cdiv(nbuckets_all, kBlock)), dim3(kBlock), 0, st, d_bidx_all, d_pval_p, d_pval_s,
+                           nbuckets_all, d_bfast_all);
+      }
+    }
     WP_LAUNCH_CHECK();
     steps = StepTable{pstart, d_pval_p, d_pval_s, d_bidx, bucket_shift, pack_steps, d_bfast};
     steps_all = steps;
     if (bucket_shift_all != bucket_shift) {
-      hipLaunchKernelGGL(piece_bucket_kernel, dim3(cdiv(nbuckets_all + 1, kBlock)), dim3(kBlock), 0, st, pstart, P, bucket_shift_all,
-                         nbuckets_all, d_bidx_all);
-      hipLaunchKernelGGL(piece_bucket_fast_kernel, dim3(cdiv(nbuckets_all, kBlock)), dim3(kBlock), 0, st, d_bidx_all, d_pval_p, d_pval_s,
-                         nbuckets_all, d_bfast_all);
-      WP_LAUNCH_CHECK();
       steps_all = StepTable{pstart, d_pval_p, d_pval_s, d_bidx_all, bucket_shift_all, pack_steps, d_bfast_all};
     }
-    if (key_lookup) key_steps(pstart, P, pack_steps);
+    if (key_lookup) {
+      if (!side_tail) key_steps(pstart, P);
+      ksteps = StepTable{d_kstart, d_kval_p, d_kval_s, d_kbidx, key_shift, pack_steps, d_kbfast};
+      ksteps_all = ksteps;
+      if (key_shift_all != key_shift) {
+        ksteps_all = StepTable{d_kstart, d_kval_p, d_kval_s, d_kbidx_all, key_shift_all, pack_steps, d_kbfast_all};
+      }
+    }
     S.step.n_marks = M;
     S.step.n_steps = P;
     S.step.n_tiles = sl_tiles;
@@ -1020,7 +1114,7 @@
     S.step.key_lookup = key_lookup ? 1 : 0;
   }
 
-  void key_steps(const uint32_t *pstart, int P, int pack_steps) {
+  void key_steps(const uint32_t *pstart, int P) {
     const uint32_t *skeys = reinterpret_cast<const uint32_t *>(keys);
     hipLaunchKernelGGL(key_steps_kernel, dim3(cdiv(P, kBlock)), dim3(kBlock), 0, st, pstart, d_pval_p, d_pval_s, P, skeys, d_kstart,
                        d_kval_p, d_kval_s);
@@ -1035,15 +1129,52 @@
                        d_kbidx);
     hipLaunchKernelGGL(piece_bucket_fast_kernel, dim3(cdiv(nkbuckets, kBlock)), dim3(kBlock), 0, st, d_kbidx, d_kval_p, d_kval_s,
                        nkbuckets, d_kbfast);
-    ksteps = StepTable{d_kstart, d_kval_p, d_kval_s, d_kbidx, key_shift, pack_steps, d_kbfast};
-    ksteps_all = ksteps;
     if (key_shift_all != key_shift) {
       hipLaunchKernelGGL(piece_bucket_kernel, dim3(cdiv(nkbuckets_all + 1, kBlock)), dim3(kBlock), 0, st, d_kstart, P, key_shift_all,
                          nkbuckets_all, d_kbidx_all);
       hipLaunchKernelGGL(piece_bucket_fast_kernel, dim3(cdiv(nkbuckets_all, kBlock)), dim3(kBlock), 0, st, d_kbidx_all, d_kval_p,
                          d_kval_s, nkbuckets_all, d_kbfast_all);
-      ksteps_all = StepTable{d_kstart, d_kval_p, d_kval_s, d_kbidx_all, key_shift_all, pack_steps, d_kbfast_all};
-    }
+    }
+    WP_LAUNCH_CHECK();
+  }
+
+  void side_tables(const uint32_t *pstart, int P, hipStream_t s) {
+    const uint32_t *skeys = reinterpret_cast<const uint32_t *>(keys);
+    hipLaunchKernelGGL(key_starts_kernel, dim3(cdiv(P, kBlock)), dim3(kBlock), 0, s, pstart, P, skeys, d_kstart, d_kneed);
+    if (n_groups > 0) {
+      hipLaunchKernelGGL(key_steps_flag_kernel, dim3(cdiv(n_groups, kBlock)), dim3(kBlock), 0, s, d_gfirst, d_gend,
+                         static_cast<uint32_t>(n_groups), pstart, P, d_kneed);
+    }
+    hipLaunchKernelGGL(piece_bucket_kernel, dim3(cdiv(nbuckets + 1, kBlock)), dim3(kBlock), 0, s, pstart, P, bucket_shift, nbuckets, d_bidx);
+    hipLaunchKernelGGL(piece_bucket_kernel, dim3(cdiv(nkbuckets + 1, kBlock)), dim3(kBlock), 0, s, d_kstart, P, key_shift, nkbuckets,
+                       d_kbidx);
+    if (bucket_shift_all != bucket_shift) {
+      hipLaunchKernelGGL(piece_bucket_kernel, dim3(cdiv(nbuckets_all + 1, kBlock)), dim3(kBlock), 0, s, pstart, P, bucket_shift_all,
+                         nbuckets_all, d_bidx_all);
+    }
+    if (key_shift_all != key_shift) {
+      hipLaunchKernelGGL(piece_bucket_kernel, dim3(cdiv(nkbuckets_all + 1, kBlock)), dim3(kBlock), 0, s, d_kstart, P, key_shift_all,
+                         nkbuckets_all, d_kbidx_all);
+    }
+    WP_LAUNCH_CHECK();
+  }
+  void fill_tables(const uint32_t *pstart, int P) {
+    StepFill fill{};
+    unsigned most = static_cast<unsigned>(P);
+    auto add = [&](const uint32_t *bidx, int2 *bfast, unsigned nb, int keyed) {
+      fill.t[fill.count++] = StepFillTable{bidx, bfast, nb, keyed};
+      most = std::max(most, nb);
+    };
+    add(d_bidx, d_bfast, nbuckets, 0);
+    add(d_kbidx, d_kbfast, nkbuckets, 1);
+    if (bucket_shift_all != bucket_shift) add(d_bidx_all, d_bfast_all, nbuckets_all, 0);
+    if (key_shift_all != key_shift) add(d_kbidx_all, d_kbfast_all, nkbuckets_all, 1);
+    hipLaunchKernelGGL(step_tables_kernel, dim3(cdiv(most, kBlock)), dim3(kBlock), 0, st, d_pval_p, d_pval_s, P, d_kneed, d_kval_p, d_kval_s,
+                       fill);
+#ifdef WP_DEBUG_BOUNDS
+    hipLaunchKernelGGL(key_steps_check_kernel, dim3(cdiv(P, kBlock)), dim3(kBlock), 0, st, pstart, P,
+                       reinterpret_cast<const uint32_t *>(keys), d_kval_p, d_kval_s);
+#endif
     WP_LAUNCH_CHECK();
   }
 
@@ -1149,7 +1280,11 @@
     WalkArgs wa = walk_args();
     S.anchor_mode = 0;
     join();
-    fetch_scalars(c, kScalarAnchorGap);
+    if (anchor_scalars_queued) {
+      WP_HIP(hipEventSynchronize(c->evs[kEvAnchorScalars]));
+    } else {
+      fetch_scalars(c, kScalarAnchorGap);
+    }
     size_t n_anchors = c->h_scalars[kScalarAnchors];
     const size_t max_anchor_gap = c->h_scalars[kScalarAnchorGap];
     S.walk.max_anchor_gap = static_cast<int32_t>(max_anchor_gap);
diff --git a/wordpiece_amd/csrc/scanline.h b/wordpiece_amd/csrc/scanline.h
--- a/wordpiece_amd/csrc/scanline.h
+++ b/wordpiece_amd/csrc/scanline.h
@@ -230,60 +230,95 @@
 
 constexpr int kCoverThreads = 1024;
 constexpr int kCoverItems = 8;
+constexpr int kCoverChunk = kCoverThreads * kCoverItems;
+constexpr int32_t kCoverNone = -2147483647 - 1;
+
+__device__ __forceinline__ void cover_values(const uint32_t *__restrict__ minfo, const int32_t *__restrict__ reach, int M, int chunk,
+                                             int c, int back, int32_t (&v)[kCoverItems]) {
+  const int first = chunk * kCoverChunk + static_cast<int>(threadIdx.x) * kCoverItems;
+  uint32_t info[kCoverItems];
+  int32_t rv[kCoverItems];
+#pragma unroll
+  for (int j = 0; j < kCoverItems; j++) {
+    const int i = first + j;
+    const int q = i < M ? (back ? M - 1 - i : i) : 0;
+    info[j] = minfo[q];
+    rv[j] = reach[q];
+  }
+#pragma unroll
+  for (int j = 0; j < kCoverItems; j++) {
+    v[j] = kCoverNone;
+    if (first + j < M && static_cast<int>(info[j] >> kMarkClsShift) == c) v[j] = back ? -rv[j] - 1 : rv[j];
+  }
+}
+
+__global__ __launch_bounds__(kCoverThreads) void mark_cover_totals_kernel(const uint32_t *__restrict__ minfo,
+                                                                          const int32_t *__restrict__ reach_fwd,
+                                                                          const int32_t *__restrict__ reach_bwd, int M,
+                                                                          int32_t *__restrict__ tot) {
+  constexpr int WAVES = kCoverThreads / kWave;
+  __shared__ int32_t wm[WAVES];
+  const int tid = threadIdx.x, lane = tid & 63, w = tid >> 6;
+  const int c = blockIdx.y >> 1, back = blockIdx.y & 1;
+  int32_t v[kCoverItems], mx = kCoverNone;
+  cover_values(minfo, back ? reach_bwd : reach_fwd, M, blockIdx.x, c, back, v);
+#pragma unroll
+  for (int j = 0; j < kCoverItems; j++) mx = max(mx, v[j]);
+  const int32_t inc = wave_incl_max(mx);
+  if (lane == kWave - 1) wm[w] = inc;
+  __syncthreads();
+  if (tid == 0) {
+    int32_t all = kCoverNone;
+#pragma unroll
+    for (int q = 0; q < WAVES; q++) all = max(all, wm[q]);
+    tot[static_cast<size_t>(blockIdx.y) * gridDim.x + blockIdx.x] = all;
+  }
+}
+
 __global__ __launch_bounds__(kCoverThreads) void mark_cover_kernel(const uint32_t *__restrict__ minfo,
                                                                    const int32_t *__restrict__ reach_fwd,
                                                                    const int32_t *__restrict__ reach_bwd, int M,
+                                                                   const int32_t *__restrict__ tot,
                                                                    int32_t *__restrict__ cover_f,
                                                                    int32_t *__restrict__ cover_b) {
   constexpr int WAVES = kCoverThreads / kWave;
-  __shared__ int32_t wm[WAVES];
+  __shared__ int32_t wm[WAVES], cm[WAVES];
   const int tid = threadIdx.x, lane = tid & 63, w = tid >> 6;
-  const int c = blockIdx.x >> 1, back = blockIdx.x & 1;
-  constexpr int32_t kNone = -2147483647 - 1;
-  int32_t carry = kNone;
-  for (int base = 0; base < M; base += kCoverThreads * kCoverItems) {
-    int32_t v[kCoverItems], mx = kNone;
-    uint32_t info[kCoverItems];
-    int32_t rv[kCoverItems];
-    const int32_t *__restrict__ reach = back ? reach_bwd : reach_fwd;
-#pragma unroll
-    for (int j = 0; j < kCoverItems; j++) {
-      const int i = base + tid * kCoverItems + j;
-      const int q = i < M ? (back ? M - 1 - i : i) : 0;
-      info[j] = minfo[q];
-      rv[j] = reach[q];
-    }
-#pragma unroll
-    for (int j = 0; j < kCoverItems; j++) {
-      const int i = base + tid * kCoverItems + j;
-      v[j] = kNone;
-      if (i < M && static_cast<int>(info[j] >> kMarkClsShift) == c) v[j] = back ? -rv[j] - 1 : rv[j];
-      mx = max(mx, v[j]);
-      v[j] = mx;
-    }
-    const int32_t inc = wave_incl_max(mx);
-    if (lane == kWave - 1) wm[w] = inc;
-    __syncthreads();
-    int32_t before = carry, all = carry;
-#pragma unroll
-    for (int q = 0; q < WAVES; q++) {
-      if (q < w) before = max(before, wm[q]);
-      all = max(all, wm[q]);
-    }
-    const int32_t up = __shfl_up(inc, 1, kWave);
-    if (lane > 0) before = max(before, up);
-#pragma unroll
-    for (int j = 0; j < kCoverItems; j++) {
-      const int i = base + tid * kCoverItems + j;
-      if (i < M) {
-        const int q = back ? M - 1 - i : i;
-        const int32_t r = max(before, v[j]);
-        if (back) cover_b[static_cast<size_t>(c) * M + q] = r == kNone ? 2147483647 : -(r + 1);
-        else cover_f[static_cast<size_t>(c) * M + q] = r;
-      }
-    }
-    carry = all;
-    __syncthreads();
+  const int c = blockIdx.y >> 1, back = blockIdx.y & 1, chunk = blockIdx.x;
+  int32_t v[kCoverItems], mx = kCoverNone;
+  cover_values(minfo, back ? reach_bwd : reach_fwd, M, chunk, c, back, v);
+  int32_t before_chunk = kCoverNone;
+  if (tot) {
+    for (int t = tid; t < chunk; t += kCoverThreads) before_chunk = max(before_chunk, tot[static_cast<size_t>(blockIdx.y) * gridDim.x + t]);
+  }
+#pragma unroll
+  for (int j = 0; j < kCoverItems; j++) {
+    mx = max(mx, v[j]);
+    v[j] = mx;
+  }
+  const int32_t inc = wave_incl_max(mx), cinc = wave_incl_max(before_chunk);
+  if (lane == kWave - 1) {
+    wm[w] = inc;
+    cm[w] = cinc;
+  }
+  __syncthreads();
+  int32_t before = kCoverNone;
+#pragma unroll
+  for (int q = 0; q < WAVES; q++) {
+    before = max(before, cm[q]);
+    if (q < w) before = max(before, wm[q]);
+  }
+  const int32_t up = __shfl_up(inc, 1, kWave);
+  if (lane > 0) before = max(before, up);
+#pragma unroll
+  for (int j = 0; j < kCoverItems; j++) {
+    const int i = chunk * kCoverChunk + tid * kCoverItems + j;
+    if (i < M) {
+      const int q = back ? M - 1 - i : i;
+      const int32_t r = max(before, v[j]);
+      if (back) cover_b[static_cast<size_t>(c) * M + q] = r == kCoverNone ? 2147483647 : -(r + 1);
+      else cover_f[static_cast<size_t>(c) * M + q] = r;
+    }
   }
 }
 
@@ -307,6 +342,7 @@
   const int lane = lane_id();
   if (k >= P) return;
   const uint32_t slot = pstart[k];
+  if (k > 0 && (k & (kWave - 1)) != 0 && pstart[k - 1] == slot) return;
   int lo = 0, hi = mv.M;
   while (hi - lo > 64) {
     const int st = (hi - lo) / kWave + 1;
@@ -323,9 +359,10 @@
     hi = first_gt < hi ? first_gt : hi;
     if (!t) hi = lo;
   }
-  while (lo < hi) {
-    const int md = (lo + hi) >> 1;
-    if (mv.mslot[md] <= slot) lo = md + 1; else hi = md;
+  {
+    const int idx = lo + lane;
+    const uint64_t m = __ballot(idx < hi ? mv.mslot[idx] > slot : true);
+    lo = m ? min(hi, lo + __ffsll(static_cast<long long>(m)) - 1) : hi;
   }
   const int ub = lo;
   int xq[2] = {-1, -1}, yq[2] = {-1, -1};
@@ -372,9 +409,10 @@
       if (yq[c] < 0 && b) yq[c] = base + __ffsll(static_cast<long long>(b)) - 1;
     }
   }
-  if (lane < 2) {
-    const int c = lane;
-    const int x = c ? xq[1] : xq[0], y = c ? yq[1] : yq[0];
+  int32_t val[2];
+#pragma unroll
+  for (int c = 0; c < 2; c++) {
+    const int x = xq[c], y = yq[c];
     int wq = -1;
     if (x >= 0 && y >= 0) {
       const int32_t xl = static_cast<int32_t>(mv.minfo[x] & kMarkLenMask), yl = static_cast<int32_t>(mv.minfo[y] & kMarkLenMask);
@@ -386,7 +424,14 @@
     }
     int32_t r = wq >= 0 ? mv.mid[wq] : -1;
     if (packed && r >= 0) r |= static_cast<int32_t>(mv.minfo[wq] & kMarkLenMask) << kStepIdBits;
-    (c ? pval_suffix : pval_prefix)[k] = r;
+    val[c] = r;
+  }
+  const int idx = k + 1 + lane, stop = (k | (kWave - 1)) + 1;
+  const uint64_t same = __ballot(idx < P && idx < stop && pstart[idx] == slot);
+  const int run = 1 + (~same ? __ffsll(static_cast<long long>(~same)) - 1 : kWave);
+  if (lane < run) {
+    pval_prefix[k + lane] = val[0];
+    pval_suffix[k + lane] = val[1];
   }
 }
 
@@ -478,6 +523,51 @@
   kval_suffix[k] = pval_suffix[k];
 }
 
+struct StepFillTable {
+  const uint32_t *bidx;
+  int2 *bfast;
+  unsigned nbuckets;
+  int keyed;
+};
+struct StepFill {
+  StepFillTable t[4];
+  int count;
+};
+__global__ __launch_bounds__(kBlock) void step_tables_kernel(const int32_t *__restrict__ pval_prefix,
+                                                             const int32_t *__restrict__ pval_suffix, int P,
+                                                             const uint8_t *__restrict__ kneed, int32_t *__restrict__ kval_prefix,
+                                                             int32_t *__restrict__ kval_suffix, StepFill fill) {
+  const unsigned i = blockIdx.x * kBlock + threadIdx.x;
+  if (i < static_cast<unsigned>(P)) {
+    const bool nd = kneed[i] != 0;
+    kval_prefix[i] = nd ? kStepNeeded : pval_prefix[i];
+    kval_suffix[i] = nd ? kStepNeeded : pval_suffix[i];
+  }
+#pragma unroll
+  for (int q = 0; q < 4; q++) {
+    if (q >= fill.count || i >= fill.t[q].nbuckets) continue;
+    const uint32_t lo = fill.t[q].bidx[i], hi = fill.t[q].bidx[i + 1];
+    int2 e;
+    if (lo != hi) {
+      e = int2{kStepSlow | static_cast<int32_t>(hi - lo), static_cast<int32_t>(lo)};
+    } else if (fill.t[q].keyed && kneed[lo - 1]) {
+      e = int2{kStepNeeded, kStepNeeded};
+    } else {
+      e = int2{pval_prefix[lo - 1], pval_suffix[lo - 1]};
+    }
+    fill.t[q].bfast[i] = e;
+  }
+}
+
+__global__ __launch_bounds__(kBlock) void key_starts_kernel(const uint32_t *__restrict__ pstart, int P,
+                                                            const uint32_t *__restrict__ sorted_keys, uint32_t *__restrict__ kstart,
+                                                            uint8_t *__restrict__ kneed) {
+  const int k = blockIdx.x * kBlock + threadIdx.x;
+  if (k >= P) return;
+  kstart[k] = k == 0 ? 0u : sorted_keys[pstart[k]];
+  kneed[k] = 0;
+}
+
 __device__ __forceinline__ int starts_lower_bound(const uint32_t *__restrict__ pstart, int P, uint32_t x) {
   int lo = 0, hi = P;
   while (lo < hi) {
@@ -500,6 +590,15 @@
   }
 }
 
+__global__ __launch_bounds__(kBlock) void key_steps_flag_kernel(const uint32_t *__restrict__ gfirst, const uint32_t *__restrict__ gend,
+                                                                uint32_t n_groups, const uint32_t *__restrict__ pstart, int P,
+                                                                uint8_t *__restrict__ kneed) {
+  const uint32_t g = blockIdx.x * kBlock + threadIdx.x;
+  if (g >= n_groups) return;
+  const int k0 = starts_lower_bound(pstart, P, gfirst[g]), k1 = starts_lower_bound(pstart, P, gend[g]);
+  for (int k = k0; k < k1; k++) kneed[k] = 1;
+}
+
 __global__ __launch_bounds__(kBlock) void key_steps_check_kernel(const uint32_t *__restrict__ pstart, int P,
                                                                  const uint32_t *__restrict__ sorted_keys,
                                                                  const int32_t *__restrict__ kval_prefix,
diff --git a/wordpiece_amd/csrc/trie.h b/wordpiece_amd/csrc/trie.h
--- a/wordpiece_amd/csrc/trie.h
+++ b/wordpiece_amd/csrc/trie.h
@@ -144,6 +144,25 @@
   rng_hi[m] = lo;
 }
 
+__device__ __forceinline__ void trie_token_range_in_list(const uint32_t *__restrict__ node_of_entry, uint32_t tok_node,
+                                                         uint32_t tok_subtree, uint32_t glo, uint32_t &rng_lo, uint32_t &rng_hi) {
+  const uint32_t base = rng_lo, ghi = glo + (rng_hi - base);
+  const uint32_t a = tok_node, b = a + tok_subtree;
+  uint32_t lo = glo, hi = ghi;
+  while (lo < hi) {
+    const uint32_t md = lo + ((hi - lo) >> 1);
+    if (node_of_entry[md] < a) lo = md + 1; else hi = md;
+  }
+  const uint32_t first = lo;
+  hi = ghi;
+  while (lo < hi) {
+    const uint32_t md = lo + ((hi - lo) >> 1);
+    if (node_of_entry[md] < b) lo = md + 1; else hi = md;
+  }
+  rng_lo = base + (first - glo);
+  rng_hi = base + (lo - glo);
+}
+
 __global__ __launch_bounds__(kBlock) void trie_token_range_list_kernel(const uint32_t *__restrict__ node_of_entry,
                                                                        const uint32_t *__restrict__ tok_node,
                                                                        const uint32_t *__restrict__ tok_subtree, int M,
@@ -155,21 +174,10 @@
   if (m >= M || !rng_long[m]) return;
   const uint32_t g = tok_group[m];
   if (g == kClaimNoGroup) return;
-  const uint32_t base = rng_lo[m], glo = ghead[g], ghi = glo + (rng_hi[m] - base);
-  const uint32_t a = tok_node[m], b = a + tok_subtree[m];
-  uint32_t lo = glo, hi = ghi;
-  while (lo < hi) {
-    const uint32_t md = lo + ((hi - lo) >> 1);
-    if (node_of_entry[md] < a) lo = md + 1; else hi = md;
-  }
-  const uint32_t first = lo;
-  hi = ghi;
-  while (lo < hi) {
-    const uint32_t md = lo + ((hi - lo) >> 1);
-    if (node_of_entry[md] < b) lo = md + 1; else hi = md;
-  }
-  rng_lo[m] = base + (first - glo);
-  rng_hi[m] = base + (lo - glo);
+  uint32_t lo = rng_lo[m], hi = rng_hi[m];
+  trie_token_range_in_list(node_of_entry, tok_node[m], tok_subtree[m], ghead[g], lo, hi);
+  rng_lo[m] = lo;
+  rng_hi[m] = hi;
 }
 
 }
```
